# petabi/petal-decomposition

Measured on AMD Instinct MI355X. Metric: samples/sec for RandomizedPca.fit() on n x d fp32, higher is better.
Workload: dtype f32

## Files before the change

include/petal_hip.h:

```cpp
#ifndef PETAL_HIP_H
#define PETAL_HIP_H

#include <stddef.h>
#include <stdint.h>

#ifdef __cplusplus
extern "C" {
#endif

typedef struct petal_ctx petal_ctx;

enum { PETAL_OK = 0, PETAL_INVALID_INPUT = 1, PETAL_LINALG_ERROR = 2, PETAL_DEVICE_ERROR = 3 };
enum { PETAL_F32 = 0, PETAL_F64 = 1 };
enum { PETAL_HOST = 0, PETAL_DEVICE = 1 };
enum { PETAL_SUM = 0, PETAL_MAX = 1, PETAL_MIN = 2 };
enum { PETAL_ICA_TEXTBOOK = 0, PETAL_ICA_REFERENCE_LITERAL = 1 };
enum { PETAL_ICA_CONTRAST_LOGCOSH = 0, PETAL_ICA_CONTRAST_EXP = 16, PETAL_ICA_CONTRAST_CUBE = 32 };
enum { PETAL_ICA_SEMANTICS_MASK = 15, PETAL_ICA_CONTRAST_MASK = 240 };

typedef struct petal_matrix {
    void*   data;
    int64_t rows, cols;
    int64_t row_stride, col_stride;
    int32_t dtype;
// ... 12 lines not shown
    double  pass_bytes;
    double  ica_step_ms;
    int64_t ica_step_launches;
    double  ica_step_flops;
    double  ica_step_bytes;
    int64_t n_iter;
    int64_t allreduce_calls;
    double  allreduce_bytes;
    double  allreduce_ms;
    int64_t allreduce_timed;
    int64_t x_row_pitch_bytes;
    int64_t x_zero_copy;
    int64_t rpca_redo;
    double  pow_ms;
    int64_t pow_launches;
    double  stream_ms;
    int64_t stream_launches;
    int64_t ica_redo;
    int64_t ica_gram_split;
    int64_t means_folded;
    int64_t eigh_redo;
} petal_stats;

int         petal_ctx_create(int device, void* stream, petal_ctx** out);
void        petal_ctx_destroy(petal_ctx* ctx);
const char* petal_last_error(const petal_ctx* ctx);
const char* petal_version(void);
int         petal_ctx_set_collective(petal_ctx* ctx, petal_allreduce_fn fn, void* user, int rank, int world_size);
int         petal_rccl_unique_id(void* out128);
int         petal_ctx_init_rccl(petal_ctx* ctx, const void* unique_id128, int rank, int world_size);
int         petal_ctx_collective_info(const petal_ctx* ctx, int* kind, int* rank, int* world_size, int* comm_count, int* comm_device,
                                      int* comm_rank);
int         petal_ctx_set_profiling(petal_ctx* ctx, int profiling);
#define PETAL_GEMM_SPLIT_BF16X3 0
#define PETAL_GEMM_FP32_MFMA 1
#define PETAL_GEMM_SPLIT_BF16X3_EXACT 2
int         petal_ctx_set_gemm_mode(petal_ctx* ctx, int mode);
#define PETAL_OPT_TWO_PLANE_OPERANDS 0
#define PETAL_OPT_TWO_PLANE_OMEGA 1
#define PETAL_OPT_TWO_PLANE_ITERATE 2
#define PETAL_OPT_STEERING_PASSES 3
#define PETAL_OPT_FUSED_PASS 4
#define PETAL_OPT_FUSED_PASS_MIN_ROWS 5
#define PETAL_OPT_VERDICT_THRESHOLD 6
#define PETAL_OPT_MEANS_FOLD_ROWS 7
#define PETAL_OPT_GRAM_SPLIT 8
#define PETAL_OPT_GRAM_SPLIT_HOOK 9
#define PETAL_OPT_D2H_KERNEL 10
#define PETAL_OPT_ROW_PAD 11
#define PETAL_OPT_EIGH_JACOBI 12
#define PETAL_OPT_POISON 13
#define PETAL_OPT_FORCE_COLLECTIVE 14
#define PETAL_OPT_STEERING_HOOK 15
int         petal_ctx_set_option(petal_ctx* ctx, int option, double value);
int         petal_ctx_get_option(const petal_ctx* ctx, int option, double* value);
int         petal_get_stats(const petal_ctx* ctx, petal_stats* out);

int petal_pca_fit(petal_ctx* ctx, const petal_matrix* x, int64_t k, int centering,
                  void* components, void* means, void* singular, void* total_variance,
                  const petal_matrix* y_out);

int petal_rpca_fit(petal_ctx* ctx, const petal_matrix* x, int64_t k, int64_t n_oversample, int64_t n_iter,
                   int centering, const void* omega,
                   void* components, void* means, void* singular, void* total_variance,
                   const petal_matrix* y_out);

int petal_transform(petal_ctx* ctx, const petal_matrix* x, const void* components, const void* means,
                    int64_t k, int64_t d, int centering, const petal_matrix* y_out);
int petal_inverse_transform(petal_ctx* ctx, const petal_matrix* y, const void* components, const void* means,
                            int64_t k, int64_t d, int centering, const petal_matrix* x_out);

int petal_fastica_fit(petal_ctx* ctx, const petal_matrix* x, int64_t n_components, double tol, int64_t max_iter,
                      int mode, const void* w_init, void* components, void* means, int64_t* n_iter,
                      const petal_matrix* y_out);

int petal_ica_par(petal_ctx* ctx, const petal_matrix* x1, double tol, int64_t max_iter, int mode,
                  const void* w_init, void* w_out, int64_t* n_iter);
int petal_symmetric_decorrelation(petal_ctx* ctx, const void* w, int64_t nc, int32_t dtype, int mode, void* out);
int petal_logcosh(petal_ctx* ctx, const petal_matrix* x, const petal_matrix* g_out, void* gprime_out);
int petal_svd_flip(petal_ctx* ctx, const petal_matrix* u, const petal_matrix* vt);

int petal_gemm_xp(petal_ctx* ctx, const petal_matrix* x, const void* mu, const void* p, int64_t N, const void* bias,
                  const petal_matrix* z_out);
int petal_gemm_atb(petal_ctx* ctx, const petal_matrix* a, const void* mu_a, const petal_matrix* b, const void* mu_b,
                   double* c_out);

int petal_power_pass(petal_ctx* ctx, const petal_matrix* x, const void* mu, const void* p, int64_t N, double* y_out,
                     const petal_matrix* z_out, int* fused_out);

#ifdef __cplusplus
}
#endif
#endif
```

petal-decomposition_amd/__init__.py:

```python
from __future__ import annotations

import ctypes as C
import os
import weakref
from typing import Optional

import numpy as np

_HERE = os.path.dirname(os.path.abspath(__file__))
DEFAULT_LIBRARY = os.path.join(_HERE, "libpetal_hip.so")

PETAL_OK, PETAL_INVALID_INPUT, PETAL_LINALG_ERROR, PETAL_DEVICE_ERROR = 0, 1, 2, 3
PETAL_F32, PETAL_F64 = 0, 1
PETAL_HOST, PETAL_DEVICE = 0, 1
PETAL_SUM, PETAL_MAX, PETAL_MIN = 0, 1, 2
GEMM_SPLIT_BF16X3, GEMM_FP32_MFMA, GEMM_SPLIT_BF16X3_EXACT = 0, 1, 2
OPTIONS = {"two_plane_operands": 0, "two_plane_omega": 1, "two_plane_iterate": 2, "steering_passes": 3, "fused_pass": 4,
           "fused_pass_min_rows": 5, "verdict_threshold": 6, "means_fold_rows": 7, "gram_split": 8, "gram_split_hook": 9,
           "d2h_kernel": 10, "row_pad": 11, "eigh_jacobi": 12, "poison": 13, "force_collective": 14, "steering_hook": 15,
           "ipca_fallback": 32,
           "pca_dual": 33, "pca_dual_fallback": 34,
           "kpca_fallback": 36,
           "nmf_fallback": 38}
ICA_TEXTBOOK, ICA_REFERENCE_LITERAL = 0, 1
ICA_CONTRAST_LOGCOSH, ICA_CONTRAST_EXP, ICA_CONTRAST_CUBE = 0, 16, 32
ICA_SEMANTICS_MASK, ICA_CONTRAST_MASK = 15, 240
_ICA_FUN = {"logcosh": ICA_CONTRAST_LOGCOSH, "exp": ICA_CONTRAST_EXP, "cube": ICA_CONTRAST_CUBE}


def _ica_contrast(fun) -> int:
    try:
        return _ICA_FUN[fun]
    except (KeyError, TypeError):
        raise InvalidInput(f"unknown contrast function {fun!r}: one of {sorted(_ICA_FUN)}") from None


from .pcg import Pcg


class DecompositionError(Exception):
    """``DecompositionError`` (src/lib.rs:22-28)."""


class InvalidInput(DecompositionError):
    def __str__(self):
        return "invalid matrix: " + super().__str__()


class LinalgError(DecompositionError):
    def __str__(self):
        return "linear algerba operation failed: " + super().__str__()


class DeviceError(DecompositionError):
    pass


class petal_matrix(C.Structure):
    _fields_ = [("data", C.c_void_p), ("rows", C.c_int64), ("cols", C.c_int64),
                ("row_stride", C.c_int64), ("col_stride", C.c_int64),
                ("dtype", C.c_int32), ("space", C.c_int32)]


class petal_stats(C.Structure):
    _fields_ = [("fit_ms", C.c_double),
                ("xp_ms", C.c_double), ("xp_launches", C.c_int64),
                ("atb_ms", C.c_double), ("atb_launches", C.c_int64),
                ("pass_flops", C.c_double), ("pass_bytes", C.c_double),
                ("ica_step_ms", C.c_double), ("ica_step_launches", C.c_int64),
                ("ica_step_flops", C.c_double), ("ica_step_bytes", C.c_double),
                ("n_iter", C.c_int64),
                ("allreduce_calls", C.c_int64), ("allreduce_bytes", C.c_double),
                ("allreduce_ms", C.c_double), ("allreduce_timed", C.c_int64),
                ("x_row_pitch_bytes", C.c_int64), ("x_zero_copy", C.c_int64),
                ("rpca_redo", C.c_int64), ("pow_ms", C.c_double), ("pow_launches", C.c_int64),
                ("stream_ms", C.c_double), ("stream_launches", C.c_int64), ("ica_redo", C.c_int64), ("ica_gram_split", C.c_int64),
# ... 2034 lines not shown
```

petal-decomposition_amd/csrc/algo.cpp:

```cpp
#include <algorithm>
#include <chrono>
#include <cstdint>
#include <memory>

#include "ctx.h"
#include "../../include/petal_hip_sparse.h"
#include "../../include/petal_hip_ipca.h"
#include "../../include/petal_hip_kpca.h"

namespace petal {

namespace {

double get_elem(const void* p, int dt, int64_t i) {
    return dt == F64 ? static_cast<const double*>(p)[i] : static_cast<double>(static_cast<const float*>(p)[i]);
}
void put_elem(void* p, int dt, int64_t i, double v) {
    if (dt == F64) static_cast<double*>(p)[i] = v;
    else static_cast<float*>(p)[i] = static_cast<float>(v);
}

void check_matrix(const petal_matrix& m, const char* what) {
    if (m.dtype != PETAL_F32 && m.dtype != PETAL_F64) invalid_input(std::string(what) + ": unsupported dtype");
    if (m.rows < 0 || m.cols < 0) invalid_input(std::string(what) + ": negative shape");
// ... 608 lines not shown
                                 steer && it + 1 < n_iter);
                    dev_set_tag(c.dev, TAG_NONE);
                }
            } else {
                op_dgemm(c.dev, true, false, LP, LP, dp, 1.0, Pcur, LP, Yp, LP, 0.0, G, LP);
                op_chol_inv(c.dev, G, L, LP, T.f64(), LP, tol_drop, nullptr, LP);
                op_dgemm(c.dev, false, false, dp, LP, LP, 1.0, Yp, LP, T.f64(), LP, 0.0, Y.f64(), LP);
                op_refill_zero_cols(c.dev, Y.f64(), dp, L, LP, P.f64(), LP);
                orthonormalize_small(c, Y, dp, L, LP, 1e-13);
                dev_set_tag(c.dev, TAG_XP);
                op_gemm_xp(c.dev, dt, X.p, n, dp, X.ld, muT.p, Y.f64(), LP, LP, nullptr, Z.p, LP, nullptr);
                dev_set_tag(c.dev, TAG_NONE);
            }
            Pcur = Y.f64();
        }
        return Pcur;
    }
    void range_basis(const Attempt& a, const double* Pcur) {
        t_rt = false;
        steered = use_pow || steer;
        if (n_iter > 0 && !a.robust) {
            if (!have_yp) {
                dev_set_tag(c.dev, TAG_ATB);
                op_gemm_atb(c.dev, dt, X.p, X.ld, dp, muT.p, Z.p, LP, LP, nullptr, n, Yp, LP);
                dev_set_tag(c.dev, TAG_NONE);
                allreduce_f64(c, Yp, dp * LP + 1, PETAL_SUM);
            }
            op_dgemm(c.dev, true, false, LP, LP, dp, 1.0, Pcur, LP, Yp, LP, 0.0, G, LP);
            t_rt = slot_flip && op_chol_rt(c.dev, dt, n, G, L, LP, T.f64(), LP, tol_drop, ndead, LP, std::max<int64_t>(k, 1));
            if (!slot_flip) op_chol_inv(c.dev, G, L, LP, T.f64(), LP, tol_drop, ndead, LP, std::max<int64_t>(k, 1));
            Usrc = Z.p; Ubuf = Z1.p;
        } else {
            op_gemm_atb(c.dev, dt, Z.p, LP, LP, nullptr, Z.p, LP, LP, nullptr, n, G, LP, true);
            allreduce_f64(c, G, LP * LP, PETAL_SUM);
            op_chol_inv(c.dev, G, L, LP, T.f64(), LP, tol_tall, nullptr, LP);
            op_gemm_xp(c.dev, dt, Z.p, n, LP, LP, nullptr, T.f64(), LP, LP, nullptr, Z1.p, LP, nullptr);
            op_gemm_atb(c.dev, dt, Z1.p, LP, LP, nullptr, Z1.p, LP, LP, nullptr, n, G, LP, true);
            dev_set_tag(c.dev, TAG_ATB);
            op_gemm_atb(c.dev, dt, X.p, X.ld, dp, muT.p, Z1.p, LP, LP, nullptr, n, Yp, LP);
            dev_set_tag(c.dev, TAG_NONE);
            allreduce_f64(c, G, LP * LP, PETAL_SUM);
            allreduce_f64(c, Yp, dp * LP + 1, PETAL_SUM);
            op_chol_inv(c.dev, G, L, LP, T.f64(), LP, tol_tall, nullptr, LP);
            Usrc = Z1.p; Ubuf = Z.p;
        }
        if (t_rt) op_trsm_right(c.dev, Yp, dp, LP, T.f64(), LP, LP, Bt.f64(), LP);
        else op_dgemm(c.dev, false, false, dp, LP, LP, 1.0, Yp, LP, T.f64(), LP, 0.0, Bt.f64(), LP);
    }
    void small_stage(const Attempt& a) {
        if (a.jacobi) dev_memset(c.dev, ndead, 0, 2 * sizeof(double));
        op_dgemm(c.dev, true, false, LP, LP, dp, 1.0, Bt.f64(), LP, Bt.f64(), LP, 0.0, S.f64(), LP);
        if (!a.robust && !a.jacobi) op_eigh(c.dev, S.f64(), L, LP, Uh.f64(), LP, lam, dt == F32 ? 1e-8 : 1e-15, false, LP, std::max<int64_t>(k, 1), neig);
        else op_eigh(c.dev, S.f64(), L, LP, Uh.f64(), LP, lam, dt == F32 ? 1e-8 : 1e-15, true, LP);
        if (!a.robust && !a.exact && two_plane_applies)
            op_tail_verdict(c.dev, lam, L, std::max<int64_t>(k, 1), (tv_from_sq && !tv_direct) ? mu64 : nullptr, dp, d, in.ri.n_total,
                            tv_direct ? mu64 + dp : tvp, steered ? 4e-6 * 1.2 : 4e-6, p2_thr, ndead);
        op_components_out(c.dev, dt, Bt.f64(), LP, Uh.f64(), LP, lam, dt == F32 ? 1e-7 : 1e-12, d, L, k, comp_dev);

        dev_set_tag(c.dev, TAG_STREAM);
        if (slot_flip)
            op_gemm_xp_prod_absmax(c.dev, dt, Usrc, n, LP, LP, nullptr, T.f64(), LP, LP, Uh.f64(), kp, LP, M2.f64(), LP, Ubuf, LP,
                                   in.ri.row_offset, flip, flip + kp, flip + 2 * kp, y_out != nullptr, t_rt);
        else
            op_gemm_xp_prod(c.dev, dt, Usrc, n, LP, LP, nullptr, T.f64(), LP, LP, Uh.f64(), kp, LP, M2.f64(), LP, Ubuf, LP);
        dev_set_tag(c.dev, TAG_NONE);
        Uout = Ubuf;
    }
    void read_back(const Attempt& a) {
        if (slot_flip) flip_signs_to_slot(c, dt, kp, flip, !a.robust ? ndead : nullptr);
        const size_t hres_len = size_t(o.len - o.tv);
        const bool one_view = sizeof(double) * hres_len + comp_bytes <= dev_view_limit(c.dev);
        const double* hres = static_cast<const double*>(dev_d2h_view(c.dev, tvp, sizeof(double) * hres_len + (one_view ? comp_bytes : 0)));
        hcomp = hres + hres_len;
        if (!one_view) {
            comp_keep.resize(comp_bytes);
            dev_d2h(c.dev, comp_keep.data(), comp_dev, comp_bytes);
            hcomp = comp_keep.data();
        }
        dev_sync(c.dev);
        keep.assign(hres, hres + hres_len);
        if (one_view && sharded(c) && !flip_slot_keys(c, dt)) {
            comp_keep.assign(static_cast<const char*>(hcomp), static_cast<const char*>(hcomp) + comp_bytes);
            hcomp = comp_keep.data();
        }
    }
    const double* host(int64_t offset) const { return &keep[size_t(offset - o.tv)]; }
    double verdict() {
        int hdead[3] = {0, 0, 0};
        std::memcpy(hdead, host(o.verdict), sizeof(hdead));
        double code = verdict_code(hdead);
        if (sharded(c)) code = flip_slot_keys(c, dt) ? *host(o.agreed) : agree_max(c, code);
        return code;
    }
    void write_out(const PcaOutputs& out) {
        const std::vector<double> sg = slot_flip ? signs_from_slot(c, dt, host(o.flip), kp)
                                                 : flip_signs(c, dt, Uout, n, kp, LP, in.ri.row_offset);
        const double* hlam = host(o.lam);
        std::vector<double> hs(size_t(std::max<int64_t>(k, 1)), 0.0);
        for (int64_t j = 0; j < k; ++j) hs[j] = std::sqrt(std::max(hlam[j], 0.0));
        const double* hmu = host(o.mu);
        double htv = keep[0];
        if (tv_direct) htv = hmu[dp];
        else if (tv_from_sq) {
            htv = 0;
            for (int64_t j = 0; j < d; ++j) htv += std::max(0.0, hmu[dp + j] - in.ri.n_total * hmu[j] * hmu[j]);
        }
        {
            bool finite = std::isfinite(keep[0]) && std::isfinite(htv);
            for (int64_t j = 0; j < d; ++j) finite = finite && std::isfinite(hmu[j]) && (!tv_from_sq || tv_direct || std::isfinite(hmu[dp + j]));
            for (int64_t j = 0; j < k; ++j) finite = finite && std::isfinite(hlam[j]);
            if (!finite) linalg_error("did not converge");
        }
        write_pca_outputs(c, out, dt, k, d, hcomp, sg.data(), hs.data(), hmu, htv, Uout, n, LP);
    }
};

}

void rpca_fit(petal_ctx& c, const petal_matrix& x, int64_t k, int64_t n_oversample, int64_t n_iter, bool centering,
              const void* omega, void* components, void* means, void* singular, void* total_variance,
              const petal_matrix* y_out) {
    const Timer timer = start_fit(c, x);
    if (k < 0 || n_oversample < 0 || n_iter < 0) invalid_input("negative parameter");
    const int dt = x.dtype;
    const int64_t d = x.cols, l_req = k + n_oversample;
    if (sharded(c) && d > 0 && l_req > 0 && omega == nullptr) invalid_input("omega is required");
    FitInput in = fit_input(c, x, !centering ? 0 : dt == F32 ? 2 : 1, omega, d * l_req);
    if (in.n_total < k || d < k) invalid_input("every dimension should be at least " + std::to_string(k));
    if (centering && in.n_total == 0) {
        if (y_out && (y_out->rows != 0)) invalid_input("output has the wrong shape");
        return;
    }
    const int64_t L = std::min(l_req, std::min(in.n_total, d));
    if (L > 0 && omega == nullptr) invalid_input("omega is required");
    if (d == 0 || L == 0) {
        if (total_variance) put_elem(total_variance, dt, 0, 0.0);
        if (y_out) emit(c, dt, nullptr, x.rows, 0, 0, *y_out);
        return;
    }
    if (!sharded(c)) in.X = ingest(c, x);
    RpcaRun run(c, in, y_out, k, l_req, n_iter, L, centering, omega);
    Attempt a{false, !run.two_plane_applies || dev_option(c.dev, OPT_TWO_PLANE) == 0, false, run.rebase_sketch};
    for (int attempt = 0; attempt < 8; ++attempt) {
        if (!a.jacobi) run.pipeline(a);
        run.small_stage(a);
        run.read_back(a);
        if (!next_attempt(a, a.robust ? 0.0 : run.verdict(), n_iter, c.stats)) break;
    }
    run.write_out({components, means, singular, total_variance, y_out});
    c.stats.means_folded = run.tv_direct ? 1 : 0;
    finish_stats(c, timer);
}

__attribute__((weak)) bool op_row_gram(Dev*, int, const void*, int64_t, int64_t, int64_t, const double*, double*, int64_t, int64_t*) {
    return false;
}
namespace {
constexpr int64_t PCA_DUAL_MIN_D = 2048;
bool pca_dual_applies(const petal_ctx& c, int64_t n_total, int64_t d) {
    if (sharded(c) || c.pca_dual < 0) return false;
    return c.pca_dual > 0 || (n_total < d && d > PCA_DUAL_MIN_D);
}
struct RowGram { bool kernel = false; int64_t chunks = 0; DBuf wide; };
RowGram row_gram_into(petal_ctx& c, const DevMat& X, const double* centre, double* K, int64_t ldk, bool force_fallback = false) {
    RowGram g;
    if (!c.pca_dual_fallback && !force_fallback) {
        dev_set_tag(c.dev, TAG_ATB);
        g.kernel = op_row_gram(c.dev, X.dtype, X.p, X.n, X.dp, X.ld, centre, K, ldk, &g.chunks);
        dev_set_tag(c.dev, TAG_NONE);
    }
    if (g.kernel) return g;
    g.chunks = 0;
    const int64_t n = X.n, dp = X.dp, count = (n - 1) * X.ld + dp;
    g.wide = DBuf(c.dev, sizeof(double) * size_t(count));
    op_cvt_to_f64(c.dev, X.dtype, g.wide.f64(), X.p, count);
    if (centre) {
        const std::vector<double> h1(size_t(n), 1.0);
        DBuf ones(c.dev, sizeof(double) * size_t(n));
        dev_h2d(c.dev, ones.p, h1.data(), ones.bytes);
        op_dgemm(c.dev, false, false, n, dp, 1, -1.0, ones.f64(), 1, centre, dp, 1.0, g.wide.f64(), X.ld);
    }
    op_dgemm(c.dev, false, true, n, n, dp, 1.0, g.wide.f64(), X.ld, g.wide.f64(), X.ld, 0.0, K, ldk);
    return g;
}

void pca_fit_dual(petal_ctx& c, const FitInput& in, int64_t k, bool centering, const PcaOutputs& out) {
    const DevMat& X = in.X;
    const int dt = X.dtype;
    const int64_t n = X.n, d = X.d, dp = X.dp, np = round_up(n, 16), kp = round_up(std::max<int64_t>(k, 1), 16);
    const size_t esz = dtype_size(dt);
    DBuf mu64, muT;
    column_means(c, X, double(n), centering, mu64, muT);
    DBuf K(c.dev, sizeof(double) * np * np), V(c.dev, sizeof(double) * np * np), lam(c.dev, sizeof(double) * np);
    DBuf sig(c.dev, sizeof(double) * np), inv(c.dev, sizeof(double) * np), diag(c.dev, sizeof(double) * np);
    dev_memset(c.dev, K.p, 0, K.bytes);
    RowGram g = row_gram_into(c, X, centering ? mu64.f64() : nullptr, K.f64(), np);
    c.pca_route[0] = 1; c.pca_route[1] = g.kernel ? 1 : 0; c.pca_route[2] = n; c.pca_route[3] = g.chunks;
    std::vector<double> hdiag(np), hs(np), hmu(dp);
    dev_copy2d(c.dev, diag.p, sizeof(double), K.p, (np + 1) * sizeof(double), sizeof(double), size_t(np), 2);
    dev_d2h(c.dev, hdiag.data(), diag.p, diag.bytes);
    dev_sync(c.dev);
    double tvar = 0;
    for (int64_t i = 0; i < n; ++i) tvar += hdiag[i];
    if (!std::isfinite(tvar)) linalg_error("did not converge");
    gram_eigen(c, dt, K, n, np, k, diag, V, lam, nullptr);
    op_sigma_inv(c.dev, lam.f64(), sig.f64(), inv.f64(), np, dt == F32 ? 1e-6 : 1e-10);
    if (centering && k >= n) dev_memset(c.dev, inv.f64() + (n - 1), 0, sizeof(double));
    const std::vector<double> sg = flip_signs(c, F64, V.p, n, k, np, 0);
// ... 3563 lines not shown
```

petal-decomposition_amd/csrc/api.cpp:

```cpp
#include <cstdio>
#include <new>

#include "ctx.h"
#include "../../include/petal_hip_score.h"
#include "../../include/petal_hip_segments.h"
#include "../../include/petal_hip_sparse.h"
#include "../../include/petal_hip_ipca.h"
#include "../../include/petal_hip_wide.h"
#include "../../include/petal_hip_kpca.h"
#include "../../include/petal_hip_nmf.h"
#include "../../include/petal_hip_nmf_sparse.h"
#include "../../include/petal_hip_nmf_kl.h"
#include "../../include/petal_hip_nmf_kl_dense.h"
#include "../../include/petal_hip_nmf_cd.h"
#include "../../include/petal_hip_probe.h"

using namespace petal;

namespace {

struct DeviceScope {
    petal::Dev* dev;
    int prev = -1;
    explicit DeviceScope(petal::Dev* d) : dev(d) { if (dev) prev = dev_push_current(dev); }
// ... 74 lines not shown

int petal_ctx_set_collective(petal_ctx* ctx, petal_allreduce_fn fn, void* user, int rank, int world_size) {
    return guarded(ctx, [&] {
        if (world_size < 1 || rank < 0 || rank >= world_size) invalid_input("bad rank / world_size");
        if (world_size > 1 && !fn) invalid_input("world_size > 1 needs an all-reduce hook");
        rccl_release(*ctx);
        ctx->allreduce = fn;
        ctx->allreduce_user = user;
        ctx->rank = rank;
        ctx->world = world_size;
    });
}

int petal_ctx_set_profiling(petal_ctx* ctx, int profiling) {
    return guarded(ctx, [&] {
        ctx->profiling = profiling < 0 ? 0 : (profiling > 2 ? 2 : profiling);
        dev_set_profiling(ctx->dev, ctx->profiling);
    });
}

int petal_ctx_collective_info(const petal_ctx* ctx, int* kind, int* rank, int* world_size, int* comm_count, int* comm_device,
                              int* comm_rank) {
    if (!ctx) return PETAL_INVALID_INPUT;
    int cnt = -1, dev = -1, rk = -1;
    petal::rccl_info(*ctx, &cnt, &dev, &rk);
    if (kind) *kind = ctx->rccl ? 2 : (ctx->allreduce ? 1 : 0);
    if (rank) *rank = ctx->rank;
    if (world_size) *world_size = ctx->world;
    if (comm_count) *comm_count = cnt;
    if (comm_device) *comm_device = dev;
    if (comm_rank) *comm_rank = rk;
    return PETAL_OK;
}

int petal_ctx_set_gemm_mode(petal_ctx* ctx, int mode) {
    return guarded(ctx, [&] {
        if (mode != PETAL_GEMM_SPLIT_BF16X3 && mode != PETAL_GEMM_FP32_MFMA && mode != PETAL_GEMM_SPLIT_BF16X3_EXACT) invalid_input("unknown GEMM mode");
        dev_set_gemm_mode(ctx->dev, mode);
    });
}

int petal_ctx_set_option(petal_ctx* ctx, int option, double value) {
    return guarded(ctx, [&] {
        if (option == PETAL_OPT_FORCE_COLLECTIVE) { ctx->force_collective = value != 0; return; }
        if (option == PETAL_OPT_IPCA_FALLBACK) { ctx->ipca_fallback = value != 0; return; }
        if (option == PETAL_OPT_PCA_DUAL) {
            if (!(value == value)) invalid_input("unknown ctx option or NaN value");
            ctx->pca_dual = value > 0 ? 1 : (value < 0 ? -1 : 0);
            return;
        }
        if (option == PETAL_OPT_PCA_DUAL_FALLBACK) { ctx->pca_dual_fallback = value != 0; return; }
        if (option == PETAL_OPT_KPCA_FALLBACK) { ctx->kpca_fallback = value != 0; return; }
        if (option == PETAL_OPT_NMF_FALLBACK) { ctx->nmf_fallback = value != 0; return; }
        if (option < 0 || option >= OPT_COUNT || !(value == value)) invalid_input("unknown ctx option or NaN value");
        dev_set_option(ctx->dev, option, value);
    });
}

int petal_ctx_get_option(const petal_ctx* ctx, int option, double* value) {
    if (!ctx || !value) return PETAL_INVALID_INPUT;
    if (option == PETAL_OPT_FORCE_COLLECTIVE) { *value = ctx->force_collective ? 1.0 : 0.0; return PETAL_OK; }
    if (option == PETAL_OPT_IPCA_FALLBACK) { *value = ctx->ipca_fallback ? 1.0 : 0.0; return PETAL_OK; }
    if (option == PETAL_OPT_PCA_DUAL) { *value = double(ctx->pca_dual); return PETAL_OK; }
    if (option == PETAL_OPT_PCA_DUAL_FALLBACK) { *value = ctx->pca_dual_fallback ? 1.0 : 0.0; return PETAL_OK; }
    if (option == PETAL_OPT_KPCA_FALLBACK) { *value = ctx->kpca_fallback ? 1.0 : 0.0; return PETAL_OK; }
    if (option == PETAL_OPT_NMF_FALLBACK) { *value = ctx->nmf_fallback ? 1.0 : 0.0; return PETAL_OK; }
    if (option < 0 || option >= OPT_COUNT) return PETAL_INVALID_INPUT;
    *value = dev_option(ctx->dev, option);
    return PETAL_OK;
}

int petal_get_stats(const petal_ctx* ctx, petal_stats* out) {
    if (!ctx || !out) return PETAL_INVALID_INPUT;
    *out = ctx->stats;
    return PETAL_OK;
}

int petal_pca_fit(petal_ctx* ctx, const petal_matrix* x, int64_t k, int centering, void* components, void* means,
                  void* singular, void* total_variance, const petal_matrix* y_out) {
    return guarded(ctx, [&] {
        need(x, "x");
        pca_fit(*ctx, *x, k, centering != 0, components, means, singular, total_variance, y_out);
    });
}

int petal_rpca_fit(petal_ctx* ctx, const petal_matrix* x, int64_t k, int64_t n_oversample, int64_t n_iter,
                   int centering, const void* omega, void* components, void* means, void* singular,
                   void* total_variance, const petal_matrix* y_out) {
    return guarded(ctx, [&] {
        need(x, "x");
        rpca_fit(*ctx, *x, k, n_oversample, n_iter, centering != 0, omega, components, means, singular, total_variance,
                 y_out);
    });
}

int petal_transform(petal_ctx* ctx, const petal_matrix* x, const void* components, const void* means, int64_t k,
                    int64_t d, int centering, const petal_matrix* y_out) {
    return guarded(ctx, [&] {
        need(x, "x");
        need(y_out, "y_out");
        transform(*ctx, *x, components, means, k, d, centering != 0, *y_out);
    });
}

int petal_inverse_transform(petal_ctx* ctx, const petal_matrix* y, const void* components, const void* means,
                            int64_t k, int64_t d, int centering, const petal_matrix* x_out) {
    return guarded(ctx, [&] {
        need(y, "y");
        need(x_out, "x_out");
        inverse_transform(*ctx, *y, components, means, k, d, centering != 0, *x_out);
    });
}

int petal_score_rows(petal_ctx* ctx, const petal_matrix* x, const void* components, const void* means, int64_t k, int64_t d,
                     int centering, const void* weights, const petal_matrix* out, const petal_matrix* y_out) {
    return guarded(ctx, [&] {
        need(x, "x");
        need(out, "out");
        score_rows(*ctx, *x, components, means, k, d, centering != 0, weights, *out, y_out);
// ... 554 lines not shown
```

petal-decomposition_amd/csrc/hip_ops.hip:

```cpp
#include <hip/hip_runtime.h>

#include <algorithm>
#include <cmath>
#include <cstdio>
#include <cstdlib>
#include <cstring>
#include <map>
#include <set>
#include <stdexcept>
#include <string>
#include <type_traits>
#include <unordered_map>
#include <vector>

#include "ops.h"

namespace petal {

#define HIP_CHECK(expr)                                                                                   \
    do {                                                                                                  \
        hipError_t _e = (expr);                                                                           \
        if (_e != hipSuccess)                                                                             \
            throw std::runtime_error(std::string("HIP error: ") + hipGetErrorString(_e) + " at " #expr);  \
    } while (0)
// ... 3 lines not shown
#ifdef PETAL_DEBUG_COUNTERS
__device__ int g_dbg[4];
__device__ long long g_cyc[32];
__device__ long long g_trace[8 * 16];
#define DBG_T(i) do { if (threadIdx.x == 0) { long long _t = clock64(); g_cyc[i] += _t - _t0; _t0 = _t; } } while (0)
}
extern "C" void petal_debug_trace(long long* out128) {
    (void)hipDeviceSynchronize();
    (void)hipMemcpyFromSymbol(out128, HIP_SYMBOL(petal::g_trace), sizeof(long long) * 128);
}
extern "C" void petal_debug_counters(long long* cyc16, int* dbg4) {
    (void)hipDeviceSynchronize();
    (void)hipMemcpyFromSymbol(cyc16, HIP_SYMBOL(petal::g_cyc), sizeof(long long) * 32);
    (void)hipMemcpyFromSymbol(dbg4, HIP_SYMBOL(petal::g_dbg), sizeof(int) * 4);
    long long z[32] = {0}; int zi[4] = {0};
    (void)hipMemcpyToSymbol(HIP_SYMBOL(petal::g_cyc), z, sizeof(z));
    (void)hipMemcpyToSymbol(HIP_SYMBOL(petal::g_dbg), zi, sizeof(zi));
}
namespace petal {
#else
#define DBG_T(i) do {} while (0)
#endif

struct Dev {
    int device = 0;
    hipStream_t stream = nullptr;
    bool own_stream = false;
    hipStream_t side = nullptr, main_saved = nullptr;
    hipEvent_t ev_fork = nullptr, ev_join = nullptr;
    bool forked = false, on_side = false;
    std::vector<void*> deferred_free;
    int gemm_mode = [] { const char* e = getenv("PETAL_GEMM"); return (e && std::string(e) == "fp32") ? 1 : (e && std::string(e) == "bf16x3-exact") ? 2 : 0; }();
    void* ica_wpk3 = nullptr;
    size_t ica_wpk3_bytes = 0;
    const double* ica_wpk3_for = nullptr;
    int64_t ica_wpk3_nc = 0;
    bool ica_wpk3_valid = false;
    void* ica_x1pl = nullptr;
    size_t ica_x1pl_bytes = 0;
    const void* ica_x1pl_for = nullptr;
    int64_t ica_x1pl_n = 0, ica_x1pl_ld = 0;
    double ica_ortho_tol2 = 1e-26;
    int profiling = 0;
    int tag = 0;
    int tag_seen[TAG_COUNT] = {};
    int tag_count[TAG_COUNT] = {};
    int tag_pick[TAG_COUNT] = {};
    int tag_active = 0;
    int fit_index = 0;
    char* pin = nullptr;
    char* pin_dev = nullptr;
    bool d2h_kernel = true;
    double opt[OPT_COUNT] = {};
    size_t pin_cap = 0, pin_used = 0;
    struct Pend { void* dst; size_t off, bytes; };
    std::vector<Pend> pend;
    std::multimap<size_t, void*> free_list, free_cold;
    bool side_nowait = false;
    std::unordered_map<void*, size_t> live;
    std::vector<hipEvent_t> ev_pool;
    struct Rec { int tag; hipEvent_t a, b; };
    std::vector<Rec> recs;
    KernelTiming acc;
    std::set<const void*> max_lds_set;
    int num_cu = 0;
    int* progress = nullptr;
};

static void dev_defaults_from_env(Dev* d) {
    auto on = [](const char* name) { return getenv(name) != nullptr; };
    auto num = [](const char* name, double dflt) { const char* e = getenv(name); return e ? atof(e) : dflt; };
    d->opt[OPT_TWO_PLANE] = on("PETAL_NO_P2") ? 0 : 1;
    d->opt[OPT_TWO_PLANE_OMEGA] = on("PETAL_NO_P2_OMEGA") ? 0 : 1;
    d->opt[OPT_TWO_PLANE_ITERATE] = on("PETAL_NO_P2_ITERATE") ? 0 : 1;
    d->opt[OPT_STEERING] = on("PETAL_NO_POW3_FAST") ? 0 : 1;
    d->opt[OPT_FUSED_PASS] = on("PETAL_NO_POW3") ? 0 : 1;
    d->opt[OPT_FUSED_PASS_MIN_ROWS] = num("PETAL_POW3_MIN_ROWS", 8192);
    d->opt[OPT_VERDICT_THRESHOLD] = num("PETAL_P2_VERDICT_THR", 4e-6);
    d->opt[OPT_MEANS_FOLD_ROWS] = on("PETAL_NO_MEANS_FOLD") ? -1 : num("PETAL_MEANS_FOLD_ROWS", 200000);
    d->opt[OPT_GRAM_SPLIT] = on("PETAL_NO_GRAM3") ? 0 : 1;
    d->opt[OPT_GRAM_SPLIT_HOOK] = on("PETAL_GRAM_SPLIT") ? 1 : 0;
    d->opt[OPT_D2H_KERNEL] = on("PETAL_D2H_MEMCPY") ? 0 : 1;
    d->opt[OPT_ROW_PAD] = on("PETAL_NO_ROW_PAD") ? 0 : 1;
    d->opt[OPT_EIGH_JACOBI] = on("PETAL_EIGH_JACOBI") ? 1 : 0;
    d->opt[OPT_POISON] = on("PETAL_POISON") ? 1 : 0;
    d->opt[OPT_STEERING_HOOK] = 0;
    d->d2h_kernel = d->opt[OPT_D2H_KERNEL] != 0;
}
void dev_set_option(Dev* d, int opt, double value) {
    if (opt < 0 || opt >= OPT_COUNT) throw std::invalid_argument("unknown ctx option");
    d->opt[opt] = value;
    if (opt == OPT_D2H_KERNEL) d->d2h_kernel = value != 0;
}
double dev_option(const Dev* d, int opt) {
    if (opt < 0 || opt >= OPT_COUNT) throw std::invalid_argument("unknown ctx option");
    return d->opt[opt];
}
static inline bool opt_on(const Dev* d, int opt) { return d->opt[opt] != 0; }

Dev* dev_create(int device, void* stream, char* err, size_t errlen) {
    auto fail = [&](const std::string& m) -> Dev* {
        if (err && errlen) std::snprintf(err, errlen, "%s", m.c_str());
        return nullptr;
    };
    int count = 0;
    hipError_t e = hipGetDeviceCount(&count);
    if (e != hipSuccess || count <= 0)
        return fail(std::string("no HIP device visible (") + hipGetErrorString(e) + "); this library has no CPU fallback");
    if (device < 0 || device >= count) return fail("device index out of range");
    if (hipSetDevice(device) != hipSuccess) return fail("hipSetDevice failed");
    hipDeviceProp_t prop;
    if (hipGetDeviceProperties(&prop, device) != hipSuccess) return fail("hipGetDeviceProperties failed");
    if (std::string(prop.gcnArchName).find("gfx950") == std::string::npos)
        return fail(std::string("device is ") + prop.gcnArchName + ", this library is built for gfx950 (MI355X) only");
    Dev* d = new Dev();
    d->device = device;
    dev_defaults_from_env(d);
    if (stream) {
        d->stream = static_cast<hipStream_t>(stream);
    } else {
        if (hipStreamCreateWithFlags(&d->stream, hipStreamNonBlocking) != hipSuccess) {
            delete d;
            return fail("hipStreamCreate failed");
        }
        d->own_stream = true;
    }
    return d;
}

void dev_destroy(Dev* d) {
    if (!d) return;
    (void)hipSetDevice(d->device);
    (void)hipStreamSynchronize(d->stream);
    for (auto& kv : d->free_list) (void)hipFree(kv.second);
    for (auto& kv : d->free_cold) (void)hipFree(kv.second);
    for (auto& kv : d->live) (void)hipFree(kv.first);
    for (auto& r : d->recs) { (void)hipEventDestroy(r.a); (void)hipEventDestroy(r.b); }
    for (auto ev : d->ev_pool) (void)hipEventDestroy(ev);
    if (d->pin) (void)hipHostFree(d->pin);
    if (d->progress) (void)hipHostFree(d->progress);
// ... 359 lines not shown
```

petal-decomposition_amd/csrc/kernels/host_gemm.inc:

```
#define DISPATCH_T(dt, ...)                              \
    do {                                                 \
        if ((dt) == F64) { using T = double; __VA_ARGS__; } \
        else { using T = float; __VA_ARGS__; }           \
    } while (0)

void op_pack_strided(Dev* d, int dt, const void* src, int64_t n, int64_t dd, int64_t rs, int64_t cs, void* dst, int64_t ld,
                     int64_t dpad) {
    if (n == 0 || dpad == 0) return;
    const int64_t blocks = (n * dpad + 1023) / 1024;
    if (blocks < (int64_t(1) << 31)) {
        DISPATCH_T(dt, hipLaunchKernelGGL(k_pack_flat<T>, dim3((unsigned)blocks), dim3(256), 0, d->stream, (const T*)src, n, dd, rs, cs,
                                          (T*)dst, ld, dpad));
    } else {
        DISPATCH_T(dt, hipLaunchKernelGGL(k_pack_strided<T>, dim3((unsigned)n, cdiv(dpad, 256)), dim3(256), 0, d->stream,
                                          (const T*)src, n, dd, rs, cs, (T*)dst, ld, dpad));
    }
    launch_check();
}
void op_unpack_strided(Dev* d, int dt, const void* src, int64_t n, int64_t dd, int64_t ld, void* dst, int64_t rs, int64_t cs,
                       const double* scale) {
    if (n == 0 || dd == 0) return;
    const int64_t blocks = (n * dd + 1023) / 1024;
    if (blocks < (int64_t(1) << 31)) {
        DISPATCH_T(dt, hipLaunchKernelGGL(k_unpack_scaled<T>, dim3((unsigned)blocks), dim3(256), 0, d->stream, (const T*)src, n, dd, ld,
// ... 52 lines not shown
    launch_check();
}
static bool aligned16(const void* p) { return (reinterpret_cast<uintptr_t>(p) & 15) == 0; }
static bool gemm_split_product(const Dev* d) { return d->gemm_mode != 1; }
static void set_max_lds(Dev* d, const void* fn) {
    if (d->max_lds_set.count(fn)) return;
    HIP_CHECK(hipFuncSetAttribute(fn, hipFuncAttributeMaxDynamicSharedMemorySize, 160 * 1024));
    d->max_lds_set.insert(fn);
}
void op_scale_pad_cols(Dev* d, const double* V, int64_t ldv, const double* inv, int64_t rows, int64_t r, int64_t rp, double* P) {
    if (rows == 0 || rp == 0) return;
    hipLaunchKernelGGL(k_scale_pad_cols, dim3(cdiv(rows * rp, 256)), dim3(256), 0, d->stream, V, ldv, inv, rows, r, rp, P);
    launch_check();
}
void op_transpose_out(Dev* d, int dt, const double* V, int64_t ldv, int64_t dd, int64_t k, void* comp) {
    if (dd == 0 || k == 0) return;
    const dim3 grid(cdiv(dd, 32), cdiv(k, 32));
    if (dt == F32) hipLaunchKernelGGL(k_transpose_out<float>, grid, dim3(256), 0, d->stream, V, ldv, dd, k, (float*)comp);
    else hipLaunchKernelGGL(k_transpose_out<double>, grid, dim3(256), 0, d->stream, V, ldv, dd, k, (double*)comp);
    launch_check();
}
void op_components_out(Dev* d, int dt, const double* Bt, int64_t ldb, const double* Uh, int64_t ldu, const double* lam, double thr,
                       int64_t dd, int64_t L, int64_t k, void* comp) {
    if (k == 0 || dd == 0) return;
    const dim3 grid(cdiv(dd, 64), cdiv(k, 16));
    if (dt == F32)
        hipLaunchKernelGGL(k_components_out<float>, grid, dim3(256), 0, d->stream, Bt, ldb, Uh, ldu, lam, thr, dd, (int)L, k, (float*)comp);
    else
        hipLaunchKernelGGL(k_components_out<double>, grid, dim3(256), 0, d->stream, Bt, ldb, Uh, ldu, lam, thr, dd, (int)L, k, (double*)comp);
    launch_check();
}
static int num_cus(Dev* d) {
    if (!d->num_cu) { hipDeviceProp_t prop; HIP_CHECK(hipGetDeviceProperties(&prop, d->device)); d->num_cu = prop.multiProcessorCount; }
    return d->num_cu;
}

template <int RT, int NT>
static void launch_xp(Dev* d, const float* X, int64_t n, int K, int64_t ldx, const float* mu, const float* Ppk, int NTtot,
                      int nt0, int N, const float* bias, float* Z, int64_t ldz, double* ss_part, int blocks) {
    const bool center = mu != nullptr, ss = ss_part != nullptr;
#define XP_ARGS X, n, K, ldx, mu, Ppk, NTtot, nt0, N, bias, Z, ldz, ss_part
    if (center && ss) hipLaunchKernelGGL((k_xp_mfma<RT, NT, true, true>), dim3(blocks), dim3(256), 0, d->stream, XP_ARGS);
    else if (center) hipLaunchKernelGGL((k_xp_mfma<RT, NT, true, false>), dim3(blocks), dim3(256), 0, d->stream, XP_ARGS);
    else if (ss) hipLaunchKernelGGL((k_xp_mfma<RT, NT, false, true>), dim3(blocks), dim3(256), 0, d->stream, XP_ARGS);
    else hipLaunchKernelGGL((k_xp_mfma<RT, NT, false, false>), dim3(blocks), dim3(256), 0, d->stream, XP_ARGS);
#undef XP_ARGS
    launch_check();
}

struct AbsmaxReq { int64_t cols, row_offset; double *absmax, *idx, *sign; };
static void gemm_xp_impl(Dev* d, int dt, const void* X, int64_t n, int64_t K, int64_t ldx, const void* mu, const double* P, int64_t N,
                         int64_t ldp, const void* bias, void* Z, int64_t ldz, double* sumsq, const double* prod_A, int64_t prod_M,
                         int64_t prod_lda, double* prod_out, int64_t prod_ldo, int prod_rt, const AbsmaxReq* am = nullptr,
                         bool p2_hint = false, bool steering = false);
void op_gemm_xp(Dev* d, int dt, const void* X, int64_t n, int64_t K, int64_t ldx, const void* mu, const double* P, int64_t N,
                int64_t ldp, const void* bias, void* Z, int64_t ldz, double* sumsq, int p_planes, bool steering) {
    gemm_xp_impl(d, dt, X, n, K, ldx, mu, P, N, ldp, bias, Z, ldz, sumsq, nullptr, 0, 0, nullptr, 0, false, nullptr, p_planes == 2, steering);
}
void op_gemm_xp_prod(Dev* d, int dt, const void* X, int64_t n, int64_t K, int64_t ldx, const void* mu, const double* A, int64_t M,
                     int64_t lda, const double* T, int64_t N, int64_t ldt, double* P_out, int64_t ldpo, void* Z, int64_t ldz) {
    const bool fused = dt == F32 && gemm_split_product(d) && n >= 64 && K % 16 == 0 && K > 0 && N % 16 == 0 && ldx % 4 == 0 &&
                       aligned16(X) && (!mu || aligned16(mu)) && ldz % 4 == 0 && aligned16(Z) && K < (1 << 24) && N < (1 << 24);
    if (fused) {
        double* tmpo = P_out ? nullptr : (double*)dev_alloc(d, sizeof(double) * K * N);
        gemm_xp_impl(d, dt, X, n, K, ldx, mu, T, N, ldt, nullptr, Z, ldz, nullptr, A, M, lda, P_out ? P_out : tmpo, P_out ? ldpo : N, false);
        if (tmpo) dev_free(d, tmpo);
        return;
    }
    double* tmp = nullptr;
    double* P = P_out;
    int64_t ldp = ldpo;
    if (!P) { tmp = (double*)dev_alloc(d, sizeof(double) * K * N); P = tmp; ldp = N; }
    op_dgemm(d, false, false, K, N, M, 1.0, A, lda, T, ldt, 0.0, P, ldp);
    op_gemm_xp(d, dt, X, n, K, ldx, mu, P, N, ldp, nullptr, Z, ldz, nullptr);
    if (tmp) dev_free(d, tmp);
}
void op_gemm_xp_prod_absmax(Dev* d, int dt, const void* X, int64_t n, int64_t K, int64_t ldx, const void* mu, const double* A, int64_t M,
                            int64_t lda, const double* T, int64_t N, int64_t ldt, double* P_out, int64_t ldpo, void* Z, int64_t ldz,
                            int64_t row_offset, double* absmax, double* idx, double* sign, bool store_product, bool a_rt) {
    const bool fused = dt == F32 && gemm_split_product(d) && n >= 64 && K % 16 == 0 && K > 0 && N % 16 == 0 && N > 0 && ldx % 4 == 0 &&
                       aligned16(X) && (!mu || aligned16(mu)) && ldz % 4 == 0 && aligned16(Z) && K < (1 << 24) && N < (1 << 24) &&
                       n < (int64_t(1) << 31) && P_out != nullptr;
    if (a_rt && !(M == K && M % 16 == 0 && M <= TRSM_MAXM && N % 16 == 0 && P_out != nullptr)) throw std::logic_error("op_gemm_xp_prod_absmax: RT-form operand of a shape the solve does not take");
    if (a_rt && !fused) {
        switch ((int)(M / 16)) {
#define PETAL_TRSML_CASE(NB)                                                                                                       \
    case NB:                                                                                                                       \
        hipLaunchKernelGGL((k_trsm_left_pack<NB>), dim3(cdiv(N, 16)), dim3(64), 0, d->stream, A, lda, T, ldt, P_out, ldpo, (bf16x8*)nullptr, 0); \
        break
            PETAL_TRSML_CASE(1); PETAL_TRSML_CASE(2); PETAL_TRSML_CASE(3); PETAL_TRSML_CASE(4); PETAL_TRSML_CASE(5);
            PETAL_TRSML_CASE(6); PETAL_TRSML_CASE(7); PETAL_TRSML_CASE(8); PETAL_TRSML_CASE(9);
#undef PETAL_TRSML_CASE
            default: throw std::logic_error("op_gemm_xp_prod_absmax: order out of range");
        }
        launch_check();
        op_gemm_xp_absmax(d, dt, X, n, K, ldx, mu, P_out, N, ldpo, Z, ldz, row_offset, absmax, idx, sign, store_product);
        return;
    }
    if (!fused) {
        op_gemm_xp_prod(d, dt, X, n, K, ldx, mu, A, M, lda, T, N, ldt, P_out, ldpo, Z, ldz);
        op_col_absmax(d, dt, Z, n, N, ldz, row_offset, absmax, idx, sign);
        return;
    }
    const AbsmaxReq am{N, row_offset, absmax, idx, sign};
    gemm_xp_impl(d, dt, X, n, K, ldx, mu, T, N, ldt, nullptr, store_product ? Z : nullptr, ldz, nullptr, A, M, lda, P_out, ldpo, a_rt ? 2 : 0, &am);
}
void op_gemm_xp_absmax(Dev* d, int dt, const void* X, int64_t n, int64_t K, int64_t ldx, const void* mu, const double* P, int64_t N,
                       int64_t ldp, void* Z, int64_t ldz, int64_t row_offset, double* absmax, double* idx, double* sign, bool store_product) {
    const bool fused = dt == F32 && gemm_split_product(d) && n >= 64 && K % 16 == 0 && K > 0 && N % 16 == 0 && N > 0 && ldx % 4 == 0 &&
                       aligned16(X) && (!mu || aligned16(mu)) && ldz % 4 == 0 && aligned16(Z) && K < (1 << 24) && N < (1 << 24) &&
                       n < (int64_t(1) << 31);
    if (!fused) {
        op_gemm_xp(d, dt, X, n, K, ldx, mu, P, N, ldp, nullptr, Z, ldz, nullptr);
        op_col_absmax(d, dt, Z, n, N, ldz, row_offset, absmax, idx, sign);
        return;
    }
    const AbsmaxReq am{N, row_offset, absmax, idx, sign};
    gemm_xp_impl(d, dt, X, n, K, ldx, mu, P, N, ldp, nullptr, store_product ? Z : nullptr, ldz, nullptr, nullptr, 0, 0, nullptr, 0, false, &am);
}
static void gemm_xp_impl(Dev* d, int dt, const void* X, int64_t n, int64_t K, int64_t ldx, const void* mu, const double* P, int64_t N,
                         int64_t ldp, const void* bias, void* Z, int64_t ldz, double* sumsq, const double* prod_A, int64_t prod_M,
                         int64_t prod_lda, double* prod_out, int64_t prod_ldo, int prod_rt, const AbsmaxReq* am, bool p2_hint, bool steering) {
    if (n == 0 || N == 0) return;
    const bool mfma = dt == F32 && K % 16 == 0 && K > 0 && ldx % 4 == 0 && aligned16(X) && (!mu || aligned16(mu)) && n >= 64 &&
                      K < (1 << 24) && N < (1 << 24) && N % 16 == 0 && ldz % 4 == 0 && aligned16(Z) && (!bias || aligned16(bias));
    const bool mfma64 = dt == F64 && K % 8 == 0 && K > 0 && ldx % 2 == 0 && aligned16(X) && (!mu || aligned16(mu)) && n >= 64 &&
                        K < (1 << 24) && N < (1 << 24) && N % 16 == 0;
    if (am && !(mfma && gemm_split_product(d) && !sumsq)) throw std::logic_error("gemm_xp_impl: abs-max epilogue outside the split-product path");
    if (mfma64) {
        const int NTtot = cdiv(N, 16);
        const int64_t total = (K / 8) * (int64_t)NTtot * 64;
        f64x2* Ppk = (f64x2*)dev_alloc(d, sizeof(f64x2) * total);
        hipLaunchKernelGGL(k_pack_p64, dim3(cdiv(total, 256)), dim3(256), 0, d->stream, P, K, N, ldp, Ppk, NTtot, total);
        launch_check();
        const int blocks = cdiv(n, 128);
        double* ssp = sumsq ? (double*)dev_alloc(d, sizeof(double) * blocks * 4) : nullptr;
        const double* Xd = (const double*)X; const double* mud = (const double*)mu; const double* bd = (const double*)bias; double* Zd = (double*)Z;
        TagScope ts(d);
        for (int nt0 = 0; nt0 < NTtot;) {
            const int rem = NTtot - nt0;
            const int w = rem >= 5 ? 5 : rem;
            double* sp = nt0 == 0 ? ssp : nullptr;
#define XP64_ARGS Xd, n, (int)K, ldx, mud, Ppk, NTtot, nt0, (int)N, bd, Zd, ldz, sp
#define XP64_LAUNCH(NTv)                                                                                                            \
            do {                                                                                                                    \
                if (mud && sp) hipLaunchKernelGGL((k_xp_f64<NTv, true, true>), dim3(blocks), dim3(256), 0, d->stream, XP64_ARGS);    \
                else if (mud) hipLaunchKernelGGL((k_xp_f64<NTv, true, false>), dim3(blocks), dim3(256), 0, d->stream, XP64_ARGS);    \
                else if (sp) hipLaunchKernelGGL((k_xp_f64<NTv, false, true>), dim3(blocks), dim3(256), 0, d->stream, XP64_ARGS);     \
                else hipLaunchKernelGGL((k_xp_f64<NTv, false, false>), dim3(blocks), dim3(256), 0, d->stream, XP64_ARGS);            \
            } while (0)
            switch (w) {
                case 5: XP64_LAUNCH(5); break;
                case 4: XP64_LAUNCH(4); break;
                case 3: XP64_LAUNCH(3); break;
                case 2: XP64_LAUNCH(2); break;
                default: XP64_LAUNCH(1); break;
            }
#undef XP64_LAUNCH
#undef XP64_ARGS
            launch_check();
            nt0 += w;
        }
        ts.stop();
        if (sumsq) {
            hipLaunchKernelGGL(k_add_scalar_parts, dim3(1), dim3(256), 0, d->stream, ssp, (int64_t)blocks * 4, sumsq);
            launch_check();
            dev_free(d, ssp);
        }
        dev_free(d, Ppk);
        return;
    }
    if (!mfma) {
        double* ssp = sumsq ? (double*)dev_alloc(d, sizeof(double) * n) : nullptr;
        TagScope ts(d);
        DISPATCH_T(dt, hipLaunchKernelGGL(k_xp_simple<T>, dim3((unsigned)n, cdiv(N, 64)), dim3(64), 0, d->stream, (const T*)X, n,
                                          K, ldx, (const T*)mu, P, N, ldp, (const T*)bias, (T*)Z, ldz, ssp));
        launch_check();
        ts.stop();
        if (sumsq) {
            hipLaunchKernelGGL(k_add_scalar_parts, dim3(1), dim3(256), 0, d->stream, ssp, n, sumsq);
            launch_check();
            dev_free(d, ssp);
        }
        return;
    }
    const int NTtot = cdiv(N, 16);
    if (gemm_split_product(d) && !sumsq) {
        const int64_t nch = (K + 31) / 32, total = nch * NTtot * 64;
        bf16x8* Ppk3 = (bf16x8*)dev_alloc(d, sizeof(bf16x8) * total * 3);
        const bool no_p2 = !opt_on(d, OPT_TWO_PLANE);
        const bool no_p2_it = no_p2 || !opt_on(d, OPT_TWO_PLANE_ITERATE), no_p2_om = no_p2 || !opt_on(d, OPT_TWO_PLANE_OMEGA);
        const bool p2 = p2_hint && ((prod_A && prod_rt && !no_p2_it) || (!prod_A && !no_p2_om)) && !am;
        const bool x2 = p2 && steering && opt_on(d, OPT_STEERING);
        if (prod_A) {
            if (prod_rt == 2) {
                switch ((int)(prod_M / 16)) {
#define PETAL_TRSML_CASE(NB)                                                                                                       \
    case NB:                                                                                                                       \
        hipLaunchKernelGGL((k_trsm_left_pack<NB>), dim3(cdiv(N, 16)), dim3(64), 0, d->stream, prod_A, prod_lda, P, ldp, prod_out, prod_ldo, Ppk3, NTtot); \
        break
                    PETAL_TRSML_CASE(1); PETAL_TRSML_CASE(2); PETAL_TRSML_CASE(3); PETAL_TRSML_CASE(4); PETAL_TRSML_CASE(5);
                    PETAL_TRSML_CASE(6); PETAL_TRSML_CASE(7); PETAL_TRSML_CASE(8); PETAL_TRSML_CASE(9);
#undef PETAL_TRSML_CASE
                    default: throw std::runtime_error("k_trsm_left_pack: order out of range");
                }
            } else if (prod_rt)
                switch ((int)(N / 16)) {
#define PETAL_TRSM_CASE(NB)                                                                                                        \
    case NB:                                                                                                                       \
        if (p2) hipLaunchKernelGGL((k_trsm_pack<NB, true>), dim3(cdiv(K, 16)), dim3(64), trsm_lds_bytes(16 * NB), d->stream, prod_A, prod_lda, P,  \
                                   ldp, K, prod_out, prod_ldo, Ppk3, NTtot);                                                       \
        else hipLaunchKernelGGL((k_trsm_pack<NB, false>), dim3(cdiv(K, 16)), dim3(64), trsm_lds_bytes(16 * NB), d->stream, prod_A, prod_lda, P,  \
                           ldp, K, prod_out, prod_ldo, Ppk3, NTtot);                                                               \
        break
                    PETAL_TRSM_CASE(1); PETAL_TRSM_CASE(2); PETAL_TRSM_CASE(3); PETAL_TRSM_CASE(4); PETAL_TRSM_CASE(5);
                    PETAL_TRSM_CASE(6); PETAL_TRSM_CASE(7); PETAL_TRSM_CASE(8); PETAL_TRSM_CASE(9);
#undef PETAL_TRSM_CASE
                    default: throw std::runtime_error("k_trsm_pack: order out of range");
                }
            else
            hipLaunchKernelGGL(k_dgemm, dim3(cdiv(N, 16), cdiv(K, 16)), dim3(16, 16), 0, d->stream, false, false, K, N, prod_M, 1.0,
                               prod_A, prod_lda, P, ldp, 0.0, prod_out, prod_ldo, prod_M, (double*)nullptr, (const double*)nullptr,
                               Ppk3, NTtot);
        } else {
            hipLaunchKernelGGL(k_pack_p3, dim3(cdiv(total, 256)), dim3(256), 0, d->stream, P, K, N, ldp, Ppk3, NTtot, total);
        }
        launch_check();
        constexpr int RTv = PETAL_XP3_RT, DPv = PETAL_XP3_DEPTH;
        const float* Xf = (const float*)X; const float* muf = (const float*)mu; const float* bf = (const float*)bias; float* Zf = (float*)Z;
        static_assert(RTv == 4, "both workgroup shapes below cover 256 rows: one abs-max partial per 256 rows");
        const int64_t am_parts = cdiv(n, 256), am_ld = am ? am->cols : 0;
        double* am_part = am ? (double*)dev_alloc(d, sizeof(double) * 3 * am_parts * am_ld) : nullptr;
        TagScope ts(d);
        const int npass = cdiv(NTtot, 9);
        for (int nt0 = 0, pass = 0; nt0 < NTtot; ++pass) {
            const int w = (NTtot - nt0 + (npass - pass) - 1) / (npass - pass);
            const size_t lds = sizeof(bf16x8) * 2 * w * 64 * (p2 ? 2 : 3) + sizeof(float) * 32 * nch;
#define XP3_LAUNCH8P(NTv, NPLv)                                                                                                           \
            do {                                                                                                                            \
                const int blocksw = cdiv(n, 256);                                                                                           \
                if (lds > 64 * 1024) set_max_lds(d, muf ? reinterpret_cast<const void*>(k_xp3<2, NTv, DPv, true, 8, PETAL_XP3_OCC, NPLv>) : reinterpret_cast<const void*>(k_xp3<2, NTv, DPv, false, 8, PETAL_XP3_OCC, NPLv>)); \
                if (muf) hipLaunchKernelGGL((k_xp3<2, NTv, DPv, true, 8, PETAL_XP3_OCC, NPLv>), dim3(blocksw), dim3(512), lds, d->stream, Xf, n, (int)K, ldx, muf, Ppk3, NTtot, nt0, (int)N, bf, Zf, ldz, am_part, am_ld); \
                else hipLaunchKernelGGL((k_xp3<2, NTv, DPv, false, 8, PETAL_XP3_OCC, NPLv>), dim3(blocksw), dim3(512), lds, d->stream, Xf, n, (int)K, ldx, muf, Ppk3, NTtot, nt0, (int)N, bf, Zf, ldz, am_part, am_ld); \
            } while (0)
#define XP3_LAUNCH8X(NTv)                                                                                                                 \
            do {                                                                                                                            \
                const int blocksw = cdiv(n, 256);                                                                                           \
                if (lds > 64 * 1024) set_max_lds(d, muf ? reinterpret_cast<const void*>(k_xp3<2, NTv, DPv, true, 8, PETAL_XP3_OCC, 2, true>) : reinterpret_cast<const void*>(k_xp3<2, NTv, DPv, false, 8, PETAL_XP3_OCC, 2, true>)); \
                if (muf) hipLaunchKernelGGL((k_xp3<2, NTv, DPv, true, 8, PETAL_XP3_OCC, 2, true>), dim3(blocksw), dim3(512), lds, d->stream, Xf, n, (int)K, ldx, muf, Ppk3, NTtot, nt0, (int)N, bf, Zf, ldz, am_part, am_ld); \
                else hipLaunchKernelGGL((k_xp3<2, NTv, DPv, false, 8, PETAL_XP3_OCC, 2, true>), dim3(blocksw), dim3(512), lds, d->stream, Xf, n, (int)K, ldx, muf, Ppk3, NTtot, nt0, (int)N, bf, Zf, ldz, am_part, am_ld); \
            } while (0)
#define XP3_LAUNCH8(NTv) do { if (p2 && x2) XP3_LAUNCH8X(NTv); else if (p2) XP3_LAUNCH8P(NTv, 2); else XP3_LAUNCH8P(NTv, 3); } while (0)
            if (w >= 6) {
                switch (w) {
                    case 9: XP3_LAUNCH8(9); break;
                    case 8: XP3_LAUNCH8(8); break;
                    case 7: XP3_LAUNCH8(7); break;
                    default: XP3_LAUNCH8(6); break;
                }
                launch_check();
                nt0 += w;
                continue;
            }
#define XP3_LAUNCHP(RTw, NTv, NPLv)                                                                                                        \
            do {                                                                                                                            \
                const int blocksw = cdiv(n, 64 * RTw);                                                                                      \
                if (lds > 64 * 1024) set_max_lds(d, muf ? reinterpret_cast<const void*>(k_xp3<RTw, NTv, DPv, true, 4, PETAL_XP3_OCC, NPLv>) : reinterpret_cast<const void*>(k_xp3<RTw, NTv, DPv, false, 4, PETAL_XP3_OCC, NPLv>)); \
                if (muf) hipLaunchKernelGGL((k_xp3<RTw, NTv, DPv, true, 4, PETAL_XP3_OCC, NPLv>), dim3(blocksw), dim3(256), lds, d->stream, Xf, n, (int)K, ldx, muf, Ppk3, NTtot, nt0, (int)N, bf, Zf, ldz, am_part, am_ld); \
                else hipLaunchKernelGGL((k_xp3<RTw, NTv, DPv, false, 4, PETAL_XP3_OCC, NPLv>), dim3(blocksw), dim3(256), lds, d->stream, Xf, n, (int)K, ldx, muf, Ppk3, NTtot, nt0, (int)N, bf, Zf, ldz, am_part, am_ld); \
            } while (0)
#define XP3_LAUNCH(RTw, NTv) do { if (p2) XP3_LAUNCHP(RTw, NTv, 2); else XP3_LAUNCHP(RTw, NTv, 3); } while (0)
            switch (w) {
                case 5: XP3_LAUNCH(RTv, 5); break;
                case 4: XP3_LAUNCH(RTv, 4); break;
                case 3: XP3_LAUNCH(RTv, 3); break;
                case 2: XP3_LAUNCH(RTv, 2); break;
                default: XP3_LAUNCH(RTv, 1); break;
// ... 384 lines not shown
            do {                                                                                                                      \
                if (ma) hipLaunchKernelGGL((k_atb3<NTv, true, 8>), grid, block, 0, d->stream, Af, lda, (int)M, ma, Bf, ldb, (int)N, 16 * nt0, n_main, chunk, part, (int)N, (int)n_tail); \
                else hipLaunchKernelGGL((k_atb3<NTv, false, 8>), grid, block, 0, d->stream, Af, lda, (int)M, ma, Bf, ldb, (int)N, 16 * nt0, n_main, chunk, part, (int)N, (int)n_tail); \
            } while (0)
            switch (w) {
                case 5: ATB3_LAUNCH(5); break;
                case 4: ATB3_LAUNCH(4); break;
                case 3: ATB3_LAUNCH(3); break;
                case 2: ATB3_LAUNCH(2); break;
                default: ATB3_LAUNCH(1); break;
            }
#undef ATB3_LAUNCH
            launch_check();
        }
        if (split3_mode) {
            nt0 += w;
            continue;
        }
        switch (w) {
            case 5: launch_atb<5>(d, Af, lda, (int)M, ma, Bf, ldb, (int)N, 16 * nt0, mb, n, chunk, part, (int)nsplit); break;
            case 4: launch_atb<4>(d, Af, lda, (int)M, ma, Bf, ldb, (int)N, 16 * nt0, mb, n, chunk, part, (int)nsplit); break;
            case 3: launch_atb<3>(d, Af, lda, (int)M, ma, Bf, ldb, (int)N, 16 * nt0, mb, n, chunk, part, (int)nsplit); break;
            case 2: launch_atb<2>(d, Af, lda, (int)M, ma, Bf, ldb, (int)N, 16 * nt0, mb, n, chunk, part, (int)nsplit); break;
            default: launch_atb<1>(d, Af, lda, (int)M, ma, Bf, ldb, (int)N, 16 * nt0, mb, n, chunk, part, (int)nsplit); break;
        }
        nt0 += w;
    }
    ts.stop();
    if ((M * N) % 2 == 0 && N % 2 == 0)
        hipLaunchKernelGGL(k_sum_parts4, dim3(cdiv(M * N, 128)), dim3(256), 0, d->stream, part, nslab, M * N, C, N, ldc);
    else
        hipLaunchKernelGGL(k_sum_parts2<float>, dim3(cdiv(M * N, 32)), dim3(256), 0, d->stream, part, nslab, M * N, C, N, ldc, false);
    launch_check();
    dev_free(d, part);
}

__global__ void k_flip_key(const double* __restrict__ t, double* __restrict__ key, int64_t L, const int* __restrict__ flag) {
    const int64_t j = (int64_t)blockIdx.x * blockDim.x + threadIdx.x;
    if (j == L && flag) key[L] = verdict_code(flag);
    if (j >= L) return;
    const double a = t[j] < 0 ? 0.0 : t[j];
    unsigned long long bits = (unsigned long long)__double_as_longlong(a);
    const double rw = t[L + j];
    const unsigned long long row = rw < (double)(1ll << 28) ? (unsigned long long)rw : (1ull << 28) - 1;
    const unsigned long long payload = ((((1ull << 28) - 1) - row) << 1) | (t[2 * L + j] < 0 ? 1ull : 0ull);
    bits = (bits & ~((1ull << 29) - 1)) | (t[j] < 0 ? 0ull : payload);
    key[j] = __longlong_as_double((long long)bits);
}
void op_flip_key(Dev* d, const double* triple, double* key, int64_t L, const int* flag) {
    if (L == 0 && !flag) return;
    hipLaunchKernelGGL(k_flip_key, dim3(cdiv(L + 1, 256)), dim3(256), 0, d->stream, triple, key, L, flag);
    launch_check();
}
__global__ __launch_bounds__(256) void k_tail_verdict(const double* __restrict__ lam, int L, int k, const double* __restrict__ mu_sq, int dp,
                                                       int d, double n_total, const double* __restrict__ tvp, double eps2, double thr,
                                                       int* __restrict__ flag2) {
    __shared__ double red[256];
    const int tid = threadIdx.x;
    double s = 0;
    if (mu_sq) for (int j = tid; j < d; j += 256) s += fmax(0.0, mu_sq[dp + j] - n_total * mu_sq[j] * mu_sq[j]);
    red[tid] = s;
    __syncthreads();
    for (int st = 128; st > 0; st >>= 1) { if (tid < st) red[tid] += red[tid + st]; __syncthreads(); }
    const double tv = mu_sq ? red[0] : tvp[0];
    __syncthreads();
    s = 0;
    for (int j = tid; j < L; j += 256) s += fmax(lam[j], 0.0);
    red[tid] = s;
    __syncthreads();
    for (int st = 128; st > 0; st >>= 1) { if (tid < st) red[tid] += red[tid + st]; __syncthreads(); }
    const double tail = fmax(tv - red[0], 0.0);
    const double T = sqrt(fmax(lam[L - 1], 0.0) * tail / (double)d);
    int bad = 0;
    for (int j = tid; j < k && j < L; j += 256) {
        const double lj = lam[j];
        if (!(lj > 0.0)) continue;
        double gap = j + 1 < L ? lj - fmax(lam[j + 1], 0.0) : lj;
        if (j > 0) gap = fmin(gap, lam[j - 1] - lj);
        const double relgap = fmax(gap / lj, 1e-3);
        if (eps2 * T / lj / relgap > thr) bad = 1;
    }
    if (__syncthreads_or(bad) && tid == 0) flag2[1] = 1;
}
void op_tail_verdict(Dev* d, const double* lam, int64_t L, int64_t k, const double* mu_sq, int64_t dp, int64_t dd, double n_total,
                     const double* tv, double eps2, double thr, int* flag2) {
    if (L <= 0 || k <= 0) return;
    hipLaunchKernelGGL(k_tail_verdict, dim3(1), dim3(256), 0, d->stream, lam, (int)L, (int)k, mu_sq, (int)dp, (int)dd, n_total, tv, eps2, thr, flag2);
    launch_check();
}
void op_col_absmax(Dev* d, int dt, const void* U, int64_t n, int64_t L, int64_t ldu, int64_t row_offset, double* absmax,
                   double* idx, double* sign) {
    if (L == 0) return;
    const int64_t rows = scan_rows_per_block(n, L), nparts = std::max<int64_t>(1, cdiv(n, rows));
    double* part = (double*)dev_alloc(d, sizeof(double) * 3 * nparts * L);
    double *pm = part, *pi = part + nparts * L, *ps = part + 2 * nparts * L;
    if (n == 0) {
        std::vector<double> h(3 * L);
        for (int64_t j = 0; j < L; ++j) { h[j] = -1.0; h[L + j] = INFINITY; h[2 * L + j] = 1.0; }
        dev_h2d(d, absmax, h.data(), sizeof(double) * L);
        dev_h2d(d, idx, h.data() + L, sizeof(double) * L);
        dev_h2d(d, sign, h.data() + 2 * L, sizeof(double) * L);
        dev_free(d, part);
        return;
    }
    DISPATCH_T(dt, hipLaunchKernelGGL(k_absmax_part2<T>, dim3((unsigned)nparts, cdiv(L, 64)), dim3(256), 0, d->stream, (const T*)U,
                                      n, L, ldu, rows, pm, pi, ps));
    launch_check();
    hipLaunchKernelGGL(k_absmax_final, dim3((unsigned)L), dim3(64), 0, d->stream, pm, pi, ps, nparts, L, row_offset, absmax, idx, sign);
    launch_check();
    dev_free(d, part);
}

void op_scale_cols(Dev* d, int dt, void* A, int64_t n, int64_t L, int64_t lda, const double* s) {
    if (n == 0 || L == 0) return;
    DISPATCH_T(dt, hipLaunchKernelGGL(k_scale_cols<T>, dim3((unsigned)n, cdiv(L, 64)), dim3(64), 0, d->stream, (T*)A, n, L, lda, s));
    launch_check();
}
void op_logcosh_rows(Dev* d, int dt, const void* X, int64_t r, int64_t c, int64_t ldx, void* G, int64_t ldg, double* gp) {
    if (r == 0) return;
    DISPATCH_T(dt, hipLaunchKernelGGL(k_logcosh_rows<T>, dim3(cdiv(r, 64)), dim3(64), 0, d->stream, (const T*)X, r, c, ldx, (T*)G, ldg, gp));
    launch_check();
}
```

petal-decomposition_amd/csrc/kernels/host_pow3_eigh.inc:

```
static bool pow3_ok(Dev* d, int dt, const void* X, int64_t n, int64_t K, int64_t ldx, const void* mu, int64_t N, const void* Z, int64_t ldz) {
    const int64_t min_rows = (int64_t)d->opt[OPT_FUSED_PASS_MIN_ROWS];
    return opt_on(d, OPT_FUSED_PASS) && dt == F32 && d->gemm_mode == 0 && (K == 512 || K == 256) && N % 16 == 0 && N >= 16 && N <= 80 && n >= min_rows &&
           n < (int64_t(1) << 40) && ldx % 4 == 0 && aligned16(X) && (!mu || aligned16(mu)) && (!Z || (ldz >= N && aligned16(Z)));
}
static bool pow3_knob_off(const Dev* d, int opt) { return !opt_on(d, OPT_TWO_PLANE) || !opt_on(d, opt); }
bool op_power_pass_applies(Dev* d, int dt, const void* X, int64_t n, int64_t K, int64_t ldx, const void* mu, int64_t N) {
    return pow3_ok(d, dt, X, n, K, ldx, mu, N, nullptr, 0);
}
static void launch_pow3(Dev* d, const float* X, int64_t n, int64_t K, int64_t ldx, const float* mu, const bf16x8* Ppk3, int64_t N, float* Z, int64_t ldz,
                        double* Y, int64_t ldy, double** ssq_parts_out = nullptr, int* nparts_out = nullptr, bool steering = false) {
    const bool ssq_out = ssq_parts_out != nullptr;
    const bool no_fast = !opt_on(d, OPT_STEERING);
    if (steering && !no_fast && !Z) {
        const int NT = (int)(N / 16);
        const int64_t nstages = cdiv(n, 32);
        const int grid = (int)std::min<int64_t>(num_cus(d), nstages);
        float* part = (float*)dev_alloc(d, sizeof(float) * (size_t)grid * K * N);
        double* ssq_part = ssq_out ? (double*)dev_alloc(d, sizeof(double) * (size_t)grid * 8) : nullptr;
        const size_t lds = (size_t)8 * 8192 + (size_t)2 * 8 * NT * 1024 + (size_t)NT * 2048 + 2048;
#define POW3F_GO(NTv, CE, ME)                                                                                                      \
    do {                                                                                                                           \
        if (K == 512) {                                                                                                            \
            set_max_lds(d, reinterpret_cast<const void*>(k_pow3f<NTv, CE, ME, 2>));                                                \
            hipLaunchKernelGGL((k_pow3f<NTv, CE, ME, 2>), dim3(grid), dim3(512), lds, d->stream, X, n, ldx, mu, Ppk3, NT, part, nstages, ssq_part); \
        } else {                                                                                                                   \
            set_max_lds(d, reinterpret_cast<const void*>(k_pow3f<NTv, CE, ME, 1>));                                                \
            hipLaunchKernelGGL((k_pow3f<NTv, CE, ME, 1>), dim3(grid), dim3(512), lds, d->stream, X, n, ldx, mu, Ppk3, NT, part, nstages, ssq_part); \
        }                                                                                                                          \
    } while (0)
#define POW3F_NT(NTv) do { if (ssq_out) POW3F_GO(NTv, true, true); else if (mu) POW3F_GO(NTv, true, false); else POW3F_GO(NTv, false, false); } while (0)
        {
            TagScope ts(d);
            switch (NT) {
                case 5: POW3F_NT(5); break;
                case 4: POW3F_NT(4); break;
                case 3: POW3F_NT(3); break;
                case 2: POW3F_NT(2); break;
                default: POW3F_NT(1); break;
            }
            launch_check();
            ts.stop();
        }
#undef POW3F_NT
#undef POW3F_GO
        hipLaunchKernelGGL(k_sum_parts4, dim3(cdiv(K * N, 128)), dim3(256), 0, d->stream, part, (int64_t)grid, (int64_t)K * N, Y, N, ldy);
        launch_check();
        dev_free(d, part);
        if (ssq_parts_out) { *ssq_parts_out = ssq_part; *nparts_out = grid * 8; }
        return;
    }
    const int NT = (int)(N / 16);
    const int64_t nstages = cdiv(n, 32);
    const int grid = (int)std::min<int64_t>(num_cus(d), nstages);
    float* part = (float*)dev_alloc(d, sizeof(float) * (size_t)grid * K * N);
    double* ssq_part = ssq_out ? (double*)dev_alloc(d, sizeof(double) * (size_t)grid * 8) : nullptr;
    const size_t lds = (size_t)8 * 12288 + (size_t)8 * NT * 1024 + (size_t)NT * 3072 + 2048;
#define POW3_GO(NTv, CE, SZ, ME)                                                                                                  \
    do {                                                                                                                          \
        if (K == 512) {                                                                                                           \
            set_max_lds(d, reinterpret_cast<const void*>(k_pow3<NTv, CE, SZ, ME, 2>));                                            \
            hipLaunchKernelGGL((k_pow3<NTv, CE, SZ, ME, 2>), dim3(grid), dim3(512), lds, d->stream, X, n, ldx, mu, Ppk3, NT, part, Z, ldz, nstages, ssq_part); \
        } else {                                                                                                                  \
            set_max_lds(d, reinterpret_cast<const void*>(k_pow3<NTv, CE, SZ, ME, 1>));                                            \
            hipLaunchKernelGGL((k_pow3<NTv, CE, SZ, ME, 1>), dim3(grid), dim3(512), lds, d->stream, X, n, ldx, mu, Ppk3, NT, part, Z, ldz, nstages, ssq_part); \
        }                                                                                                                         \
    } while (0)
#define POW3_NT(NTv)                                                                                                              \
    do {                                                                                                                          \
        if (ssq_out) POW3_GO(NTv, true, false, true);                                                                             \
        else if (mu && Z) POW3_GO(NTv, true, true, false); else if (mu) POW3_GO(NTv, true, false, false);                         \
        else if (Z) POW3_GO(NTv, false, true, false); else POW3_GO(NTv, false, false, false);                                     \
    } while (0)
    {
        TagScope ts(d);
        switch (NT) {
            case 5: POW3_NT(5); break;
            case 4: POW3_NT(4); break;
            case 3: POW3_NT(3); break;
            case 2: POW3_NT(2); break;
            default: POW3_NT(1); break;
        }
        launch_check();
        ts.stop();
    }
#undef POW3_NT
#undef POW3_GO
    hipLaunchKernelGGL(k_sum_parts4, dim3(cdiv(K * N, 128)), dim3(256), 0, d->stream, part, (int64_t)grid, (int64_t)K * N, Y, N, ldy);
    launch_check();
    dev_free(d, part);
    if (ssq_parts_out) { *ssq_parts_out = ssq_part; *nparts_out = grid * 8; }
}
template <bool FINISH>
__global__ __launch_bounds__(256) void k_mean_fix(double* __restrict__ Y, int K, int d, int N, int64_t ldy, int c1, int L, double n_total,
                                                  const double* __restrict__ P, int64_t ldp, double* __restrict__ mu64, float* __restrict__ muT,
                                                  const double* __restrict__ ssq_part, int nparts, double* __restrict__ tv) {
    __shared__ double sd[512];
    __shared__ double sr[256];
    __shared__ double st[4];
    const int tid = threadIdx.x;
    if (FINISH) {
        for (int f = tid; f < K; f += 256) Y[(int64_t)f * ldy + c1] = 0.0;
        return;
    }
    for (int f = tid; f < K; f += 256) sd[f] = f < d ? Y[(int64_t)f * ldy + c1] / n_total : 0.0;
    __syncthreads();
    const int j0 = blockIdx.x * 4, jj = tid & 3, fl = tid >> 2;
    double acc = 0;
    auto two_plane = [](double v) {
        auto bf = [](float f) {
            unsigned u = __float_as_uint(f);
            u = (u + 0x7fffu + ((u >> 16) & 1u)) & 0xffff0000u;
            return __uint_as_float(u);
        };
        const float f = (float)v, h = bf(f), m = bf(f - h);
        return (double)h + (double)m;
    };
    if (j0 + jj < L)
        for (int f = fl; f < K; f += 64) acc += sd[f] * two_plane(P[(int64_t)f * ldp + j0 + jj]);
    sr[tid] = acc;
    __syncthreads();
    if (tid < 4) {
        double t = 0;
        for (int g = 0; g < 64; ++g) t += sr[g * 4 + tid];
        st[tid] = t;
    }
    __syncthreads();
    if (j0 + jj < L && j0 + jj != c1)
        for (int f = fl; f < K; f += 64) Y[(int64_t)f * ldy + j0 + jj] -= n_total * sd[f] * st[jj];
    if (blockIdx.x == 0) {
        double q = 0;
        for (int f = tid; f < K; f += 256) q += sd[f] * sd[f];
        double sp = 0;
        for (int e = tid; e < nparts; e += 256) sp += ssq_part[e];
        __syncthreads();
        sr[tid] = q;
        __syncthreads();
        for (int h = 128; h > 0; h >>= 1) { if (tid < h) sr[tid] += sr[tid + h]; __syncthreads(); }
        const double q2 = sr[0];
        __syncthreads();
        sr[tid] = sp;
        __syncthreads();
        for (int h = 128; h > 0; h >>= 1) { if (tid < h) sr[tid] += sr[tid + h]; __syncthreads(); }
        if (tid == 0) tv[0] = fmax(sr[0] - n_total * q2, 0.0);
        for (int f = tid; f < K; f += 256) {
            const double m = (double)muT[f] + sd[f];
            mu64[f] = m;
            muT[f] = (float)m;
        }
    }
}
bool op_power_pass_means(Dev* d, int dt, const void* X, int64_t n, int64_t K, int64_t dcols, int64_t ldx, double n_total, const double* P,
                         int64_t N, int64_t ldp, int64_t L, double* Y, int64_t ldy, double* mu64, void* muT, double* ssq_scratch, double* tv) {
    const bool off = d->opt[OPT_MEANS_FOLD_ROWS] < 0 || pow3_knob_off(d, OPT_TWO_PLANE_OMEGA);
    if (off || L >= N || !pow3_ok(d, dt, X, n, K, ldx, muT, N, nullptr, 0)) return false;
    const int64_t ns = std::min<int64_t>(n, 4096), stride = n / ns;
    op_colmean(d, dt, X, ns, K, ldx * stride, double(ns), mu64, muT, false);
    const int64_t total = (K / 32) * (N / 16) * 64;
    bf16x8* Ppk3 = (bf16x8*)dev_alloc(d, sizeof(bf16x8) * total * 3);
    hipLaunchKernelGGL(k_pack_p3, dim3(cdiv(total, 256)), dim3(256), 0, d->stream, P, K, N, ldp, Ppk3, (int)(N / 16), total);
    launch_check();
    double* parts = nullptr;
    int nparts = 0;
    launch_pow3(d, (const float*)X, n, K, ldx, (const float*)muT, Ppk3, N, nullptr, 0, Y, ldy, &parts, &nparts, true);
    dev_free(d, Ppk3);
    (void)ssq_scratch;
    const int c1 = (int)(N - 1);
    hipLaunchKernelGGL(k_mean_fix<false>, dim3((unsigned)cdiv(L, 4)), dim3(256), 0, d->stream, Y, (int)K, (int)dcols, (int)N, ldy, c1, (int)L, n_total, P, ldp,
                       mu64, (float*)muT, (const double*)parts, nparts, tv);
    hipLaunchKernelGGL(k_mean_fix<true>, dim3(1), dim3(256), 0, d->stream, Y, (int)K, (int)dcols, (int)N, ldy, c1, (int)L, n_total, P, ldp, mu64,
                       (float*)muT, (const double*)parts, nparts, tv);
    launch_check();
    dev_free(d, parts);
    return true;
}
bool op_power_pass(Dev* d, int dt, const void* X, int64_t n, int64_t K, int64_t ldx, const void* mu, const double* P, int64_t N, int64_t ldp,
                   void* Z, int64_t ldz, double* Y, int64_t ldy, bool steering) {
    const bool knob = pow3_knob_off(d, OPT_TWO_PLANE_OMEGA);
    if (knob || !pow3_ok(d, dt, X, n, K, ldx, mu, N, Z, ldz)) return false;
    const int64_t total = (K / 32) * (N / 16) * 64;
    bf16x8* Ppk3 = (bf16x8*)dev_alloc(d, sizeof(bf16x8) * total * 3);
    hipLaunchKernelGGL(k_pack_p3, dim3(cdiv(total, 256)), dim3(256), 0, d->stream, P, K, N, ldp, Ppk3, (int)(N / 16), total);
    launch_check();
    launch_pow3(d, (const float*)X, n, K, ldx, (const float*)mu, Ppk3, N, (float*)Z, ldz, Y, ldy, nullptr, nullptr, steering && Z == nullptr);
    dev_free(d, Ppk3);
    return true;
}
bool op_rebase_power_pass(Dev* d, int dt, const void* X, int64_t n, int64_t K, int64_t ldx, const void* mu, const double* G, int64_t L,
                          int64_t ldg, double rel_tol, int* ndead, const double* A, int64_t M, int64_t lda, double* T, int64_t ldt,
                          double* P_out, int64_t ldpo, void* Z, int64_t ldz, double* Y, int64_t ldy, bool steering) {
    const bool no_rt = pow3_knob_off(d, OPT_TWO_PLANE_ITERATE);
    if (!pow3_ok(d, dt, X, n, K, ldx, mu, M, Z, ldz) || no_rt || L == 0 || L > CHOL2_MAXL || M > TRSM_MAXM || M < L || P_out == nullptr) return false;
    launch_chol_rt(d, G, L, ldg, T, ldt, rel_tol, ndead, M);
    const int NTtot = (int)(M / 16);
    const int64_t total = (K / 32) * (int64_t)NTtot * 64;
    bf16x8* Ppk3 = (bf16x8*)dev_alloc(d, sizeof(bf16x8) * total * 3);
    switch (NTtot) {
#define PETAL_TRSM_CASE(NB)                                                                                                            \
    case NB:                                                                                                                           \
        hipLaunchKernelGGL((k_trsm_pack<NB, true>), dim3(cdiv(K, 16)), dim3(64), trsm_lds_bytes(16 * NB), d->stream, A, lda, T, ldt, K, P_out, \
                           ldpo, Ppk3, NTtot);                                                                                         \
        break
        PETAL_TRSM_CASE(1); PETAL_TRSM_CASE(2); PETAL_TRSM_CASE(3); PETAL_TRSM_CASE(4); PETAL_TRSM_CASE(5);
#undef PETAL_TRSM_CASE
        default: throw std::runtime_error("op_rebase_power_pass: order out of range");
    }
    launch_check();
    launch_pow3(d, (const float*)X, n, K, ldx, (const float*)mu, Ppk3, M, (float*)Z, ldz, Y, ldy, nullptr, nullptr, steering && Z == nullptr);
    dev_free(d, Ppk3);
    return true;
}

// ... 388 lines not shown
```

petal-decomposition_amd/csrc/kernels/k_eigen.inc:

```
constexpr int TMW_NV = 8;
__global__ __launch_bounds__(256) void k_tridiag_mw(double* __restrict__ W, int64_t ld, int L, int k, const double* __restrict__ vp_prev,
                                                    double* __restrict__ vp_cur, double* __restrict__ dd, double* __restrict__ ee,
                                                    double* __restrict__ HV, double* __restrict__ tau) {
    extern __shared__ __attribute__((aligned(16))) double sm_mw[];
    double* svp = sm_mw;
    double* swp = svp + L;
    double* svn = swp + L;
    double* s_red = svn + L;
    const int tid = threadIdx.x, lane = tid & 63, wv = tid >> 6;
    int red_slot = 0;
    auto block_sum = [&](double a) {
        for (int off = 32; off > 0; off >>= 1) a += __shfl_xor(a, off, 64);
        double* slot = s_red + 4 * red_slot;
        red_slot ^= 1;
        if (lane == 0) slot[wv] = a;
        __syncthreads();
        return (slot[0] + slot[1]) + (slot[2] + slot[3]);
    };
    double vq[TMW_NV], pq[TMW_NV];
    double pv = 0;
#pragma unroll
    for (int t = 0; t < TMW_NV; ++t) {
        const int j = tid + 256 * t;
        vq[t] = (k > 0 && j < L) ? vp_prev[j] : 0.0;
// ... 1227 lines not shown
    __syncthreads();
    if ((tid & 63) == 0) ws.red[tid >> 6] = lim;
    __syncthreads();
    double tl = 0;
    for (int w = 0; w < (nt >> 6); ++w) tl = fmax(tl, ws.red[w]);
    if (done) return;
    if (res) { for (int e = tid; e < nc * nc; e += nt) W[e] = resl[(e / nc) * ldl + (e % nc)]; }
    else { for (int e = tid; e < nc * nc; e += nt) W[e] = W1[e]; }
    if (wpk3) {
        const int NT = (nc + 15) >> 4, KCH = (16 * NT + 31) >> 5;
        for (int idx = tid; idx < KCH * NT * 64; idx += nt) {
            const int lane = idx & 63, tile = idx >> 6, u = tile % NT, kc = tile / NT;
            const int comp = 16 * u + (lane & 15), k0 = 32 * kc + 8 * (lane >> 4);
            f32x8 x;
#pragma unroll
            for (int e = 0; e < 8; ++e)
                x[e] = (comp < nc && k0 + e < nc) ? (float)(res ? resl[comp * ldl + k0 + e] : W1[comp * nc + k0 + e]) : 0.f;
            bf16x8 h, m, l;
            split3(x, h, m, l);
            wpk3[(tile * 3 + 0) * 64 + lane] = h;
            wpk3[(tile * 3 + 1) * 64 + lane] = m;
            wpk3[(tile * 3 + 2) * 64 + lane] = l;
        }
    }
    if (tid == 0 && (tl < tol)) { state[0] = 1; state[1] = iter + 1; }
    if (tid == 0 && progress) {
        if (tl < tol) __hip_atomic_store(progress, iter + 1, __ATOMIC_RELAXED, __HIP_MEMORY_SCOPE_SYSTEM);
        __hip_atomic_store(progress + 1, iter + 1, __ATOMIC_RELAXED, __HIP_MEMORY_SCOPE_SYSTEM);
    }
}

__global__ void k_dscal(double* x, int64_t count, double alpha) {
    const int64_t e = blockIdx.x * (int64_t)blockDim.x + threadIdx.x;
    if (e < count) x[e] *= alpha;
}
__global__ void k_daxpy(int64_t count, double alpha, const double* x, double* y) {
    const int64_t e = blockIdx.x * (int64_t)blockDim.x + threadIdx.x;
    if (e < count) y[e] += alpha * x[e];
}
__global__ void k_dvec(int mode, const double* x, double* y, int64_t count, double thr) {
    const int64_t e = blockIdx.x * (int64_t)blockDim.x + threadIdx.x;
    if (e >= count) return;
    if (mode == 0) y[e] = sqrt(fmax(x[e], 0.0));
    else if (mode == 2) y[e] = x[e] * x[e];
    else y[e] = (x[e] > thr * x[0] && x[e] > 0.0) ? 1.0 / x[e] : 0.0;
}
__global__ void k_sigma_inv(const double* __restrict__ lam, double* __restrict__ sig, double* __restrict__ inv, int64_t count, double thr) {
    const int64_t e = blockIdx.x * (int64_t)blockDim.x + threadIdx.x;
    if (e >= count) return;
    const double s = sqrt(fmax(lam[e], 0.0)), s0 = sqrt(fmax(lam[0], 0.0));
    sig[e] = s;
    inv[e] = (s > thr * s0 && s > 0.0) ? 1.0 / s : 0.0;
}
template <class T>
__global__ __launch_bounds__(256) void k_components_out(const double* __restrict__ Bt, int64_t ldb, const double* __restrict__ Uh,
                                                        int64_t ldu, const double* __restrict__ lam, double thr, int64_t d, int L,
                                                        int64_t k, T* __restrict__ comp) {
    __shared__ double sB[64][65];
    __shared__ double sU[64][16];
    const int tid = threadIdx.x, ti = tid & 15, tj = tid >> 4;
    const int64_t i0 = (int64_t)blockIdx.x * 64, j0 = (int64_t)blockIdx.y * 16;
    double acc[4] = {0.0, 0.0, 0.0, 0.0};
    for (int l0 = 0; l0 < L; l0 += 64) {
        double vb[16], vu[4];
#pragma unroll
        for (int u = 0; u < 16; ++u) {
            const int r = (tid >> 6) + 4 * u, l = l0 + (tid & 63);
            vb[u] = (i0 + r < d && l < L) ? Bt[(i0 + r) * ldb + l] : 0.0;
        }
#pragma unroll
        for (int u = 0; u < 4; ++u) {
            const int l = l0 + (tid >> 4) + 16 * u;
            vu[u] = (l < L && j0 + ti < k) ? Uh[(int64_t)l * ldu + j0 + ti] : 0.0;
        }
        __syncthreads();
#pragma unroll
        for (int u = 0; u < 16; ++u) sB[(tid >> 6) + 4 * u][tid & 63] = vb[u];
#pragma unroll
        for (int u = 0; u < 4; ++u) sU[(tid >> 4) + 16 * u][ti] = vu[u];
        __syncthreads();
#pragma unroll 8
        for (int l = 0; l < 64; ++l) {
            const double u = sU[l][tj];
#pragma unroll
            for (int r = 0; r < 4; ++r) acc[r] += sB[ti + 16 * r][l] * u;
        }
    }
    const int64_t j = j0 + tj;
    if (j < k) {
        const double s = sqrt(fmax(lam[j], 0.0)), s0 = sqrt(fmax(lam[0], 0.0));
        const double inv = (s > thr * s0 && s > 0.0) ? 1.0 / s : 0.0;
#pragma unroll
        for (int r = 0; r < 4; ++r) {
            const int64_t i = i0 + ti + 16 * r;
            if (i < d) comp[j * d + i] = (T)(acc[r] * inv);
        }
    }
}
__global__ void k_scale_pad_cols(const double* __restrict__ V, int64_t ldv, const double* __restrict__ inv, int64_t rows, int64_t r,
                                 int64_t rp, double* __restrict__ P) {
    const int64_t e = (int64_t)blockIdx.x * blockDim.x + threadIdx.x;
    if (e >= rows * rp) return;
    const int64_t i = e / rp, j = e - i * rp;
    P[e] = j < r ? V[i * ldv + j] * inv[j] : 0.0;
}
template <class T>
__global__ __launch_bounds__(256) void k_transpose_out(const double* __restrict__ V, int64_t ldv, int64_t d, int64_t k, T* __restrict__ comp) {
    __shared__ double tile[32][33];
    const int tx = threadIdx.x & 31, ty = threadIdx.x >> 5;
    const int64_t i0 = (int64_t)blockIdx.x * 32, j0 = (int64_t)blockIdx.y * 32;
#pragma unroll
    for (int u = 0; u < 4; ++u) {
        const int64_t i = i0 + ty + 8 * u, j = j0 + tx;
        tile[ty + 8 * u][tx] = (i < d && j < k) ? V[i * ldv + j] : 0.0;
    }
    __syncthreads();
#pragma unroll
    for (int u = 0; u < 4; ++u) {
        const int64_t j = j0 + ty + 8 * u, i = i0 + tx;
        if (j < k && i < d) comp[j * d + i] = (T)tile[tx][ty + 8 * u];
    }
}
template <class T>
__global__ __launch_bounds__(256) void k_colmean_final(const double* __restrict__ part, const double* __restrict__ part_lo, int64_t nparts,
                                                       int64_t w, int64_t d, double inv_n, double n_total, double* __restrict__ mu64,
                                                       T* __restrict__ muT) {
    __shared__ double red[32][9], redc[32][9];
    const int e = threadIdx.x & 7, pl = threadIdx.x >> 3;
    const int64_t j = (int64_t)blockIdx.x * 8 + e;
    const bool pairs = sizeof(T) == 8 && part_lo;
    double acc = 0, lo = 0;
    if (j < w) {
        if (pairs) {
            for (int64_t p = pl; p < nparts; p += 32) { two_sum_acc(acc, lo, part[p * w + j]); lo += part_lo[p * w + j]; }
        } else {
            for (int64_t p = pl; p < nparts; p += 32) acc += part[p * w + j];
        }
    }
    red[pl][e] = acc; redc[pl][e] = lo;
    __syncthreads();
    if (pl == 0 && j < w) {
        double t = 0;
        if (pairs) {
            double c = 0;
#pragma unroll
            for (int k = 0; k < 32; ++k) { two_sum_acc(t, c, red[k][e]); c += redc[k][e]; }
            if (j < d) {
                const double q = t / n_total;
                t = q + (fma(-q, n_total, t) + c) / n_total;
                muT[j] = (T)t;
// ... 80 lines not shown
```

petal-decomposition_amd/csrc/kernels/k_gemm_split_k1.inc:

```
typedef __bf16 bf16x8 __attribute__((ext_vector_type(8)));
typedef float f32x8 __attribute__((ext_vector_type(8)));
typedef __bf16 bf16x2 __attribute__((ext_vector_type(2)));
typedef float f32x2 __attribute__((ext_vector_type(2)));
typedef unsigned u32x4 __attribute__((ext_vector_type(4)));
__device__ __forceinline__ unsigned cvt_pk_bf16(float a, float b) {
    return __builtin_bit_cast(unsigned, __builtin_convertvector(f32x2{a, b}, bf16x2));
}
#ifndef PETAL_STEER_PIECES
#define PETAL_STEER_PIECES 4
#endif
#ifndef PETAL_SPLIT_DOT2
#define PETAL_SPLIT_DOT2 1
#endif
__device__ __forceinline__ void sub_pk_bf16(float& x0, float& x1, unsigned pk) {
#if PETAL_SPLIT_DOT2
    unsigned c0u, c1u;
    asm("s_mov_b32 %0, 0xbf80" : "=s"(c0u));
    asm("s_mov_b32 %0, 0xbf800000" : "=s"(c1u));
    x0 = __builtin_amdgcn_fdot2_f32_bf16(__builtin_bit_cast(bf16x2, pk), __builtin_bit_cast(bf16x2, c0u), x0, false);
    x1 = __builtin_amdgcn_fdot2_f32_bf16(__builtin_bit_cast(bf16x2, pk), __builtin_bit_cast(bf16x2, c1u), x1, false);
#else
    x0 -= __uint_as_float(pk << 16);
    x1 -= __uint_as_float(pk & 0xffff0000u);
#endif
}
__device__ __forceinline__ void split3(const f32x8 x, bf16x8& h, bf16x8& m, bf16x8& l) {
    u32x4 hh, mm, ll;
#pragma unroll
    for (int e = 0; e < 4; ++e) {
        float r0 = x[2 * e], r1 = x[2 * e + 1];
        hh[e] = cvt_pk_bf16(r0, r1);
        sub_pk_bf16(r0, r1, hh[e]);
        mm[e] = cvt_pk_bf16(r0, r1);
        sub_pk_bf16(r0, r1, mm[e]);
        ll[e] = cvt_pk_bf16(r0, r1);
    }
    h = __builtin_bit_cast(bf16x8, hh);
    m = __builtin_bit_cast(bf16x8, mm);
    l = __builtin_bit_cast(bf16x8, ll);
}
__device__ __forceinline__ void split2(const f32x8 x, bf16x8& h, bf16x8& m) {
    u32x4 hh, mm;
#pragma unroll
    for (int e = 0; e < 4; ++e) {
        float r0 = x[2 * e], r1 = x[2 * e + 1];
        hh[e] = cvt_pk_bf16(r0, r1);
        sub_pk_bf16(r0, r1, hh[e]);
        mm[e] = cvt_pk_bf16(r0, r1);
    }
    h = __builtin_bit_cast(bf16x8, hh);
    m = __builtin_bit_cast(bf16x8, mm);
}
__global__ __launch_bounds__(256) void k_pack_p3(const double* __restrict__ P, int64_t K, int64_t N, int64_t ldp,
                                                 bf16x8* __restrict__ out, int NTtot, int64_t total) {
    const int64_t idx = (int64_t)blockIdx.x * 256 + threadIdx.x;
    if (idx >= total) return;
    const int lane = (int)(idx & 63);
    const int64_t tile = idx >> 6;
    const int nt = (int)(tile % NTtot);
    const int64_t c = tile / NTtot;
    const int64_t col = 16 * nt + (lane & 15), k0 = 32 * c + 8 * (lane >> 4);
    f32x8 x;
#pragma unroll
    for (int e = 0; e < 8; ++e) x[e] = (k0 + e < K && col < N) ? (float)P[(k0 + e) * ldp + col] : 0.f;
    bf16x8 h, m, l;
    split3(x, h, m, l);
    out[(tile * 3 + 0) * 64 + lane] = h;
    out[(tile * 3 + 1) * 64 + lane] = m;
    out[(tile * 3 + 2) * 64 + lane] = l;
}
#ifndef PETAL_XP3_RT
#define PETAL_XP3_RT 4
#define PETAL_XP3_DEPTH 1
#define PETAL_XP3_OCC 2
#endif
template <int RT, int NT, int DEPTH, bool CENTER, int WVK = 4, int OCC = PETAL_XP3_OCC, int NPL = 3, bool X2 = false>
__global__ __launch_bounds__(64 * WVK, OCC) void k_xp3(const float* __restrict__ X, int64_t n, int K, int64_t ldx,
                                                            const float* __restrict__ mu, const bf16x8* __restrict__ Ppk3,
                                                            int NTtot, int nt0, int N, const float* __restrict__ bias,
                                                            float* __restrict__ Z, int64_t ldz, double* __restrict__ amax,
                                                            int64_t am_ld) {
    constexpr int PITEMS = NT * 64 * NPL;
    constexpr int NTHR = 64 * WVK;
    constexpr int PI = (PITEMS + NTHR - 1) / NTHR;
    extern __shared__ __attribute__((aligned(16))) unsigned char sm_xp3[];
    bf16x8* sP = reinterpret_cast<bf16x8*>(sm_xp3);
    float* sMu = reinterpret_cast<float*>(sm_xp3 + sizeof(bf16x8) * 2 * PITEMS);
    const int tid = threadIdx.x, lane = tid & 63, wave = tid >> 6;
    const int i = lane & 15, q = lane >> 4;
    const int64_t row0 = ((int64_t)blockIdx.x * WVK + wave) * (16 * RT);
    const int nchunk = (K + 31) >> 5;
    if (CENTER)
        for (int k = tid; k < 32 * nchunk; k += NTHR) sMu[k] = k < K ? mu[k] : 0.f;
    f32x4 acc[RT][NT];
#pragma unroll
    for (int t = 0; t < RT; ++t)
#pragma unroll
        for (int u = 0; u < NT; ++u) acc[t][u] = f32x4{0.f, 0.f, 0.f, 0.f};
    const float* xrow[RT];
#pragma unroll
    for (int t = 0; t < RT; ++t) {
        const int64_t r = row0 + 16 * t + i;
        xrow[t] = X + (r < n ? r : (n - 1)) * ldx + 8 * q;
    }
    const bf16x8* psrc = Ppk3 + (int64_t)nt0 * 192;
    int poff[PI];
#pragma unroll
    for (int it = 0; it < PI; ++it) {
        const int j = tid + NTHR * it;
        poff[it] = NPL == 3 ? j : (j / (64 * NPL)) * 192 + (j % (64 * NPL));
    }
    auto load_a = [&](int c, f32x8(&a)[RT]) {
        const bool in = 32 * c + 8 * q < K;
#pragma unroll
        for (int t = 0; t < RT; ++t) {
            f32x4 lo = f32x4{0.f, 0.f, 0.f, 0.f}, hi = lo;
            if (in) { lo = ld_stream(xrow[t] + 32 * c); hi = ld_stream(xrow[t] + 32 * c + 4); }
            a[t] = f32x8{lo[0], lo[1], lo[2], lo[3], hi[0], hi[1], hi[2], hi[3]};
        }
    };
    auto load_p = [&](int c, bf16x8(&pn)[PI]) {
#pragma unroll
// ... 161 lines not shown
```

petal-decomposition_amd/csrc/kernels/k_generic.inc:

```
template <class T>
__global__ void k_pack_strided(const T* __restrict__ src, int64_t n, int64_t d, int64_t rs, int64_t cs, T* __restrict__ dst,
                               int64_t ld, int64_t dpad) {
    const int64_t j = blockIdx.y * (int64_t)blockDim.x + threadIdx.x;
    const int64_t i = blockIdx.x;
    if (j >= dpad) return;
    dst[i * ld + j] = j < d ? src[i * rs + j * cs] : T(0);
}
template <class T>
__global__ void k_unpack_strided(const T* __restrict__ src, int64_t n, int64_t d, int64_t ld, T* __restrict__ dst, int64_t rs,
                                 int64_t cs) {
    const int64_t j = blockIdx.y * (int64_t)blockDim.x + threadIdx.x;
    const int64_t i = blockIdx.x;
    if (j >= d) return;
    dst[i * rs + j * cs] = src[i * ld + j];
}
template <class T>
__global__ __launch_bounds__(256) void k_pack_flat(const T* __restrict__ src, int64_t n, int64_t d, int64_t rs, int64_t cs, T* __restrict__ dst,
                                                   int64_t ld, int64_t dpad) {
    const int64_t total = n * dpad;
#pragma unroll
    for (int u = 0; u < 4; ++u) {
        const int64_t e = ((int64_t)blockIdx.x * 4 + u) * 256 + threadIdx.x;
        if (e >= total) return;
        const int64_t i = e / dpad, j = e - i * dpad;
// ... 91 lines not shown
    if (SQ) redq[ry][cx] = (q0 + q1) + (q2 + q3);
    __syncthreads();
    if (ry == 0 && j < d) {
        const int64_t w = SQ ? 2 * d : d;
        part[(int64_t)blockIdx.x * w + j] = (red[0][cx] + red[1][cx]) + (red[2][cx] + red[3][cx]);
        if (SQ) part[(int64_t)blockIdx.x * w + d + j] = (redq[0][cx] + redq[1][cx]) + (redq[2][cx] + redq[3][cx]);
    }
}
template <class T>
__global__ __launch_bounds__(256) void k_absmax_part2(const T* __restrict__ U, int64_t n, int64_t L, int64_t ldu, int64_t rows,
                                                      double* __restrict__ pmax, double* __restrict__ pidx,
                                                      double* __restrict__ psgn) {
    __shared__ double rm[SCAN_RY][64], ri[SCAN_RY][64], rs[SCAN_RY][64];
    const int cx = threadIdx.x & 63, ry = threadIdx.x >> 6;
    const int64_t j = blockIdx.y * (int64_t)64 + cx;
    const int64_t r0 = (int64_t)blockIdx.x * rows, r1 = min(n, r0 + rows);
    double best = -1.0, bi = INFINITY, bs = 1.0;
    if (j < L) {
#pragma unroll 4
        for (int64_t i = r0 + ry; i < r1; i += SCAN_RY) {
            const double v = (double)U[i * ldu + j], a = fabs(v);
            if (a > best) { best = a; bi = (double)i; bs = signbit(v) ? -1.0 : 1.0; }
        }
    }
    rm[ry][cx] = best; ri[ry][cx] = bi; rs[ry][cx] = bs;
    __syncthreads();
    if (ry == 0 && j < L) {
#pragma unroll
        for (int k = 1; k < SCAN_RY; ++k)
            if (rm[k][cx] > best || (rm[k][cx] == best && ri[k][cx] < bi)) { best = rm[k][cx]; bi = ri[k][cx]; bs = rs[k][cx]; }
        const int64_t o = (int64_t)blockIdx.x * L + j;
        pmax[o] = best; pidx[o] = bi; psgn[o] = bs;
    }
}
template <class TP>
__global__ __launch_bounds__(256) void k_sum_parts2(const TP* __restrict__ part, int64_t nparts, int64_t count,
                                                    double* __restrict__ out, int64_t N, int64_t ldc, bool accumulate) {
    __shared__ double red[8][33];
    const int tx = threadIdx.x & 31, ty = threadIdx.x >> 5;
    const int64_t e = (int64_t)blockIdx.x * 32 + tx;
    double s = 0;
    if (e < count)
        for (int64_t p = ty; p < nparts; p += 8) s += (double)part[p * count + e];
    red[ty][tx] = s;
    __syncthreads();
    if (ty == 0 && e < count) {
        double t = 0;
#pragma unroll
        for (int k = 0; k < 8; ++k) t += red[k][tx];
        double* o = out + (e / N) * ldc + (e % N);
        *o = accumulate ? *o + t : t;
    }
}
__global__ __launch_bounds__(256) void k_sum_parts4(const float* __restrict__ part, int64_t nparts, int64_t count,
                                                    double* __restrict__ out, int64_t N, int64_t ldc) {
    __shared__ double red[3][64][3];
    const int lane = threadIdx.x & 63, wave = threadIdx.x >> 6;
    const int64_t e = ((int64_t)blockIdx.x * 64 + lane) * 2;
    double s0 = 0, s1 = 0;
    if (e < count) {
        const float* src = part + e;
        int64_t p = wave;
        for (; p + 28 < nparts; p += 32) {
            f32x2 v[8];
#pragma unroll
            for (int k = 0; k < 8; ++k) v[k] = *reinterpret_cast<const f32x2*>(src + (p + 4 * k) * count);
#pragma unroll
            for (int k = 0; k < 8; ++k) { s0 += (double)v[k][0]; s1 += (double)v[k][1]; }
        }
        for (; p < nparts; p += 4) {
            const f32x2 v = *reinterpret_cast<const f32x2*>(src + p * count);
            s0 += (double)v[0]; s1 += (double)v[1];
        }
    }
    if (wave > 0) { red[wave - 1][lane][0] = s0; red[wave - 1][lane][1] = s1; }
    __syncthreads();
    if (wave == 0 && e < count) {
#pragma unroll
        for (int w = 0; w < 3; ++w) { s0 += red[w][lane][0]; s1 += red[w][lane][1]; }
        double* o = out + (e / N) * ldc + (e % N);
        o[0] = s0; o[1] = s1;
    }
}
__global__ __launch_bounds__(256) void k_add_scalar_parts(const double* __restrict__ part, int64_t nparts, double* __restrict__ out) {
    __shared__ double red[256];
    double s = 0;
    for (int64_t p = threadIdx.x; p < nparts; p += 256) s += part[p];
    red[threadIdx.x] = s;
    __syncthreads();
    for (int st = 128; st > 0; st >>= 1) {
        if ((int)threadIdx.x < st) red[threadIdx.x] += red[threadIdx.x + st];
        __syncthreads();
    }
    if (threadIdx.x == 0) out[0] += red[0];
}

template <class T>
__global__ void k_xp_simple(const T* __restrict__ X, int64_t n, int64_t K, int64_t ldx, const T* __restrict__ mu,
                            const double* __restrict__ P, int64_t N, int64_t ldp, const T* __restrict__ bias,
                            T* __restrict__ Z, int64_t ldz, double* __restrict__ ss_part) {
    const int64_t j = blockIdx.y * (int64_t)blockDim.x + threadIdx.x;
    const int64_t i = blockIdx.x;
    double acc = 0, ss = 0;
    const bool want_ss = ss_part != nullptr && blockIdx.y == 0 && threadIdx.x == 0;
    if (j < N || want_ss) {
        for (int64_t k = 0; k < K; ++k) {
            T xv = X[i * ldx + k];
            if (mu) xv = xv - mu[k];
            const double a = (double)xv;
            if (j < N) acc += a * (sizeof(T) == 4 ? (double)(float)P[k * ldp + j] : P[k * ldp + j]);
            ss += a * a;
        }
    }
    if (j < N) Z[i * ldz + j] = (T)(acc + (bias ? (double)bias[j] : 0.0));
    if (want_ss) ss_part[i] = ss;
}

constexpr int ATB_S_ROWS = 256;
template <class T>
__global__ void k_atb_simple(const T* __restrict__ A, int64_t lda, int64_t M, const T* __restrict__ muA,
                             const T* __restrict__ B, int64_t ldb, int64_t N, const T* __restrict__ muB, int64_t n,
                             double* __restrict__ part) {
    const int64_t j = blockIdx.y * (int64_t)blockDim.x + threadIdx.x;
    const int64_t m = blockIdx.z * (int64_t)blockDim.y + threadIdx.y;
    if (j >= N || m >= M) return;
    const int64_t r0 = (int64_t)blockIdx.x * ATB_S_ROWS, r1 = min(n, r0 + ATB_S_ROWS);
    const T ma = muA ? muA[m] : T(0), mb = muB ? muB[j] : T(0);
    double s = 0;
    for (int64_t i = r0; i < r1; ++i) s += (double)(T)(A[i * lda + m] - ma) * (double)(T)(B[i * ldb + j] - mb);
    part[((int64_t)blockIdx.x * M + m) * N + j] = s;
}
__global__ __launch_bounds__(64) void k_absmax_final(const double* __restrict__ pmax, const double* __restrict__ pidx,
                                                     const double* __restrict__ psgn, int64_t nparts, int64_t L,
                                                     int64_t row_offset, double* __restrict__ omax, double* __restrict__ oidx,
// ... 35 lines not shown
```

petal-decomposition_amd/csrc/kernels/k_smallmat.inc:

```
__global__ __launch_bounds__(256) void k_dgemm(bool ta, bool tb, int64_t M, int64_t N, int64_t K, double alpha,
                                               const double* __restrict__ A, int64_t lda, const double* __restrict__ B, int64_t ldb,
                                               double beta, double* __restrict__ C, int64_t ldc, int64_t kchunk,
                                               double* __restrict__ part, const double* __restrict__ colscale,
                                               bf16x8* __restrict__ pk3, int NTtot) {
    constexpr int BK = 32;
    __shared__ double sa[16][BK + 1], sb[BK][17];
    const int tx = threadIdx.x, ty = threadIdx.y;
    const int64_t i0 = (int64_t)blockIdx.y * 16, j0 = (int64_t)blockIdx.x * 16;
    const int64_t kbeg = (int64_t)blockIdx.z * kchunk;
    if (K > kbeg + kchunk) K = kbeg + kchunk;
    double acc = 0;
    for (int64_t k0 = kbeg; k0 < K; k0 += BK) {
#pragma unroll
        for (int h = 0; h < 2; ++h) {
            if (ta) {
                const int kk = ty + 16 * h;
                const int64_t k = k0 + kk, i = i0 + tx;
                sa[tx][kk] = (i < M && k < K) ? A[k * lda + i] : 0.0;
            } else {
                const int kk = tx + 16 * h;
                const int64_t k = k0 + kk, i = i0 + ty;
                sa[ty][kk] = (i < M && k < K) ? A[i * lda + k] : 0.0;
            }
            if (tb) {
// ... 97 lines not shown
        cf64x4 pt = cf64x4{0.0, 0.0, 0.0, 0.0};
#pragma unroll
        for (int r = 0; r < 4; ++r) pt = __builtin_amdgcn_mfma_f64_16x16x4f64(cur[I][r], X[I][r], pt, 0, 0, 0);
#pragma unroll
        for (int J = I + 1; J < NB; ++J) {
#pragma unroll
            for (int r = 0; r < 4; ++r)
                X[J] = __builtin_amdgcn_mfma_f64_16x16x4f64(-cur[J][r], pt[r], X[J], 0, 0, 0);
        }
#pragma unroll
        for (int r = 0; r < 4; ++r) sP[li * ldsp + 16 * I + lk + 4 * r] = pt[r];
        __builtin_amdgcn_sched_barrier(0);
    }
    __syncthreads();
    if (P_out && !P2)
        for (int e = lane; e < 16 * M; e += 64) {
            const int r = e / M, c = e - r * M;
            P_out[(i0 + r) * ldpo + c] = sP[r * ldsp + c];
        }
    if (pk3) {
        for (int idx = lane; idx < 2 * M; idx += 64) {
            const int g = idx / M, col = idx - g * M;
            bf16x8 h, m, l;
            if (P2) {
#pragma unroll
                for (int e = 0; e < 8; ++e) {
                    double hd, md;
                    two_plane_f64(sP[(8 * g + e) * ldsp + col], hd, md);
                    h[e] = (__bf16)(float)hd;
                    m[e] = (__bf16)(float)md;
                    if (P_out) P_out[(i0 + 8 * g + e) * ldpo + col] = hd + md;
                }
            } else {
                f32x8 x;
#pragma unroll
                for (int e = 0; e < 8; ++e) x[e] = (float)sP[(8 * g + e) * ldsp + col];
                split3(x, h, m, l);
            }
            const int64_t c = i0 >> 5, tile = c * NTtot + (col >> 4);
            const int ln = (col & 15) + 16 * (int)(((i0 & 31) + 8 * g) >> 3);
            pk3[(tile * 3 + 0) * 64 + ln] = h;
            pk3[(tile * 3 + 1) * 64 + ln] = m;
            if (!P2) pk3[(tile * 3 + 2) * 64 + ln] = l;
            if ((K & 31) == 16 && i0 + 16 == K) {
                bf16x8 z; for (int e = 0; e < 8; ++e) z[e] = (__bf16)0.0f;
#pragma unroll
                for (int pl = 0; pl < (P2 ? 2 : 3); ++pl) pk3[(tile * 3 + pl) * 64 + ln + 32] = z;
            }
        }
    }
}

template <int NB>
__global__ __launch_bounds__(64) void k_trsm_left_pack(const double* __restrict__ RT, int64_t ldt, const double* __restrict__ B, int64_t ldb,
                                                       double* __restrict__ X_out, int64_t ldxo, bf16x8* __restrict__ pk3, int NTtot) {
    constexpr int M = 16 * NB, MP = (M + 31) / 32 * 32;
    __shared__ double sX[MP * 17];
    const int lane = threadIdx.x, li = lane & 15, lk = lane >> 4;
    const int64_t j0 = (int64_t)blockIdx.x * 16;
    cf64x4 X[NB];
#pragma unroll
    for (int I = 0; I < NB; ++I)
#pragma unroll
        for (int r = 0; r < 4; ++r) X[I][r] = B[(int64_t)(16 * I + lk + 4 * r) * ldb + j0 + li];
    cf64x4 rt[2][NB];
    auto load_row = [&](int I, cf64x4(&dst)[NB]) {
        const double* rrow = RT + (int64_t)(16 * I + li) * ldt + lk;
#pragma unroll
        for (int K = 0; K < NB; ++K)
            if (K >= I) {
#pragma unroll
                for (int r = 0; r < 4; ++r) dst[K][r] = rrow[16 * K + 4 * r];
            }
    };
    load_row(NB - 1, rt[(NB - 1) & 1]);
#pragma unroll
    for (int I = NB - 1; I >= 0; --I) {
        if (I > 0) load_row(I - 1, rt[(I - 1) & 1]);
        const cf64x4(&cur)[NB] = rt[I & 1];
        cf64x4 acc = X[I];
#pragma unroll
        for (int K = I + 1; K < NB; ++K) {
#pragma unroll
            for (int r = 0; r < 4; ++r) acc = __builtin_amdgcn_mfma_f64_16x16x4f64(-cur[K][r], X[K][r], acc, 0, 0, 0);
        }
        cf64x4 xi = cf64x4{0.0, 0.0, 0.0, 0.0};
#pragma unroll
        for (int r = 0; r < 4; ++r) xi = __builtin_amdgcn_mfma_f64_16x16x4f64(cur[I][r], acc[r], xi, 0, 0, 0);
        X[I] = xi;
#pragma unroll
        for (int r = 0; r < 4; ++r) {
            sX[(16 * I + lk + 4 * r) * 17 + li] = xi[r];
            if (X_out) X_out[(int64_t)(16 * I + lk + 4 * r) * ldxo + j0 + li] = xi[r];
        }
        __builtin_amdgcn_sched_barrier(0);
    }
    if (MP > M)
        for (int e = lane; e < (MP - M) * 17; e += 64) sX[M * 17 + e] = 0.0;
    __syncthreads();
    if (pk3) {
#pragma unroll
        for (int cc = 0; cc < MP / 32; ++cc) {
            f32x8 x;
#pragma unroll
            for (int e = 0; e < 8; ++e) x[e] = (float)sX[(32 * cc + 8 * lk + e) * 17 + li];
            bf16x8 h, m, l;
            split3(x, h, m, l);
            const int64_t tile = (int64_t)cc * NTtot + blockIdx.x;
            pk3[(tile * 3 + 0) * 64 + lane] = h;
            pk3[(tile * 3 + 1) * 64 + lane] = m;
            pk3[(tile * 3 + 2) * 64 + lane] = l;
        }
    }
}

constexpr int CHOL_THREADS = 512;
__device__ __forceinline__ double readlane_d(double x, int l) {
    const int lo = __builtin_amdgcn_readlane(__double2loint(x), l), hi = __builtin_amdgcn_readlane(__double2hiint(x), l);
    return __hiloint2double(hi, lo);
}
__device__ __forceinline__ double fast_rsqrt_pos(double d) {
    double y = __builtin_amdgcn_rsq(d);
#pragma unroll
    for (int it = 0; it < 2; ++it) {
        const double e = fma(-d * y, y, 1.0);
        y = fma(0.5 * y, e, y);
    }
    return y;
}
__device__ __forceinline__ double bperm_d(double x, int src_lane) {
    const int lo = __builtin_amdgcn_ds_bpermute(src_lane << 2, __double2loint(x)), hi = __builtin_amdgcn_ds_bpermute(src_lane << 2, __double2hiint(x));
    return __hiloint2double(hi, lo);
}
__device__ __forceinline__ int cp(int k, int c) { return (c * (c + 1)) / 2 + k; }
typedef double cf64x4 __attribute__((ext_vector_type(4)));
__device__ __forceinline__ double ld_up(const double* P, int r, int c, int L) { return (r <= c && c < L) ? P[cp(r, c)] : 0.0; }
constexpr int CHOL2_MAXL = 140;
__host__ __device__ inline size_t chol2_lds_bytes(int L) {
    return sizeof(double) * ((size_t)L * (L + 1) + 2 * (size_t)L) + sizeof(int) * (size_t)L;
}
__device__ __forceinline__ void chol2_body(double* sm_chol, int L, double* __restrict__ T, int64_t ldt, double rel_tol,
                                           int* __restrict__ ndead_out, int Lz, int rt_form, int ncount) {
    const int tid = threadIdx.x, nt = blockDim.x;
    const int np = L * (L + 1) / 2;
    double* Rc = sm_chol;
    double* Tc = Rc + np;
    double* gd = Tc + np;
    double* rinv = gd + L;
    int* dead = reinterpret_cast<int*>(rinv + L);
    for (int e = tid; e < Lz * Lz; e += nt) {
        const int r = e / Lz, c = e - r * Lz;
        if (r >= L || c >= L) T[(int64_t)r * ldt + c] = 0.0;
    }
    __syncthreads();
#ifdef PETAL_DEBUG_COUNTERS
    long long _t0 = clock64();
#endif
    const int nb = (L + 15) / 16;
    for (int J = 0; J < nb; ++J) {
        const int jb = 16 * J;
        double gdv[16];
#pragma unroll
        for (int i = 0; i < 16; ++i) gdv[i] = (tid < 64 && jb + i < L) ? gd[jb + i] : 0.0;
        cf64x4 dacc = cf64x4{0.0, 0.0, 0.0, 0.0};
        if (jb > 0) {
            const int lane = tid & 63, li = lane & 15, lk = lane >> 4;
// ... 837 lines not shown
```

petal-decomposition_amd/csrc/ops.h:

```cpp
#pragma once
#include <cstddef>
#include <cstdint>

namespace petal {

enum DType : int { F32 = 0, F64 = 1 };
inline size_t dtype_size(int dt) { return dt == F64 ? 8 : 4; }

struct Dev;

enum Tag : int { TAG_NONE = 0, TAG_XP = 1, TAG_ATB = 2, TAG_ICA = 3, TAG_COMM = 4, TAG_POW = 5, TAG_STREAM = 6, TAG_COUNT = 7 };
struct KernelTiming {
    double ms[TAG_COUNT] = {0, 0, 0, 0, 0, 0, 0};
    int64_t launches[TAG_COUNT] = {0, 0, 0, 0, 0, 0, 0};
};

Dev*  dev_create(int device, void* stream, char* err, size_t errlen);
void  dev_destroy(Dev*);
void* dev_stream(Dev*);
void* dev_alloc(Dev*, size_t bytes);
void  dev_free(Dev*, void*);
bool  dev_live(Dev*, int64_t* blocks, int64_t* bytes);
void  dev_memset(Dev*, void* p, int v, size_t bytes);
void  dev_h2d(Dev*, void* dst, const void* src, size_t bytes);
void  dev_h2d_async(Dev*, void* dst, const void* src, size_t bytes);
void  dev_d2h(Dev*, void* dst, const void* src, size_t bytes);
void  dev_d2h_multi(Dev*, int nseg, void* const* dst, const void* const* src, const size_t* bytes);
const void* dev_h2d_view(Dev*, const void* src, size_t bytes);
const void* dev_d2h_view(Dev*, const void* src, size_t bytes);
size_t dev_view_limit(Dev*);
void  dev_d2d(Dev*, void* dst, const void* src, size_t bytes);
void  dev_copy2d(Dev*, void* dst, size_t dpitch, const void* src, size_t spitch, size_t width, size_t height, int kind);
void  dev_sync(Dev*);
void  dev_set_profiling(Dev*, int level);
enum PetalOpt {
    OPT_TWO_PLANE = 0,
    OPT_TWO_PLANE_OMEGA = 1,
    OPT_TWO_PLANE_ITERATE = 2,
    OPT_STEERING = 3,
    OPT_FUSED_PASS = 4,
    OPT_FUSED_PASS_MIN_ROWS = 5,
    OPT_VERDICT_THRESHOLD = 6,
    OPT_MEANS_FOLD_ROWS = 7,
    OPT_GRAM_SPLIT = 8,
    OPT_GRAM_SPLIT_HOOK = 9,
    OPT_D2H_KERNEL = 10,
    OPT_ROW_PAD = 11,
    OPT_EIGH_JACOBI = 12,
    OPT_POISON = 13,
    OPT_STEERING_HOOK = 15,
    OPT_COUNT = 16
};
void   dev_set_option(Dev*, int opt, double value);
double dev_option(const Dev*, int opt);
void  dev_set_gemm_mode(Dev*, int mode);
int   dev_gemm_mode(const Dev*);
void  dev_make_current(Dev*);
int   dev_push_current(Dev*);
void  dev_pop_current(Dev*, int prev);
void  dev_abort(Dev*);
void  dev_reset_timing(Dev*);
void  dev_set_tag(Dev*, int tag);
void  dev_fork(Dev*, bool after_main = true);
void  dev_fork_end(Dev*);
void  dev_join(Dev*);
void  dev_fork_abort(Dev*);
KernelTiming dev_timing(Dev*);
void* dev_span_begin(Dev*, int tag);
void  dev_span_end(Dev*, void* token);

void op_pack_strided(Dev*, int dtype, const void* src, int64_t n, int64_t d, int64_t rs, int64_t cs,
                     void* dst, int64_t ld_dst, int64_t d_pad);
void op_unpack_strided(Dev*, int dtype, const void* src, int64_t n, int64_t d, int64_t ld_src,
                       void* dst, int64_t rs, int64_t cs, const double* scale = nullptr);
void op_colsum(Dev*, int dtype, const void* X, int64_t n, int64_t d, int64_t ldx, double* out, bool with_sq = false);
void op_colmean(Dev*, int dtype, const void* X, int64_t n, int64_t d, int64_t ldx, double n_total, double* mu64, void* muT, bool with_sq);
void op_gemm_xp(Dev*, int dtype, const void* X, int64_t n, int64_t K, int64_t ldx, const void* mu,
                const double* P, int64_t N, int64_t ldp, const void* bias,
                void* Z, int64_t ldz, double* sumsq, int p_planes = 3, bool steering = false);
void op_gemm_xp_prod(Dev*, int dtype, const void* X, int64_t n, int64_t K, int64_t ldx, const void* mu,
                     const double* A, int64_t M, int64_t lda, const double* T, int64_t N, int64_t ldt,
                     double* P_out, int64_t ldpo, void* Z, int64_t ldz);
void op_gemm_xp_prod_absmax(Dev*, int dtype, const void* X, int64_t n, int64_t K, int64_t ldx, const void* mu,
                            const double* A, int64_t M, int64_t lda, const double* T, int64_t N, int64_t ldt,
                            double* P_out, int64_t ldpo, void* Z, int64_t ldz,
                            int64_t row_offset, double* absmax, double* idx, double* sign, bool store_product = true, bool a_rt = false);
void op_gemm_xp_absmax(Dev*, int dtype, const void* X, int64_t n, int64_t K, int64_t ldx, const void* mu, const double* P, int64_t N,
                       int64_t ldp, void* Z, int64_t ldz, int64_t row_offset, double* absmax, double* idx, double* sign,
                       bool store_product = true);
void op_gemm_xp_scores(Dev*, int dtype, const void* X, int64_t n, int64_t K, int64_t ldx, const void* mu, const double* P, int64_t N,
                       int64_t ldp, const void* wts, void* Z, int64_t ldz, void* st, int64_t ldst);
bool op_pca_segments(Dev*, int dtype, const void* X, int64_t ldx, int64_t d, const int64_t* offsets, int64_t nseg, int64_t k, bool centering,
                     void* comp, void* means, void* sing, void* tv, int32_t* status, void* Y);
bool op_transform_segments(Dev*, int dtype, const void* X, int64_t ldx, const int64_t* offsets, int64_t nseg, const void* comp,
                           const void* means, int64_t k, int64_t d, void* Y);
bool op_inverse_transform_segments(Dev*, int dtype, const void* Y, int64_t ldy, const int64_t* offsets, int64_t nseg, const void* comp,
                                   const void* means, int64_t k, int64_t d, void* X);
struct CsrItem { int64_t first; int32_t row, count, slot, pad; };
struct CsrSplit { int32_t row, first_slot, count, pad; };
struct CsrImage {
    int64_t rows = 0, nnz = 0;
    const int32_t* idx = nullptr;
    const void* val = nullptr;
    const CsrItem* items = nullptr;
    int64_t n_items = 0;
    const CsrSplit* splits = nullptr;
    int64_t n_splits = 0, n_slots = 0;
// ... 3 lines not shown
                 void* out, int64_t ldo);
bool op_csr_colstats(Dev*, int dtype, const CsrImage& img, double* stats);
bool op_tall_times_small(Dev*, int dtype, const void* M, int64_t rows, int64_t K, int64_t ldm, const double* S, int64_t N, int64_t lds,
                         void* out, int64_t ldo);
bool op_ipca_accumulate(Dev*, int dtype, const void* X, int64_t m, int64_t dp, int64_t ldx, const double* centre, double n_seen, double* M2,
                        double* mean);
bool op_ipca_merge(Dev*, int64_t dp, double n_a, double* M2_a, const double* mean_a, double* mean_out, double n_b, const double* M2_b,
                   const double* mean_b);
bool op_row_gram(Dev*, int dtype, const void* X, int64_t n, int64_t dp, int64_t ldx, const double* centre, double* K, int64_t ldk,
                 int64_t* chunks);
bool op_kpca_map(Dev*, int kernel, double gamma, double coef0, int degree, double* K, int64_t n, int64_t ldk, const double* diag,
                 double* rbar, double* tbar);
bool op_kernel_apply(Dev*, int dtype, const void* Xt, int64_t n, int64_t ldt, const void* Xq, int64_t m, int64_t ldq, int64_t dp,
                     const double* centre, const double* nt, int kernel, double gamma, double coef0, int degree, const double* A, int64_t lda,
                     int64_t cols, double* out, int64_t ldo);
bool op_kpca_finish(Dev*, int dtype, const double* O, int64_t ldo, int64_t m, int64_t k, const double* ra, const double* oa, double n,
                    const double* tbar, void* Y, int64_t ldy);
inline int64_t nmf_padded_k(int64_t k) { return k <= 16 ? 16 : (k <= 32 ? 32 : (k + 15) / 16 * 16); }
bool op_nmf_scan(Dev*, int dtype, const void* X, int64_t n, int64_t dp, int64_t ldx, double* out4);
bool op_nmf_pass(Dev*, int dtype, const void* X, int64_t n, int64_t dp, int64_t ldx, const double* H, const double* HHt, int64_t k, int64_t kp,
                 double* W, bool from_const, double wconst, double l1, double l2, int64_t inner, double* A, double* B);
bool op_nmf_hupdate(Dev*, int64_t kp, int64_t dp, const double* A, const double* B, double* H, double* HHt, double l1, double l2, double* dots2);
inline int64_t nmf_csr_padded_k(int64_t k) { return k <= 16 ? 16 : (k <= 32 ? 32 : 64); }
bool op_nmf_sweep_csr(Dev*, int dtype, const CsrImage& img, int64_t k, int64_t kp, const double* F, double* G, const double* S, bool from_const,
                      double gconst, double l1, double l2, int64_t inner, double* gram_dot);
bool op_nmf_gram(Dev*, const double* G, int64_t rows, int64_t kp, const double* dots, double* gram_dot);
bool op_nmf_valscan(Dev*, int dtype, const void* val, int64_t nnz, double* out4);
bool op_nmf_kl_sweep_csr(Dev*, int dtype, const CsrImage& img, int64_t k, int64_t kp, const double* F, double* G, const double* csum,
                         bool from_const, double gconst, double l1, double l2, int64_t inner, double* colsum_term);
bool op_nmf_kl_colsum(Dev*, const double* G, int64_t rows, int64_t kp, const double* terms, double* colsum_term);
bool op_nmf_kl_vsum(Dev*, int dtype, const void* val, int64_t nnz, double* out1);
bool op_nmf_kl_pass(Dev*, int dtype, const void* X, int64_t n, int64_t dp, int64_t ldx, const double* H, const double* rsum, int64_t k, int64_t kp,
                    double* W, bool from_const, double wconst, double l1, double l2, int64_t inner, double* A, double* cts);
bool op_nmf_kl_hrule(Dev*, int64_t kp, int64_t dp, const double* A, const double* colsum, double* H, double l1, double l2);
bool op_nmf_kl_rowsum(Dev*, int64_t kp, int64_t dp, const double* H, double* out);
bool op_nmf_cd_pass(Dev*, int dtype, const void* X, int64_t n, int64_t dp, int64_t ldx, const double* H, const double* HHt, int64_t k, int64_t kp,
                    double* W, bool from_zero, double l1, double l2, int64_t inner, double* A, double* B, double* viol);
bool op_nmf_cd_hupdate(Dev*, int64_t k, int64_t kp, int64_t dp, const double* A, const double* B, double* H, double* HHt, double l1, double l2,
                       double* dots2, double* viol1);
bool op_csr_densify(Dev*, int dtype, const CsrImage& img, void* out, int64_t cols, int64_t ldo);
void op_rebase_xp(Dev*, int dtype, const void* X, int64_t n, int64_t K, int64_t ldx, const void* mu, const double* G, int64_t L,
                  int64_t ldg, double rel_tol, int* ndead, const double* A, int64_t M, int64_t lda, double* T, int64_t ldt,
                  double* P_out, int64_t ldpo, void* Z, int64_t ldz, int p_planes = 2, bool steering = false);
bool op_power_pass_applies(Dev*, int dtype, const void* X, int64_t n, int64_t K, int64_t ldx, const void* mu, int64_t N);
bool op_power_pass(Dev*, int dtype, const void* X, int64_t n, int64_t K, int64_t ldx, const void* mu, const double* P, int64_t N, int64_t ldp,
                   void* Z, int64_t ldz, double* Y, int64_t ldy, bool steering = false);
bool op_power_pass_means(Dev*, int dtype, const void* X, int64_t n, int64_t K, int64_t d, int64_t ldx, double n_total, const double* P,
                         int64_t N, int64_t ldp, int64_t L, double* Y, int64_t ldy, double* mu64, void* muT, double* ssq_scratch, double* tv);
bool op_rebase_power_pass(Dev*, int dtype, const void* X, int64_t n, int64_t K, int64_t ldx, const void* mu, const double* G, int64_t L,
                          int64_t ldg, double rel_tol, int* ndead, const double* A, int64_t M, int64_t lda, double* T, int64_t ldt,
                          double* P_out, int64_t ldpo, void* Z, int64_t ldz, double* Y, int64_t ldy, bool steering = false);
void op_tail_verdict(Dev*, const double* lam, int64_t L, int64_t k, const double* mu_sq, int64_t dp, int64_t d, double n_total,
                     const double* tv, double eps2, double thr, int* flag2);
void op_gemm_atb(Dev*, int dtype, const void* A, int64_t lda, int64_t M, const void* muA,
                 const void* B, int64_t ldb, int64_t N, const void* muB, int64_t n,
                 double* C, int64_t ldc, bool precise = false, bool steering = false);
bool op_gram_split(Dev*, const void* X, int64_t n, int64_t d, int64_t dp, int64_t ldx, const void* mu, double* C, int64_t ldc,
                   double* mu64_fold = nullptr, double n_total = 0.0);
void op_col_absmax(Dev*, int dtype, const void* U, int64_t n, int64_t L, int64_t ldu, int64_t row_offset,
                   double* absmax, double* idx, double* sign);
void op_flip_key(Dev*, const double* triple, double* key, int64_t L, const int* flag = nullptr);
constexpr double VERDICT_TAIL = 1.0, VERDICT_EIG = 2.0, VERDICT_PIVOT = 3.0;
constexpr double verdict_code(const int* w) {
    return w[0] != 0 ? VERDICT_PIVOT : (w[1] != 0 ? VERDICT_TAIL : (w[2] != 0 ? VERDICT_EIG : 0.0));
}
void op_scale_cols(Dev*, int dtype, void* A, int64_t n, int64_t L, int64_t lda, const double* s);
void op_logcosh_rows(Dev*, int dtype, const void* X, int64_t r, int64_t c, int64_t ldx, void* G, int64_t ldg, double* gp);

void op_ica_prepare(Dev*, int dtype, const void* X1T, int64_t n, int64_t nc, int64_t ld);
void op_ica_step(Dev*, int dtype, const void* X1T, int64_t n, int64_t nc, int64_t ld,
                 const double* W, double* GX_gp , const int* state);
void op_ica_step_g(Dev*, int dtype, const void* X1T, int64_t n, int64_t nc, int64_t ld,
                   const double* W, double* GX_gp , const int* state, int contrast);
void op_ica_tail(Dev*, int64_t nc, double n_total, double* W, const double* GX_gp, int mode, double tol,
                 int* state, int iter, int* progress = nullptr);
volatile int* dev_host_progress(Dev*);
void op_symdecorr(Dev*, int64_t nc, const double* Win, double* Wout, int mode, int* zero2 = nullptr);

void op_dgemm(Dev*, bool ta, bool tb, int64_t M, int64_t N, int64_t K, double alpha,
              const double* A, int64_t lda, const double* B, int64_t ldb, double beta, double* C, int64_t ldc,
              const double* colscale = nullptr);
void op_sigma_inv(Dev*, const double* lam, double* sig, double* inv, int64_t count, double thr);
void op_scale_pad_cols(Dev*, const double* V, int64_t ldv, const double* inv, int64_t rows, int64_t r, int64_t rp, double* P);
void op_transpose_out(Dev*, int dtype, const double* V, int64_t ldv, int64_t d, int64_t k, void* comp);
void op_components_out(Dev*, int dtype, const double* Bt, int64_t ldb, const double* Uh, int64_t ldu, const double* lam, double thr,
                       int64_t d, int64_t L, int64_t k, void* comp);
bool op_chol_rt(Dev*, int dtype, int64_t n, const double* G, int64_t L, int64_t ldg, double* T, int64_t ldt, double rel_tol, int* ndead,
                int64_t Lz, int64_t ndead_cols);
void op_trsm_right(Dev*, const double* A, int64_t rows, int64_t lda, const double* RT, int64_t M, int64_t ldt, double* out, int64_t ldo);
void op_chol_inv(Dev*, const double* G, int64_t L, int64_t ldg, double* T, int64_t ldt, double rel_tol, int* ndead = nullptr,
                 int64_t Lz = 0, int64_t ndead_cols = 0);
void op_eigh(Dev*, double* A, int64_t L, int64_t lda, double* V, int64_t ldv, double* w, double tol_rel = 1e-15,
             bool clustered = false, int64_t Lz = 0, int64_t ncheck = 0, int* verdict = nullptr, bool verdict_fresh = false,
             double gap_tol_override = 0.0);
void op_ritz_residual(Dev*, const double* CV, int64_t ldc, const double* Vr, int64_t ldv, int64_t rows, int64_t nc, const double* theta,
                      const int* flag, double* out3, double* w_out = nullptr, const int* flag2 = nullptr);
void op_whiten_k(Dev*, const double* U, int64_t ldu, const double* lam, int64_t rows, int64_t nc, int64_t ncp, double scale,
                 double* KT, double* KTs);
void op_jacobi_svd_rows(Dev*, double* A, int64_t L, int64_t lda, double* U, int64_t ldu, double* s_inv, int* nonconv = nullptr);
void op_refill_zero_cols(Dev*, double* Y, int64_t rows, int64_t cols, int64_t ldy, const double* Src, int64_t lds);
void op_dscal(Dev*, double* x, int64_t count, double alpha);
void op_daxpy(Dev*, int64_t count, double alpha, const double* x, double* y);
void op_dvec(Dev*, int mode, const double* x, double* y, int64_t count, double thr);
void op_dscale_cols(Dev*, double* A, int64_t M, int64_t N, int64_t lda, const double* s);
void op_cvt_from_f64(Dev*, int dtype, void* dst, const double* src, int64_t count);
void op_cvt_to_f64(Dev*, int dtype, double* dst, const void* src, int64_t count);
// ... 5 lines not shown
```

Baseline: 111.2 million.

## Merge small-stage tail kernels and fold-means reductions into fewer launches

Adds a merged small-stage consumer path that runs the tail verdict, the components output and the triangular solve with operand-plane packing in one launch, then feeds the pre-packed planes into the absmax GEMM. It also merges the means-fold partial-sum reduction with a column extraction, and lowers the default row threshold for means folding. The aim is to cut kernel-launch and small-kernel overhead in the randomized PCA tail. Two new options allow reverting to the old multi-launch sequence.

New measurement: 109.7 million. -1.4%, worse.

```diff
diff --git a/dev/fold_crossover.py b/dev/fold_crossover.py
--- /dev/null
+++ b/dev/fold_crossover.py
@@ -0,0 +1,119 @@
+import argparse
+import json
+import os
+import sys
+import time
+
+import numpy as np
+
+ROOT = os.path.dirname(os.path.dirname(os.path.abspath(__file__)))
+sys.path.insert(0, ROOT)
+
+
+def main():
+    ap = argparse.ArgumentParser()
+    ap.add_argument("--pairs", type=int, default=7)
+    ap.add_argument("--fits", type=int, default=200)
+    ap.add_argument("--rows", type=int, nargs="+", default=[25000, 50000, 100000, 200000])
+    ap.add_argument("--merge-rows", type=int, nargs="*", default=[100000, 1000000])
+    ap.add_argument("--out", default=os.path.join(ROOT, "profiles", "means_fold_crossover.json"))
+    args = ap.parse_args()
+
+    import torch
+    import petal_decomposition_amd as petal
+    from synth_data import synth_pca
+
+    dev = torch.device("cuda", 0)
+    torch.cuda.set_device(0)
+    ctx = petal.Context(0, stream=torch.cuda.current_stream(dev).cuda_stream)
+    ctx.set_profiling(True)
+    d, k, n_iter = 512, 64, 5
+    omega = np.random.default_rng(3).standard_normal((d, k + 10)).astype(np.float32)
+
+    def sample(model, x):
+        torch.cuda.synchronize(dev)
+        t0 = time.perf_counter()
+        for _ in range(args.fits):
+            model.fit(x, omega=omega)
+        torch.cuda.synchronize(dev)
+        return (time.perf_counter() - t0) / args.fits * 1e3
+
+    def run_arms(x, arms):
+        model = petal.RandomizedPca(k, ctx=ctx, n_iter=n_iter)
+        ms = {name: [] for name in arms}
+        folded = {}
+        for name, opts in arms.items():
+            for o, v in opts.items():
+                ctx.set_option(o, v)
+            for _ in range(10):
+                model.fit(x, omega=omega)
+            folded[name] = int(ctx.stats()["means_folded"])
+        t_end = time.perf_counter() + 0.25
+        while time.perf_counter() < t_end:
+            model.fit(x, omega=omega)
+        for _ in range(args.pairs):
+            for name, opts in arms.items():
+                for o, v in opts.items():
+                    ctx.set_option(o, v)
+                ms[name].append(round(sample(model, x), 4))
+        return ms, folded
+
+    def summary(v):
+        return {"ms": v, "median": round(float(np.median(v)), 4), "spread": round(max(v) - min(v), 4)}
+
+    table = {"shape": {"d": d, "k": k, "n_iter": n_iter}, "fits_per_sample": args.fits, "samples_per_arm": args.pairs, "rows": {}}
+    keep = {o: ctx.get_option(o) for o in ("means_fold_rows", "fold_merged", "tail_merged")}
+    try:
+        for n in args.rows:
+            x = torch.from_numpy(synth_pca(n, d, k, seed=2, dtype=np.float32)).to(dev)
+            ctx.set_option("tail_merged", keep["tail_merged"])
+            ms, folded = run_arms(x, {"means_pass": {"means_fold_rows": -1, "fold_merged": 1},
+                                      "fold": {"means_fold_rows": 0, "fold_merged": 1},
+                                      "fold_previous_launches": {"means_fold_rows": 0, "fold_merged": 0}})
+            assert folded == {"means_pass": 0, "fold": 1, "fold_previous_launches": 1}, folded
+            row = {name: summary(v) for name, v in ms.items()}
+            gain = row["means_pass"]["median"] - row["fold"]["median"]
+            row["fold_gain_ms"] = round(gain, 4)
+            row["fold_wins"] = bool(gain > row["fold"]["spread"])
+            table["rows"][str(n)] = row
+            print(n, json.dumps(row), flush=True)
+            if n == 100000:
+                ctx.set_option("means_fold_rows", keep["means_fold_rows"])
+                ctx.set_option("fold_merged", keep["fold_merged"])
+                ms, _ = run_arms(x, {"three_launches": {"tail_merged": 0}, "one_launch": {"tail_merged": 1}})
+                tail = {name: summary(v) for name, v in ms.items()}
+                tail["gain_ms"] = round(tail["three_launches"]["median"] - tail["one_launch"]["median"], 4)
+                table["tail_at_100000"] = tail
+                print("tail", json.dumps(tail), flush=True)
+            del x
+        for n in args.merge_rows:
+            x = torch.from_numpy(synth_pca(n, d, k, seed=2, dtype=np.float32)).to(dev)
+            ctx.set_option("means_fold_rows", keep["means_fold_rows"])
+            ms, folded = run_arms(x, {"previous_launches": {"fold_merged": 0, "tail_merged": 0}, "merged": {"fold_merged": 1, "tail_merged": 1}})
+            row = {name: summary(v) for name, v in ms.items()}
+            row["means_folded"] = folded["merged"]
+            row["gain_ms"] = round(row["previous_launches"]["median"] - row["merged"]["median"], 4)
+            table.setdefault("merges_at", {})[str(n)] = row
+            print("merges", n, json.dumps(row), flush=True)
+            del x
+    finally:
+        for o, v in keep.items():
+            ctx.set_option(o, v)
+    rows = sorted(int(n) for n in table["rows"])
+    first = None
+    for n in reversed(rows):
+        if not table["rows"][str(n)]["fold_wins"]:
+            break
+        first = n
+    table["fold_wins_from"] = first
+    table["threshold"] = None if first is None else 1 << (int(first).bit_length() - 1)
+    os.makedirs(os.path.dirname(args.out), exist_ok=True)
+    with open(args.out, "w") as f:
+        json.dump(table, f, indent=1)
+        f.write("\n")
+    print(json.dumps({"fold_wins_from": first, "threshold": table["threshold"]}))
+    ctx.close()
+
+
+if __name__ == "__main__":
+    main()
diff --git a/include/petal_hip.h b/include/petal_hip.h
--- a/include/petal_hip.h
+++ b/include/petal_hip.h
@@ -88,6 +88,8 @@
 #define PETAL_OPT_POISON 13
 #define PETAL_OPT_FORCE_COLLECTIVE 14
 #define PETAL_OPT_STEERING_HOOK 15
+#define PETAL_OPT_FOLD_MERGED 40
+#define PETAL_OPT_TAIL_MERGED 41
 int         petal_ctx_set_option(petal_ctx* ctx, int option, double value);
 int         petal_ctx_get_option(const petal_ctx* ctx, int option, double* value);
 int         petal_get_stats(const petal_ctx* ctx, petal_stats* out);
diff --git a/petal-decomposition_amd/__init__.py b/petal-decomposition_amd/__init__.py
--- a/petal-decomposition_amd/__init__.py
+++ b/petal-decomposition_amd/__init__.py
@@ -21,7 +21,8 @@
            "ipca_fallback": 32,
            "pca_dual": 33, "pca_dual_fallback": 34,
            "kpca_fallback": 36,
-           "nmf_fallback": 38}
+           "nmf_fallback": 38,
+           "fold_merged": 40, "tail_merged": 41}
 ICA_TEXTBOOK, ICA_REFERENCE_LITERAL = 0, 1
 ICA_CONTRAST_LOGCOSH, ICA_CONTRAST_EXP, ICA_CONTRAST_CUBE = 0, 16, 32
 ICA_SEMANTICS_MASK, ICA_CONTRAST_MASK = 15, 240
diff --git a/petal-decomposition_amd/csrc/algo.cpp b/petal-decomposition_amd/csrc/algo.cpp
--- a/petal-decomposition_amd/csrc/algo.cpp
+++ b/petal-decomposition_amd/csrc/algo.cpp
@@ -684,7 +684,25 @@
         op_dgemm(c.dev, true, false, LP, LP, dp, 1.0, Bt.f64(), LP, Bt.f64(), LP, 0.0, S.f64(), LP);
         if (!a.robust && !a.jacobi) op_eigh(c.dev, S.f64(), L, LP, Uh.f64(), LP, lam, dt == F32 ? 1e-8 : 1e-15, false, LP, std::max<int64_t>(k, 1), neig);
         else op_eigh(c.dev, S.f64(), L, LP, Uh.f64(), LP, lam, dt == F32 ? 1e-8 : 1e-15, true, LP);
-        if (!a.robust && !a.exact && two_plane_applies)
+        const bool verdict = !a.robust && !a.exact && two_plane_applies;
+        if (slot_flip) {
+            SmallStageConsumers s{};
+            s.lam = lam; s.Uh = Uh.f64(); s.ldu = LP; s.L = L; s.LP = LP;
+            s.verdict = verdict; s.mu_sq = (tv_from_sq && !tv_direct) ? mu64 : nullptr; s.tv = tv_direct ? mu64 + dp : tvp;
+            s.n_total = in.ri.n_total; s.eps2 = steered ? 4e-6 * 1.2 : 4e-6; s.verdict_thr = p2_thr; s.flag2 = ndead;
+            s.Bt = Bt.f64(); s.ldb = LP; s.comp_thr = dt == F32 ? 1e-7 : 1e-12; s.d = d; s.dp = dp; s.k = k; s.comp = comp_dev;
+            s.RT = T.f64(); s.ldt = LP; s.rt_form = t_rt; s.N = kp; s.P_out = M2.f64(); s.ldpo = LP;
+            void* planes = nullptr;
+            if (op_small_stage_consumers(c.dev, dt, n, s, &planes)) {
+                dev_set_tag(c.dev, TAG_STREAM);
+                op_gemm_xp_packed_absmax(c.dev, dt, Usrc, n, LP, LP, M2.f64(), kp, LP, planes, Ubuf, LP, in.ri.row_offset, flip, flip + kp,
+                                         flip + 2 * kp, y_out != nullptr);
+                dev_set_tag(c.dev, TAG_NONE);
+                Uout = Ubuf;
+                return;
+            }
+        }
+        if (verdict)
             op_tail_verdict(c.dev, lam, L, std::max<int64_t>(k, 1), (tv_from_sq && !tv_direct) ? mu64 : nullptr, dp, d, in.ri.n_total,
                             tv_direct ? mu64 + dp : tvp, steered ? 4e-6 * 1.2 : 4e-6, p2_thr, ndead);
         op_components_out(c.dev, dt, Bt.f64(), LP, Uh.f64(), LP, lam, dt == F32 ? 1e-7 : 1e-12, d, L, k, comp_dev);
@@ -786,6 +804,18 @@
 
 __attribute__((weak)) bool op_row_gram(Dev*, int, const void*, int64_t, int64_t, int64_t, const double*, double*, int64_t, int64_t*) {
     return false;
+}
+__attribute__((weak)) void dev_set_launch_merge(Dev*, int which, bool) {
+    if (which < 0 || which >= MERGE_COUNT) throw std::invalid_argument("unknown ctx option");
+}
+__attribute__((weak)) bool dev_launch_merge(const Dev*, int which) {
+    if (which < 0 || which >= MERGE_COUNT) throw std::invalid_argument("unknown ctx option");
+    return false;
+}
+__attribute__((weak)) bool op_small_stage_consumers(Dev*, int, int64_t, const SmallStageConsumers&, void**) { return false; }
+__attribute__((weak)) void op_gemm_xp_packed_absmax(Dev*, int, const void*, int64_t, int64_t, int64_t, const double*, int64_t, int64_t, void*, void*,
+                                                    int64_t, int64_t, double*, double*, double*, bool) {
+    throw std::logic_error("op_gemm_xp_packed_absmax: no device layer packs operand planes ahead of the product");
 }
 namespace {
 constexpr int64_t PCA_DUAL_MIN_D = 2048;
diff --git a/petal-decomposition_amd/csrc/api.cpp b/petal-decomposition_amd/csrc/api.cpp
--- a/petal-decomposition_amd/csrc/api.cpp
+++ b/petal-decomposition_amd/csrc/api.cpp
@@ -150,6 +150,10 @@
         if (option == PETAL_OPT_PCA_DUAL_FALLBACK) { ctx->pca_dual_fallback = value != 0; return; }
         if (option == PETAL_OPT_KPCA_FALLBACK) { ctx->kpca_fallback = value != 0; return; }
         if (option == PETAL_OPT_NMF_FALLBACK) { ctx->nmf_fallback = value != 0; return; }
+        if (option == PETAL_OPT_FOLD_MERGED || option == PETAL_OPT_TAIL_MERGED) {
+            dev_set_launch_merge(ctx->dev, option - PETAL_OPT_FOLD_MERGED, value != 0);
+            return;
+        }
         if (option < 0 || option >= OPT_COUNT || !(value == value)) invalid_input("unknown ctx option or NaN value");
         dev_set_option(ctx->dev, option, value);
     });
@@ -163,6 +167,10 @@
     if (option == PETAL_OPT_PCA_DUAL_FALLBACK) { *value = ctx->pca_dual_fallback ? 1.0 : 0.0; return PETAL_OK; }
     if (option == PETAL_OPT_KPCA_FALLBACK) { *value = ctx->kpca_fallback ? 1.0 : 0.0; return PETAL_OK; }
     if (option == PETAL_OPT_NMF_FALLBACK) { *value = ctx->nmf_fallback ? 1.0 : 0.0; return PETAL_OK; }
+    if (option == PETAL_OPT_FOLD_MERGED || option == PETAL_OPT_TAIL_MERGED) {
+        *value = dev_launch_merge(ctx->dev, option - PETAL_OPT_FOLD_MERGED) ? 1.0 : 0.0;
+        return PETAL_OK;
+    }
     if (option < 0 || option >= OPT_COUNT) return PETAL_INVALID_INPUT;
     *value = dev_option(ctx->dev, option);
     return PETAL_OK;
diff --git a/petal-decomposition_amd/csrc/hip_ops.hip b/petal-decomposition_amd/csrc/hip_ops.hip
--- a/petal-decomposition_amd/csrc/hip_ops.hip
+++ b/petal-decomposition_amd/csrc/hip_ops.hip
@@ -79,6 +79,8 @@
     char* pin_dev = nullptr;
     bool d2h_kernel = true;
     double opt[OPT_COUNT] = {};
+    bool fold_merged = true;
+    bool tail_merged = true;
     size_t pin_cap = 0, pin_used = 0;
     struct Pend { void* dst; size_t off, bytes; };
     std::vector<Pend> pend;
@@ -104,7 +106,7 @@
     d->opt[OPT_FUSED_PASS] = on("PETAL_NO_POW3") ? 0 : 1;
     d->opt[OPT_FUSED_PASS_MIN_ROWS] = num("PETAL_POW3_MIN_ROWS", 8192);
     d->opt[OPT_VERDICT_THRESHOLD] = num("PETAL_P2_VERDICT_THR", 4e-6);
-    d->opt[OPT_MEANS_FOLD_ROWS] = on("PETAL_NO_MEANS_FOLD") ? -1 : num("PETAL_MEANS_FOLD_ROWS", 200000);
+    d->opt[OPT_MEANS_FOLD_ROWS] = on("PETAL_NO_MEANS_FOLD") ? -1 : num("PETAL_MEANS_FOLD_ROWS", 131072);
     d->opt[OPT_GRAM_SPLIT] = on("PETAL_NO_GRAM3") ? 0 : 1;
     d->opt[OPT_GRAM_SPLIT_HOOK] = on("PETAL_GRAM_SPLIT") ? 1 : 0;
     d->opt[OPT_D2H_KERNEL] = on("PETAL_D2H_MEMCPY") ? 0 : 1;
@@ -113,6 +115,18 @@
     d->opt[OPT_POISON] = on("PETAL_POISON") ? 1 : 0;
     d->opt[OPT_STEERING_HOOK] = 0;
     d->d2h_kernel = d->opt[OPT_D2H_KERNEL] != 0;
+    d->fold_merged = !on("PETAL_NO_FOLD_MERGE");
+    d->tail_merged = !on("PETAL_NO_TAIL_MERGE");
+}
+void dev_set_launch_merge(Dev* d, int which, bool merged) {
+    if (which == MERGE_FOLD) d->fold_merged = merged;
+    else if (which == MERGE_TAIL) d->tail_merged = merged;
+    else throw std::invalid_argument("unknown ctx option");
+}
+bool dev_launch_merge(const Dev* d, int which) {
+    if (which == MERGE_FOLD) return d->fold_merged;
+    if (which == MERGE_TAIL) return d->tail_merged;
+    throw std::invalid_argument("unknown ctx option");
 }
 void dev_set_option(Dev* d, int opt, double value) {
     if (opt < 0 || opt >= OPT_COUNT) throw std::invalid_argument("unknown ctx option");
diff --git a/petal-decomposition_amd/csrc/kernels/host_gemm.inc b/petal-decomposition_amd/csrc/kernels/host_gemm.inc
--- a/petal-decomposition_amd/csrc/kernels/host_gemm.inc
+++ b/petal-decomposition_amd/csrc/kernels/host_gemm.inc
@@ -128,7 +128,7 @@
 static void gemm_xp_impl(Dev* d, int dt, const void* X, int64_t n, int64_t K, int64_t ldx, const void* mu, const double* P, int64_t N,
                          int64_t ldp, const void* bias, void* Z, int64_t ldz, double* sumsq, const double* prod_A, int64_t prod_M,
                          int64_t prod_lda, double* prod_out, int64_t prod_ldo, int prod_rt, const AbsmaxReq* am = nullptr,
-                         bool p2_hint = false, bool steering = false);
+                         bool p2_hint = false, bool steering = false, bf16x8* packed = nullptr);
 void op_gemm_xp(Dev* d, int dt, const void* X, int64_t n, int64_t K, int64_t ldx, const void* mu, const double* P, int64_t N,
                 int64_t ldp, const void* bias, void* Z, int64_t ldz, double* sumsq, int p_planes, bool steering) {
     gemm_xp_impl(d, dt, X, n, K, ldx, mu, P, N, ldp, bias, Z, ldz, sumsq, nullptr, 0, 0, nullptr, 0, false, nullptr, p_planes == 2, steering);
@@ -196,8 +196,10 @@
 }
 static void gemm_xp_impl(Dev* d, int dt, const void* X, int64_t n, int64_t K, int64_t ldx, const void* mu, const double* P, int64_t N,
                          int64_t ldp, const void* bias, void* Z, int64_t ldz, double* sumsq, const double* prod_A, int64_t prod_M,
-                         int64_t prod_lda, double* prod_out, int64_t prod_ldo, int prod_rt, const AbsmaxReq* am, bool p2_hint, bool steering) {
-    if (n == 0 || N == 0) return;
+                         int64_t prod_lda, double* prod_out, int64_t prod_ldo, int prod_rt, const AbsmaxReq* am, bool p2_hint, bool steering,
+                         bf16x8* packed) {
+    if (packed && !(dt == F32 && gemm_split_product(d) && !sumsq && !prod_A)) throw std::logic_error("gemm_xp_impl: packed planes outside the split-product path");
+    if (n == 0 || N == 0) { if (packed) dev_free(d, packed); return; }
     const bool mfma = dt == F32 && K % 16 == 0 && K > 0 && ldx % 4 == 0 && aligned16(X) && (!mu || aligned16(mu)) && n >= 64 &&
                       K < (1 << 24) && N < (1 << 24) && N % 16 == 0 && ldz % 4 == 0 && aligned16(Z) && (!bias || aligned16(bias));
     const bool mfma64 = dt == F64 && K % 8 == 0 && K > 0 && ldx % 2 == 0 && aligned16(X) && (!mu || aligned16(mu)) && n >= 64 &&
@@ -263,7 +265,7 @@
     const int NTtot = cdiv(N, 16);
     if (gemm_split_product(d) && !sumsq) {
         const int64_t nch = (K + 31) / 32, total = nch * NTtot * 64;
-        bf16x8* Ppk3 = (bf16x8*)dev_alloc(d, sizeof(bf16x8) * total * 3);
+        bf16x8* Ppk3 = packed ? packed : (bf16x8*)dev_alloc(d, sizeof(bf16x8) * total * 3);
         const bool no_p2 = !opt_on(d, OPT_TWO_PLANE);
         const bool no_p2_it = no_p2 || !opt_on(d, OPT_TWO_PLANE_ITERATE), no_p2_om = no_p2 || !opt_on(d, OPT_TWO_PLANE_OMEGA);
         const bool p2 = p2_hint && ((prod_A && prod_rt && !no_p2_it) || (!prod_A && !no_p2_om)) && !am;
@@ -298,7 +300,7 @@
             hipLaunchKernelGGL(k_dgemm, dim3(cdiv(N, 16), cdiv(K, 16)), dim3(16, 16), 0, d->stream, false, false, K, N, prod_M, 1.0,
                                prod_A, prod_lda, P, ldp, 0.0, prod_out, prod_ldo, prod_M, (double*)nullptr, (const double*)nullptr,
                                Ppk3, NTtot);
-        } else {
+        } else if (!packed) {
             hipLaunchKernelGGL(k_pack_p3, dim3(cdiv(total, 256)), dim3(256), 0, d->stream, P, K, N, ldp, Ppk3, NTtot, total);
         }
         launch_check();
@@ -789,10 +791,9 @@
     hipLaunchKernelGGL(k_flip_key, dim3(cdiv(L + 1, 256)), dim3(256), 0, d->stream, triple, key, L, flag);
     launch_check();
 }
-__global__ __launch_bounds__(256) void k_tail_verdict(const double* __restrict__ lam, int L, int k, const double* __restrict__ mu_sq, int dp,
-                                                       int d, double n_total, const double* __restrict__ tvp, double eps2, double thr,
-                                                       int* __restrict__ flag2) {
-    __shared__ double red[256];
+__device__ __forceinline__ void tail_verdict_block(const double* __restrict__ lam, int L, int k, const double* __restrict__ mu_sq, int dp,
+                                                   int d, double n_total, const double* __restrict__ tvp, double eps2, double thr,
+                                                   int* __restrict__ flag2, double* __restrict__ red) {
     const int tid = threadIdx.x;
     double s = 0;
     if (mu_sq) for (int j = tid; j < d; j += 256) s += fmax(0.0, mu_sq[dp + j] - n_total * mu_sq[j] * mu_sq[j]);
@@ -819,6 +820,75 @@
     }
     if (__syncthreads_or(bad) && tid == 0) flag2[1] = 1;
 }
+__global__ __launch_bounds__(256) void k_tail_verdict(const double* __restrict__ lam, int L, int k, const double* __restrict__ mu_sq, int dp,
+                                                       int d, double n_total, const double* __restrict__ tvp, double eps2, double thr,
+                                                       int* __restrict__ flag2) {
+    __shared__ double red[256];
+    tail_verdict_block(lam, L, k, mu_sq, dp, d, n_total, tvp, eps2, thr, flag2, red);
+}
+struct TailArgs {
+    const double *lam, *Uh; int64_t ldu; int L;
+    const double* Bt; int64_t ldb; double cthr; int64_t d, k; float* comp; int gx, ncomp;
+    const double* RT; int64_t ldt; double* P_out; int64_t ldpo; bf16x8* pk3; int NTtot, ntrsm;
+    const double *mu_sq, *tvp; int vk, dp; double n_total, eps2, vthr; int* flag2;
+};
+template <int NB>
+__global__ __launch_bounds__(256) void k_small_stage_consumers(const TailArgs a) {
+    constexpr int MP = (16 * NB + 31) / 32 * 32;
+    constexpr int LDS = COMPONENTS_LDS > MP * 17 ? COMPONENTS_LDS : MP * 17;
+    __shared__ double sm[LDS];
+    const int b = blockIdx.x;
+    if (b < a.ncomp) {
+        components_out_block<float>(a.Bt, a.ldb, a.Uh, a.ldu, a.lam, a.cthr, a.d, a.L, a.k, a.comp, b % a.gx, b / a.gx,
+                                    reinterpret_cast<double(*)[65]>(sm), reinterpret_cast<double(*)[16]>(sm + 64 * 65));
+    } else if (b < a.ncomp + a.ntrsm) {
+        if (threadIdx.x < 64) trsm_left_solve<NB>(a.RT, a.ldt, a.Uh, a.ldu, a.P_out, a.ldpo, b - a.ncomp, sm);
+        __syncthreads();
+        if (threadIdx.x < 64) trsm_left_planes<NB>(sm, a.pk3, a.NTtot, b - a.ncomp);
+    } else {
+        tail_verdict_block(a.lam, a.L, a.vk, a.mu_sq, a.dp, (int)a.d, a.n_total, a.tvp, a.eps2, a.vthr, a.flag2, sm);
+    }
+}
+bool op_small_stage_consumers(Dev* d, int dt, int64_t n, const SmallStageConsumers& s, void** planes) {
+    const int64_t K = s.LP, N = s.N;
+    const bool fused = dt == F32 && gemm_split_product(d) && n >= 64 && n < (int64_t(1) << 31) && K % 16 == 0 && K > 0 && K <= TRSM_MAXM &&
+                       N % 16 == 0 && N > 0 && N <= K && s.P_out != nullptr && s.rt_form;
+    if (!d->tail_merged || !fused || s.k <= 0 || s.d <= 0 || s.L <= 0 || s.L > K || !planes) return false;
+    const int NTtot = (int)(N / 16);
+    const int64_t nch = (K + 31) / 32, total = nch * NTtot * 64;
+    bf16x8* Ppk3 = (bf16x8*)dev_alloc(d, sizeof(bf16x8) * total * 3);
+    TailArgs a;
+    a.lam = s.lam; a.Uh = s.Uh; a.ldu = s.ldu; a.L = (int)s.L;
+    a.Bt = s.Bt; a.ldb = s.ldb; a.cthr = s.comp_thr; a.d = s.d; a.k = s.k; a.comp = (float*)s.comp;
+    a.gx = cdiv(s.d, 64); a.ncomp = a.gx * cdiv(s.k, 16);
+    a.RT = s.RT; a.ldt = s.ldt; a.P_out = s.P_out; a.ldpo = s.ldpo; a.pk3 = Ppk3; a.NTtot = NTtot; a.ntrsm = NTtot;
+    a.mu_sq = s.mu_sq; a.tvp = s.tv; a.vk = (int)s.k; a.dp = (int)s.dp; a.n_total = s.n_total; a.eps2 = s.eps2; a.vthr = s.verdict_thr; a.flag2 = s.flag2;
+    const dim3 grid((unsigned)(a.ncomp + a.ntrsm + (s.verdict ? 1 : 0)));
+    switch ((int)(K / 16)) {
+#define PETAL_TAIL_CASE(NB) case NB: hipLaunchKernelGGL((k_small_stage_consumers<NB>), grid, dim3(256), 0, d->stream, a); break
+        PETAL_TAIL_CASE(1); PETAL_TAIL_CASE(2); PETAL_TAIL_CASE(3); PETAL_TAIL_CASE(4); PETAL_TAIL_CASE(5);
+        PETAL_TAIL_CASE(6); PETAL_TAIL_CASE(7); PETAL_TAIL_CASE(8); PETAL_TAIL_CASE(9);
+#undef PETAL_TAIL_CASE
+        default: dev_free(d, Ppk3); return false;
+    }
+    launch_check();
+    *planes = Ppk3;
+    return true;
+}
+void op_gemm_xp_packed_absmax(Dev* d, int dt, const void* X, int64_t n, int64_t K, int64_t ldx, const double* P, int64_t N, int64_t ldp,
+                              void* planes, void* Z, int64_t ldz, int64_t row_offset, double* absmax, double* idx, double* sign,
+                              bool store_product) {
+    const bool fused = dt == F32 && gemm_split_product(d) && n >= 64 && K % 16 == 0 && K > 0 && N % 16 == 0 && N > 0 && ldx % 4 == 0 &&
+                       aligned16(X) && ldz % 4 == 0 && aligned16(Z) && K < (1 << 24) && N < (1 << 24) && n < (int64_t(1) << 31) && planes;
+    if (!fused) {
+        if (planes) dev_free(d, planes);
+        op_gemm_xp_absmax(d, dt, X, n, K, ldx, nullptr, P, N, ldp, Z, ldz, row_offset, absmax, idx, sign, store_product);
+        return;
+    }
+    const AbsmaxReq am{N, row_offset, absmax, idx, sign};
+    gemm_xp_impl(d, dt, X, n, K, ldx, nullptr, P, N, ldp, nullptr, store_product ? Z : nullptr, ldz, nullptr, nullptr, 0, 0, nullptr, 0, false, &am,
+                 false, false, (bf16x8*)planes);
+}
 void op_tail_verdict(Dev* d, const double* lam, int64_t L, int64_t k, const double* mu_sq, int64_t dp, int64_t dd, double n_total,
                      const double* tv, double eps2, double thr, int* flag2) {
     if (L <= 0 || k <= 0) return;
diff --git a/petal-decomposition_amd/csrc/kernels/host_pow3_eigh.inc b/petal-decomposition_amd/csrc/kernels/host_pow3_eigh.inc
--- a/petal-decomposition_amd/csrc/kernels/host_pow3_eigh.inc
+++ b/petal-decomposition_amd/csrc/kernels/host_pow3_eigh.inc
@@ -7,8 +7,16 @@
 bool op_power_pass_applies(Dev* d, int dt, const void* X, int64_t n, int64_t K, int64_t ldx, const void* mu, int64_t N) {
     return pow3_ok(d, dt, X, n, K, ldx, mu, N, nullptr, 0);
 }
+static void launch_pow3_combine(Dev* d, const float* part, int grid, int64_t K, int64_t N, double* Y, int64_t ldy, double* sums_col) {
+    if (sums_col)
+        hipLaunchKernelGGL(k_sum_parts4_col, dim3(cdiv(K * N, 128)), dim3(256), 0, d->stream, part, (int64_t)grid, (int64_t)K * N, Y, N, ldy, N - 1, sums_col);
+    else
+        hipLaunchKernelGGL(k_sum_parts4, dim3(cdiv(K * N, 128)), dim3(256), 0, d->stream, part, (int64_t)grid, (int64_t)K * N, Y, N, ldy);
+    launch_check();
+}
 static void launch_pow3(Dev* d, const float* X, int64_t n, int64_t K, int64_t ldx, const float* mu, const bf16x8* Ppk3, int64_t N, float* Z, int64_t ldz,
-                        double* Y, int64_t ldy, double** ssq_parts_out = nullptr, int* nparts_out = nullptr, bool steering = false) {
+                        double* Y, int64_t ldy, double** ssq_parts_out = nullptr, int* nparts_out = nullptr, bool steering = false,
+                        double* sums_col = nullptr) {
     const bool ssq_out = ssq_parts_out != nullptr;
     const bool no_fast = !opt_on(d, OPT_STEERING);
     if (steering && !no_fast && !Z) {
@@ -43,8 +51,7 @@
         }
 #undef POW3F_NT
 #undef POW3F_GO
-        hipLaunchKernelGGL(k_sum_parts4, dim3(cdiv(K * N, 128)), dim3(256), 0, d->stream, part, (int64_t)grid, (int64_t)K * N, Y, N, ldy);
-        launch_check();
+        launch_pow3_combine(d, part, grid, K, N, Y, ldy, sums_col);
         dev_free(d, part);
         if (ssq_parts_out) { *ssq_parts_out = ssq_part; *nparts_out = grid * 8; }
         return;
@@ -85,8 +92,7 @@
     }
 #undef POW3_NT
 #undef POW3_GO
-    hipLaunchKernelGGL(k_sum_parts4, dim3(cdiv(K * N, 128)), dim3(256), 0, d->stream, part, (int64_t)grid, (int64_t)K * N, Y, N, ldy);
-    launch_check();
+    launch_pow3_combine(d, part, grid, K, N, Y, ldy, sums_col);
     dev_free(d, part);
     if (ssq_parts_out) { *ssq_parts_out = ssq_part; *nparts_out = grid * 8; }
 }
@@ -149,14 +155,155 @@
         }
     }
 }
+__global__ __launch_bounds__(1024) void k_mean_fix_col(double* __restrict__ Y, int K, int d, int64_t ldy, int L, double n_total,
+                                                       const double* __restrict__ sums, const double* __restrict__ P, int64_t ldp,
+                                                       double* __restrict__ mu64, float* __restrict__ muT,
+                                                       const double* __restrict__ ssq_part, int nparts, double* __restrict__ tv) {
+    __shared__ double sd[512];
+    __shared__ double sr[1024];
+    __shared__ double st[16];
+    const int tid = threadIdx.x;
+    const int jj = tid & 15, fl = tid >> 4, j = blockIdx.x * 16 + jj;
+    const bool last = blockIdx.x + 1 == gridDim.x, col = !last && j < L;
+    double pv[8], yv[8];
+#pragma unroll
+    for (int u = 0; u < 8; ++u) {
+        const int f = fl + 64 * u;
+        pv[u] = (col && f < K) ? P[(int64_t)f * ldp + j] : 0.0;
+        yv[u] = (col && f < K) ? Y[(int64_t)f * ldy + j] : 0.0;
+    }
+    for (int f = tid; f < K; f += 1024) sd[f] = f < d ? sums[f] / n_total : 0.0;
+    __syncthreads();
+    double acc = 0;
+    auto two_plane = [](double v) {
+        auto bf = [](float f) {
+            unsigned u = __float_as_uint(f);
+            u = (u + 0x7fffu + ((u >> 16) & 1u)) & 0xffff0000u;
+            return __uint_as_float(u);
+        };
+        const float f = (float)v, h = bf(f), m = bf(f - h);
+        return (double)h + (double)m;
+    };
+    if (col) {
+#pragma unroll
+        for (int u = 0; u < 8; ++u)
+            if (fl + 64 * u < K) acc += sd[fl + 64 * u] * two_plane(pv[u]);
+    }
+    sr[fl * 16 + jj] = acc;
+    __syncthreads();
+    if (tid < 16) {
+        double t = 0;
+        for (int g = 0; g < 64; ++g) t += sr[g * 16 + tid];
+        st[tid] = t;
+    }
+    __syncthreads();
+    if (col) {
+#pragma unroll
+        for (int u = 0; u < 8; ++u) {
+            const int f = fl + 64 * u;
+            if (f < K) Y[(int64_t)f * ldy + j] = yv[u] - n_total * sd[f] * st[jj];
+        }
+    }
+    if (last) {
+        double q = 0, sp = 0;
+        if (tid < 256) {
+            for (int f = tid; f < K; f += 256) q += sd[f] * sd[f];
+            for (int e = tid; e < nparts; e += 256) sp += ssq_part[e];
+        }
+        __syncthreads();
+        if (tid < 256) sr[tid] = q;
+        __syncthreads();
+        for (int h = 128; h > 0; h >>= 1) { if (tid < h) sr[tid] += sr[tid + h]; __syncthreads(); }
+        const double q2 = sr[0];
+        __syncthreads();
+        if (tid < 256) sr[tid] = sp;
+        __syncthreads();
+        for (int h = 128; h > 0; h >>= 1) { if (tid < h) sr[tid] += sr[tid + h]; __syncthreads(); }
+        if (tid == 0) tv[0] = fmax(sr[0] - n_total * q2, 0.0);
+        for (int f = tid; f < K; f += 1024) {
+            const double m = (double)muT[f] + sd[f];
+            mu64[f] = m;
+            muT[f] = (float)m;
+        }
+    }
+}
+__global__ __launch_bounds__(1024) void k_sample_means_pack(const float* __restrict__ X, int64_t ns, int64_t ldxs, int64_t rows, int nparts,
+                                                            double inv_n, double* __restrict__ mu64, float* __restrict__ muT, int mean_blocks,
+                                                            const double* __restrict__ P, int64_t K, int64_t N, int64_t ldp,
+                                                            bf16x8* __restrict__ out, int NTtot, int64_t total) {
+    const int tid = threadIdx.x;
+    if ((int)blockIdx.x >= mean_blocks) {
+        const int64_t idx = (int64_t)(blockIdx.x - mean_blocks) * 1024 + tid;
+        if (idx < total) pack_p3_item(P, K, N, ldp, out, NTtot, idx);
+        return;
+    }
+    __shared__ double red[16][SCAN_RY][16];
+    __shared__ double psum[16][16];
+    const int cx = tid & 15, ry = (tid >> 4) & 3, p = tid >> 6;
+    const int64_t j = (int64_t)blockIdx.x * 16 + cx;
+    const int64_t r0 = (int64_t)p * rows, r1 = min(ns, r0 + rows);
+    double s0 = 0, s1 = 0, s2 = 0, s3 = 0;
+    if (p < nparts) {
+        int64_t i = r0 + ry;
+        for (; i + (8 * 4 - 1) * SCAN_RY < r1; i += 8 * 4 * SCAN_RY) {
+            float v[8][4];
+#pragma unroll
+            for (int u = 0; u < 8; ++u)
+#pragma unroll
+                for (int q = 0; q < 4; ++q) v[u][q] = X[(i + (4 * u + q) * SCAN_RY) * ldxs + j];
+#pragma unroll
+            for (int u = 0; u < 8; ++u) { s0 += (double)v[u][0]; s1 += (double)v[u][1]; s2 += (double)v[u][2]; s3 += (double)v[u][3]; }
+        }
+        for (; i + 3 * SCAN_RY < r1; i += 4 * SCAN_RY) {
+            const double v0 = (double)X[i * ldxs + j], v1 = (double)X[(i + SCAN_RY) * ldxs + j];
+            const double v2 = (double)X[(i + 2 * SCAN_RY) * ldxs + j], v3 = (double)X[(i + 3 * SCAN_RY) * ldxs + j];
+            s0 += v0; s1 += v1; s2 += v2; s3 += v3;
+        }
+        for (; i < r1; i += SCAN_RY) s0 += (double)X[i * ldxs + j];
+    }
+    red[p][ry][cx] = (s0 + s1) + (s2 + s3);
+    __syncthreads();
+    if (ry == 0) psum[p][cx] = (red[p][0][cx] + red[p][1][cx]) + (red[p][2][cx] + red[p][3][cx]);
+    __syncthreads();
+    if (tid < 16) {
+        double t = 0;
+        for (int q = 0; q < nparts; ++q) t += psum[q][tid];
+        t *= inv_n;
+        mu64[j] = t;
+        muT[j] = (float)t;
+    }
+}
 bool op_power_pass_means(Dev* d, int dt, const void* X, int64_t n, int64_t K, int64_t dcols, int64_t ldx, double n_total, const double* P,
                          int64_t N, int64_t ldp, int64_t L, double* Y, int64_t ldy, double* mu64, void* muT, double* ssq_scratch, double* tv) {
     const bool off = d->opt[OPT_MEANS_FOLD_ROWS] < 0 || pow3_knob_off(d, OPT_TWO_PLANE_OMEGA);
     if (off || L >= N || !pow3_ok(d, dt, X, n, K, ldx, muT, N, nullptr, 0)) return false;
     const int64_t ns = std::min<int64_t>(n, 4096), stride = n / ns;
-    op_colmean(d, dt, X, ns, K, ldx * stride, double(ns), mu64, muT, false);
     const int64_t total = (K / 32) * (N / 16) * 64;
     bf16x8* Ppk3 = (bf16x8*)dev_alloc(d, sizeof(bf16x8) * total * 3);
+    const int64_t srows = scan_rows_per_block(ns, K), sparts = cdiv64(ns, srows);
+    if (d->fold_merged && sparts <= 16) {
+        {
+            TagScope ts(d);
+            hipLaunchKernelGGL(k_sample_means_pack, dim3((unsigned)(K / 16 + cdiv(total, 1024))), dim3(1024), 0, d->stream, (const float*)X, ns,
+                               ldx * stride, srows, (int)sparts, 1.0 / double(ns), mu64, (float*)muT, (int)(K / 16), P, K, N, ldp, Ppk3,
+                               (int)(N / 16), total);
+            launch_check();
+            ts.stop();
+        }
+        double* parts = nullptr;
+        int nparts = 0;
+        double* sums = (double*)dev_alloc(d, sizeof(double) * K);
+        launch_pow3(d, (const float*)X, n, K, ldx, (const float*)muT, Ppk3, N, nullptr, 0, Y, ldy, &parts, &nparts, true, sums);
+        dev_free(d, Ppk3);
+        (void)ssq_scratch;
+        hipLaunchKernelGGL(k_mean_fix_col, dim3((unsigned)cdiv(L, 16) + 1), dim3(1024), 0, d->stream, Y, (int)K, (int)dcols, ldy, (int)L, n_total,
+                           (const double*)sums, P, ldp, mu64, (float*)muT, (const double*)parts, nparts, tv);
+        launch_check();
+        dev_free(d, sums);
+        dev_free(d, parts);
+        return true;
+    }
+    op_colmean(d, dt, X, ns, K, ldx * stride, double(ns), mu64, muT, false);
     hipLaunchKernelGGL(k_pack_p3, dim3(cdiv(total, 256)), dim3(256), 0, d->stream, P, K, N, ldp, Ppk3, (int)(N / 16), total);
     launch_check();
     double* parts = nullptr;
diff --git a/petal-decomposition_amd/csrc/kernels/k_eigen.inc b/petal-decomposition_amd/csrc/kernels/k_eigen.inc
--- a/petal-decomposition_amd/csrc/kernels/k_eigen.inc
+++ b/petal-decomposition_amd/csrc/kernels/k_eigen.inc
@@ -1303,50 +1303,57 @@
     sig[e] = s;
     inv[e] = (s > thr * s0 && s > 0.0) ? 1.0 / s : 0.0;
 }
+constexpr int COMPONENTS_LDS = 64 * 65 + 64 * 16;
+template <class T>
+__device__ __forceinline__ void components_out_block(const double* __restrict__ Bt, int64_t ldb, const double* __restrict__ Uh,
+                                                     int64_t ldu, const double* __restrict__ lam, double thr, int64_t d, int L,
+                                                     int64_t k, T* __restrict__ comp, int bx, int by, double (*sB)[65], double (*sU)[16]) {
+    const int tid = threadIdx.x, ti = tid & 15, tj = tid >> 4;
+    const int64_t i0 = (int64_t)bx * 64, j0 = (int64_t)by * 16;
+    double acc[4] = {0.0, 0.0, 0.0, 0.0};
+    for (int l0 = 0; l0 < L; l0 += 64) {
+        double vb[16], vu[4];
+#pragma unroll
+        for (int u = 0; u < 16; ++u) {
+            const int r = (tid >> 6) + 4 * u, l = l0 + (tid & 63);
+            vb[u] = (i0 + r < d && l < L) ? Bt[(i0 + r) * ldb + l] : 0.0;
+        }
+#pragma unroll
+        for (int u = 0; u < 4; ++u) {
+            const int l = l0 + (tid >> 4) + 16 * u;
+            vu[u] = (l < L && j0 + ti < k) ? Uh[(int64_t)l * ldu + j0 + ti] : 0.0;
+        }
+        __syncthreads();
+#pragma unroll
+        for (int u = 0; u < 16; ++u) sB[(tid >> 6) + 4 * u][tid & 63] = vb[u];
+#pragma unroll
+        for (int u = 0; u < 4; ++u) sU[(tid >> 4) + 16 * u][ti] = vu[u];
+        __syncthreads();
+#pragma unroll 8
+        for (int l = 0; l < 64; ++l) {
+            const double u = sU[l][tj];
+#pragma unroll
+            for (int r = 0; r < 4; ++r) acc[r] += sB[ti + 16 * r][l] * u;
+        }
+    }
+    const int64_t j = j0 + tj;
+    if (j < k) {
+        const double s = sqrt(fmax(lam[j], 0.0)), s0 = sqrt(fmax(lam[0], 0.0));
+        const double inv = (s > thr * s0 && s > 0.0) ? 1.0 / s : 0.0;
+#pragma unroll
+        for (int r = 0; r < 4; ++r) {
+            const int64_t i = i0 + ti + 16 * r;
+            if (i < d) comp[j * d + i] = (T)(acc[r] * inv);
+        }
+    }
+}
 template <class T>
 __global__ __launch_bounds__(256) void k_components_out(const double* __restrict__ Bt, int64_t ldb, const double* __restrict__ Uh,
                                                         int64_t ldu, const double* __restrict__ lam, double thr, int64_t d, int L,
                                                         int64_t k, T* __restrict__ comp) {
     __shared__ double sB[64][65];
     __shared__ double sU[64][16];
-    const int tid = threadIdx.x, ti = tid & 15, tj = tid >> 4;
-    const int64_t i0 = (int64_t)blockIdx.x * 64, j0 = (int64_t)blockIdx.y * 16;
-    double acc[4] = {0.0, 0.0, 0.0, 0.0};
-    for (int l0 = 0; l0 < L; l0 += 64) {
-        double vb[16], vu[4];
-#pragma unroll
-        for (int u = 0; u < 16; ++u) {
-            const int r = (tid >> 6) + 4 * u, l = l0 + (tid & 63);
-            vb[u] = (i0 + r < d && l < L) ? Bt[(i0 + r) * ldb + l] : 0.0;
-        }
-#pragma unroll
-        for (int u = 0; u < 4; ++u) {
-            const int l = l0 + (tid >> 4) + 16 * u;
-            vu[u] = (l < L && j0 + ti < k) ? Uh[(int64_t)l * ldu + j0 + ti] : 0.0;
-        }
-        __syncthreads();
-#pragma unroll
-        for (int u = 0; u < 16; ++u) sB[(tid >> 6) + 4 * u][tid & 63] = vb[u];
-#pragma unroll
-        for (int u = 0; u < 4; ++u) sU[(tid >> 4) + 16 * u][ti] = vu[u];
-        __syncthreads();
-#pragma unroll 8
-        for (int l = 0; l < 64; ++l) {
-            const double u = sU[l][tj];
-#pragma unroll
-            for (int r = 0; r < 4; ++r) acc[r] += sB[ti + 16 * r][l] * u;
-        }
-    }
-    const int64_t j = j0 + tj;
-    if (j < k) {
-        const double s = sqrt(fmax(lam[j], 0.0)), s0 = sqrt(fmax(lam[0], 0.0));
-        const double inv = (s > thr * s0 && s > 0.0) ? 1.0 / s : 0.0;
-#pragma unroll
-        for (int r = 0; r < 4; ++r) {
-            const int64_t i = i0 + ti + 16 * r;
-            if (i < d) comp[j * d + i] = (T)(acc[r] * inv);
-        }
-    }
+    components_out_block<T>(Bt, ldb, Uh, ldu, lam, thr, d, L, k, comp, (int)blockIdx.x, (int)blockIdx.y, sB, sU);
 }
 __global__ void k_scale_pad_cols(const double* __restrict__ V, int64_t ldv, const double* __restrict__ inv, int64_t rows, int64_t r,
                                  int64_t rp, double* __restrict__ P) {
diff --git a/petal-decomposition_amd/csrc/kernels/k_gemm_split_k1.inc b/petal-decomposition_amd/csrc/kernels/k_gemm_split_k1.inc
--- a/petal-decomposition_amd/csrc/kernels/k_gemm_split_k1.inc
+++ b/petal-decomposition_amd/csrc/kernels/k_gemm_split_k1.inc
@@ -51,10 +51,8 @@
     h = __builtin_bit_cast(bf16x8, hh);
     m = __builtin_bit_cast(bf16x8, mm);
 }
-__global__ __launch_bounds__(256) void k_pack_p3(const double* __restrict__ P, int64_t K, int64_t N, int64_t ldp,
-                                                 bf16x8* __restrict__ out, int NTtot, int64_t total) {
-    const int64_t idx = (int64_t)blockIdx.x * 256 + threadIdx.x;
-    if (idx >= total) return;
+__device__ __forceinline__ void pack_p3_item(const double* __restrict__ P, int64_t K, int64_t N, int64_t ldp, bf16x8* __restrict__ out,
+                                             int NTtot, int64_t idx) {
     const int lane = (int)(idx & 63);
     const int64_t tile = idx >> 6;
     const int nt = (int)(tile % NTtot);
@@ -68,6 +66,11 @@
     out[(tile * 3 + 0) * 64 + lane] = h;
     out[(tile * 3 + 1) * 64 + lane] = m;
     out[(tile * 3 + 2) * 64 + lane] = l;
+}
+__global__ __launch_bounds__(256) void k_pack_p3(const double* __restrict__ P, int64_t K, int64_t N, int64_t ldp,
+                                                 bf16x8* __restrict__ out, int NTtot, int64_t total) {
+    const int64_t idx = (int64_t)blockIdx.x * 256 + threadIdx.x;
+    if (idx < total) pack_p3_item(P, K, N, ldp, out, NTtot, idx);
 }
 #ifndef PETAL_XP3_RT
 #define PETAL_XP3_RT 4
diff --git a/petal-decomposition_amd/csrc/kernels/k_generic.inc b/petal-decomposition_amd/csrc/kernels/k_generic.inc
--- a/petal-decomposition_amd/csrc/kernels/k_generic.inc
+++ b/petal-decomposition_amd/csrc/kernels/k_generic.inc
@@ -167,12 +167,10 @@
         *o = accumulate ? *o + t : t;
     }
 }
-__global__ __launch_bounds__(256) void k_sum_parts4(const float* __restrict__ part, int64_t nparts, int64_t count,
-                                                    double* __restrict__ out, int64_t N, int64_t ldc) {
+__device__ __forceinline__ bool sum_parts4_pair(const float* __restrict__ part, int64_t nparts, int64_t count, int64_t e, double& s0, double& s1) {
     __shared__ double red[3][64][3];
     const int lane = threadIdx.x & 63, wave = threadIdx.x >> 6;
-    const int64_t e = ((int64_t)blockIdx.x * 64 + lane) * 2;
-    double s0 = 0, s1 = 0;
+    s0 = 0; s1 = 0;
     if (e < count) {
         const float* src = part + e;
         int64_t p = wave;
@@ -190,11 +188,29 @@
     }
     if (wave > 0) { red[wave - 1][lane][0] = s0; red[wave - 1][lane][1] = s1; }
     __syncthreads();
-    if (wave == 0 && e < count) {
-#pragma unroll
-        for (int w = 0; w < 3; ++w) { s0 += red[w][lane][0]; s1 += red[w][lane][1]; }
+    if (wave != 0 || e >= count) return false;
+#pragma unroll
+    for (int w = 0; w < 3; ++w) { s0 += red[w][lane][0]; s1 += red[w][lane][1]; }
+    return true;
+}
+__global__ __launch_bounds__(256) void k_sum_parts4(const float* __restrict__ part, int64_t nparts, int64_t count,
+                                                    double* __restrict__ out, int64_t N, int64_t ldc) {
+    const int64_t e = ((int64_t)blockIdx.x * 64 + (threadIdx.x & 63)) * 2;
+    double s0, s1;
+    if (sum_parts4_pair(part, nparts, count, e, s0, s1)) {
         double* o = out + (e / N) * ldc + (e % N);
         o[0] = s0; o[1] = s1;
+    }
+}
+__global__ __launch_bounds__(256) void k_sum_parts4_col(const float* __restrict__ part, int64_t nparts, int64_t count,
+                                                        double* __restrict__ out, int64_t N, int64_t ldc, int64_t c1, double* __restrict__ col) {
+    const int64_t e = ((int64_t)blockIdx.x * 64 + (threadIdx.x & 63)) * 2;
+    double s0, s1;
+    if (sum_parts4_pair(part, nparts, count, e, s0, s1)) {
+        const int64_t r = e / N, c = e % N;
+        double* o = out + r * ldc + c;
+        o[0] = s0;
+        if (c + 1 == c1) { col[r] = s1; o[1] = 0.0; } else o[1] = s1;
     }
 }
 __global__ __launch_bounds__(256) void k_add_scalar_parts(const double* __restrict__ part, int64_t nparts, double* __restrict__ out) {
diff --git a/petal-decomposition_amd/csrc/kernels/k_smallmat.inc b/petal-decomposition_amd/csrc/kernels/k_smallmat.inc
--- a/petal-decomposition_amd/csrc/kernels/k_smallmat.inc
+++ b/petal-decomposition_amd/csrc/kernels/k_smallmat.inc
@@ -173,66 +173,76 @@
 }
 
 template <int NB>
+__device__ __forceinline__ void trsm_left_solve(const double* __restrict__ RT, int64_t ldt, const double* __restrict__ B, int64_t ldb,
+                                                double* __restrict__ X_out, int64_t ldxo, int blk, double* __restrict__ sX) {
+    constexpr int M = 16 * NB, MP = (M + 31) / 32 * 32;
+    const int lane = threadIdx.x, li = lane & 15, lk = lane >> 4;
+    const int64_t j0 = (int64_t)blk * 16;
+    cf64x4 X[NB];
+#pragma unroll
+    for (int I = 0; I < NB; ++I)
+#pragma unroll
+        for (int r = 0; r < 4; ++r) X[I][r] = B[(int64_t)(16 * I + lk + 4 * r) * ldb + j0 + li];
+    cf64x4 rt[2][NB];
+    auto load_row = [&](int I, cf64x4(&dst)[NB]) {
+        const double* rrow = RT + (int64_t)(16 * I + li) * ldt + lk;
+#pragma unroll
+        for (int K = 0; K < NB; ++K)
+            if (K >= I) {
+#pragma unroll
+                for (int r = 0; r < 4; ++r) dst[K][r] = rrow[16 * K + 4 * r];
+            }
+    };
+    load_row(NB - 1, rt[(NB - 1) & 1]);
+#pragma unroll
+    for (int I = NB - 1; I >= 0; --I) {
+        if (I > 0) load_row(I - 1, rt[(I - 1) & 1]);
+        const cf64x4(&cur)[NB] = rt[I & 1];
+        cf64x4 acc = X[I];
+#pragma unroll
+        for (int K = I + 1; K < NB; ++K) {
+#pragma unroll
+            for (int r = 0; r < 4; ++r) acc = __builtin_amdgcn_mfma_f64_16x16x4f64(-cur[K][r], X[K][r], acc, 0, 0, 0);
+        }
+        cf64x4 xi = cf64x4{0.0, 0.0, 0.0, 0.0};
+#pragma unroll
+        for (int r = 0; r < 4; ++r) xi = __builtin_amdgcn_mfma_f64_16x16x4f64(cur[I][r], acc[r], xi, 0, 0, 0);
+        X[I] = xi;
+#pragma unroll
+        for (int r = 0; r < 4; ++r) {
+            sX[(16 * I + lk + 4 * r) * 17 + li] = xi[r];
+            if (X_out) X_out[(int64_t)(16 * I + lk + 4 * r) * ldxo + j0 + li] = xi[r];
+        }
+        __builtin_amdgcn_sched_barrier(0);
+    }
+    if (MP > M)
+        for (int e = lane; e < (MP - M) * 17; e += 64) sX[M * 17 + e] = 0.0;
+}
+template <int NB>
+__device__ __forceinline__ void trsm_left_planes(const double* __restrict__ sX, bf16x8* __restrict__ pk3, int NTtot, int blk) {
+    constexpr int M = 16 * NB, MP = (M + 31) / 32 * 32;
+    const int lane = threadIdx.x, li = lane & 15, lk = lane >> 4;
+#pragma unroll
+    for (int cc = 0; cc < MP / 32; ++cc) {
+        f32x8 x;
+#pragma unroll
+        for (int e = 0; e < 8; ++e) x[e] = (float)sX[(32 * cc + 8 * lk + e) * 17 + li];
+        bf16x8 h, m, l;
+        split3(x, h, m, l);
+        const int64_t tile = (int64_t)cc * NTtot + blk;
+        pk3[(tile * 3 + 0) * 64 + lane] = h;
+        pk3[(tile * 3 + 1) * 64 + lane] = m;
+        pk3[(tile * 3 + 2) * 64 + lane] = l;
+    }
+}
+template <int NB>
 __global__ __launch_bounds__(64) void k_trsm_left_pack(const double* __restrict__ RT, int64_t ldt, const double* __restrict__ B, int64_t ldb,
                                                        double* __restrict__ X_out, int64_t ldxo, bf16x8* __restrict__ pk3, int NTtot) {
     constexpr int M = 16 * NB, MP = (M + 31) / 32 * 32;
     __shared__ double sX[MP * 17];
-    const int lane = threadIdx.x, li = lane & 15, lk = lane >> 4;
-    const int64_t j0 = (int64_t)blockIdx.x * 16;
-    cf64x4 X[NB];
-#pragma unroll
-    for (int I = 0; I < NB; ++I)
-#pragma unroll
-        for (int r = 0; r < 4; ++r) X[I][r] = B[(int64_t)(16 * I + lk + 4 * r) * ldb + j0 + li];
-    cf64x4 rt[2][NB];
-    auto load_row = [&](int I, cf64x4(&dst)[NB]) {
-        const double* rrow = RT + (int64_t)(16 * I + li) * ldt + lk;
-#pragma unroll
-        for (int K = 0; K < NB; ++K)
-            if (K >= I) {
-#pragma unroll
-                for (int r = 0; r < 4; ++r) dst[K][r] = rrow[16 * K + 4 * r];
-            }
-    };
-    load_row(NB - 1, rt[(NB - 1) & 1]);
-#pragma unroll
-    for (int I = NB - 1; I >= 0; --I) {
-        if (I > 0) load_row(I - 1, rt[(I - 1) & 1]);
-        const cf64x4(&cur)[NB] = rt[I & 1];
-        cf64x4 acc = X[I];
-#pragma unroll
-        for (int K = I + 1; K < NB; ++K) {
-#pragma unroll
-            for (int r = 0; r < 4; ++r) acc = __builtin_amdgcn_mfma_f64_16x16x4f64(-cur[K][r], X[K][r], acc, 0, 0, 0);
-        }
-        cf64x4 xi = cf64x4{0.0, 0.0, 0.0, 0.0};
-#pragma unroll
-        for (int r = 0; r < 4; ++r) xi = __builtin_amdgcn_mfma_f64_16x16x4f64(cur[I][r], acc[r], xi, 0, 0, 0);
-        X[I] = xi;
-#pragma unroll
-        for (int r = 0; r < 4; ++r) {
-            sX[(16 * I + lk + 4 * r) * 17 + li] = xi[r];
-            if (X_out) X_out[(int64_t)(16 * I + lk + 4 * r) * ldxo + j0 + li] = xi[r];
-        }
-        __builtin_amdgcn_sched_barrier(0);
-    }
-    if (MP > M)
-        for (int e = lane; e < (MP - M) * 17; e += 64) sX[M * 17 + e] = 0.0;
-    __syncthreads();
-    if (pk3) {
-#pragma unroll
-        for (int cc = 0; cc < MP / 32; ++cc) {
-            f32x8 x;
-#pragma unroll
-            for (int e = 0; e < 8; ++e) x[e] = (float)sX[(32 * cc + 8 * lk + e) * 17 + li];
-            bf16x8 h, m, l;
-            split3(x, h, m, l);
-            const int64_t tile = (int64_t)cc * NTtot + blockIdx.x;
-            pk3[(tile * 3 + 0) * 64 + lane] = h;
-            pk3[(tile * 3 + 1) * 64 + lane] = m;
-            pk3[(tile * 3 + 2) * 64 + lane] = l;
-        }
-    }
+    trsm_left_solve<NB>(RT, ldt, B, ldb, X_out, ldxo, (int)blockIdx.x, sX);
+    __syncthreads();
+    if (pk3) trsm_left_planes<NB>(sX, pk3, NTtot, (int)blockIdx.x);
 }
 
 constexpr int CHOL_THREADS = 512;
diff --git a/petal-decomposition_amd/csrc/ops.h b/petal-decomposition_amd/csrc/ops.h
--- a/petal-decomposition_amd/csrc/ops.h
+++ b/petal-decomposition_amd/csrc/ops.h
@@ -53,6 +53,9 @@
 };
 void   dev_set_option(Dev*, int opt, double value);
 double dev_option(const Dev*, int opt);
+enum PetalMerge { MERGE_FOLD = 0, MERGE_TAIL = 1, MERGE_COUNT = 2 };
+void   dev_set_launch_merge(Dev*, int which, bool merged);
+bool   dev_launch_merge(const Dev*, int which);
 void  dev_set_gemm_mode(Dev*, int mode);
 int   dev_gemm_mode(const Dev*);
 void  dev_make_current(Dev*);
@@ -162,6 +165,16 @@
                           double* P_out, int64_t ldpo, void* Z, int64_t ldz, double* Y, int64_t ldy, bool steering = false);
 void op_tail_verdict(Dev*, const double* lam, int64_t L, int64_t k, const double* mu_sq, int64_t dp, int64_t d, double n_total,
                      const double* tv, double eps2, double thr, int* flag2);
+struct SmallStageConsumers {
+    const double *lam, *Uh; int64_t ldu, L, LP;
+    bool verdict; const double *mu_sq, *tv; double n_total, eps2, verdict_thr; int* flag2;
+    const double* Bt; int64_t ldb; double comp_thr; int64_t d, dp, k; void* comp;
+    const double* RT; int64_t ldt; bool rt_form; int64_t N; double* P_out; int64_t ldpo;
+};
+bool op_small_stage_consumers(Dev*, int dtype, int64_t n, const SmallStageConsumers&, void** planes);
+void op_gemm_xp_packed_absmax(Dev*, int dtype, const void* X, int64_t n, int64_t K, int64_t ldx, const double* P, int64_t N, int64_t ldp,
+                              void* planes, void* Z, int64_t ldz, int64_t row_offset, double* absmax, double* idx, double* sign,
+                              bool store_product);
 void op_gemm_atb(Dev*, int dtype, const void* A, int64_t lda, int64_t M, const void* muA,
                  const void* B, int64_t ldb, int64_t N, const void* muB, int64_t n,
                  double* C, int64_t ldc, bool precise = false, bool steering = false);
```
